# pashtari/factorizer

Hardware: AMD Instinct MI355X
Metric: volumes/sec fwd+bwd, Swin Factorizer 128^3 (higher is better)
Workload: dtype f32

## Files before the change

### factorizer_amd/csrc/mlp_chain.hip

```cpp
#include "mlp_chain.h"

using namespace fz;

static int mlp_nacc() { return 2; }

extern "C" int64_t fz_mlp_partials(int B, int64_t V) {
  const int64_t tw = 128 * mlp_nacc();
  return ((V + tw - 1) / tw) * (int64_t)B;
}

extern "C" int fz_mlp_pre_supported(int C, int H, int64_t V, int products) {
  if (!(V > 0 && (V % 4) == 0 && V <= ((int64_t)1 << 27) && products_split(products))) return 0;
  if (C == 32 && H == 64) return knob_chain_fwd_bx() ? 1 : 0;
  if (C == 64 && H == 128) return (((V + 255) / 256) % 2 == 0 && knob_chain64_p512()) ? 1 : 0;
  return 0;
}

extern "C" int fz_outproj_factors_supported(int C, int Hd, int D, int H, int W, int d, int pd, int ph, int pw, int R, int T, int Tgrad,
                                            int nshift, const int* shifts, int act_dtype, int products, int dropout) {
  if (C != 32 || Hd != 64 || act_dtype != FZ_STORE_F32 || dropout || nshift != 2) return 0;
  if (!fz_nmf_cf_factors_supported(C, D, H, W, d, pd, ph, pw, R, T, Tgrad, nshift, shifts)) return 0;
  return fz_mlp_pre_supported(C, Hd, (int64_t)D * H * W, products);
}

extern "C" int fz_mlp_supported(int C, int H, int64_t V) {
  const bool shape = (C == 32 && (H == 64 || H == 128)) || (C == 64 && H == 128);
  return (shape && V > 0 && (V % 4) == 0 && V <= ((int64_t)1 << 27)) ? 1 : 0;
}

extern "C" int fz_mlp_drop_supported(int C, int H, int64_t V, int products) {
  return (C == 32 && H == 64 && fz_mlp_supported(C, H, V) && fz_mlp_pre_supported(C, H, V, products) && products_split(products)
          && knob_chain_fwd_bx()) ? 1 : 0;
}

template <typename AT>
static void forward_args(const fz_mlp_desc* d, bool fac, int ldw, int ldwB, GemmArgsT<AT>& a, ChainArgsT<AT>& c) {
  a.w = d->w1; a.w_t = 0; a.ldw = ldw;
  a.bias = d->b1; a.ln = 1; a.ln_g = d->ln_g; a.ln_b = d->ln_b; a.ln_eps = d->ln_eps; a.stats_out = d->stats;
  a.res = (const AT*)d->in; a.y = (AT*)d->out;
  c.wB = d->w2; c.wB_t = 0; c.ldwB = ldwB; c.biasB = d->b2; c.side = (AT*)d->z1;
  if (d->pre_in || fac) {
    c.preA = (const AT*)d->pre_in; c.preW = d->pre_w; c.preB = d->pre_b; c.preRes = (const AT*)d->pre_res; c.preOut = (AT*)d->pre_out;
    if (d->C == 64) a.res = (const AT*)d->pre_out;
    else { c.postW = d->post_w; c.postB = d->post_b; c.postOut = (AT*)d->post_out; c.postM = d->post_m; }
  }
}
template <typename AT>
static void backward_args(const fz_mlp_desc* d, int ldw, int ldwB, AT* side, GemmArgsT<AT>& a, ChainArgsT<AT>& c) {
  a.w = d->w2; a.w_t = 1; a.ldw = ldw;
  a.emul = (const AT*)d->z1; a.y = (AT*)d->out;
  a.lnb_x = (const AT*)d->x1; a.lnb_stats = d->stats; a.lnb_g = d->ln_g; a.lnb_gadd = (const AT*)d->in; a.lnb_part = d->part;
  c.wB = d->w1; c.wB_t = 1; c.ldwB = ldwB; c.side = side;
}

static int mlp_check(const fz_mlp_desc* d, const fz_mlp_dropout* dd, bool drop, bool fac) {
  if (!fz_mlp_supported(d->C, d->H, d->V)) return fail(FZ_E_UNSUPPORTED, "fz_mlp_chain: needs (C, H) in {(32, 64), (32, 128), (64, 128)}, V % 4 == 0");
  if (drop) {
    if (!fz_mlp_drop_supported(d->C, d->H, d->V, d->products) || d->mode != 0 || !d->pre_in)
      return fail(FZ_E_UNSUPPORTED, "fz_mlp_chain: dropout needs (C, H) = (32, 64), split-bf16 products, mode 0 with pre_in (fz_mlp_drop_supported)");
    if (!drop_scale_ok(dd->m0, dd->s0) || !drop_scale_ok(dd->m1, dd->s1) || !drop_scale_ok(dd->m2, dd->s2))
      return fail(FZ_E_ARG, "fz_mlp_chain: a dropout scale 1 / (1 - p) must be >= 1 and finite");
  }
  if (d->C == 64 && d->mode == 2) return fail(FZ_E_UNSUPPORTED, "fz_mlp_chain: the fused weight gradients need C == 32, H == 64");
  if (d->B < 0) return fail(FZ_E_SHAPE, "fz_mlp_chain: negative batch");
  if (fac && (d->C != 32 || d->H != 64 || d->mode != 0 || d->act_dtype != FZ_STORE_F32 || drop || d->pre_in
              || !fz_mlp_pre_supported(d->C, d->H, d->V, d->products)))
    return fail(FZ_E_UNSUPPORTED, "fz_mlp_chain_fac: needs (C, H) = (32, 64), mode 0, fp32 storage, split-bf16 products, pre_in == NULL (fz_outproj_factors_supported)");
  const bool pre = d->pre_in != nullptr || fac;
  if (pre && (d->mode != 0 || !d->pre_w || !d->pre_res || !d->pre_out))
    return fail(FZ_E_ARG, "fz_mlp_chain: pre_in needs mode 0, pre_w, pre_res, pre_out (see fz_mlp_pre_supported)");
  if (pre && !fz_mlp_pre_supported(d->C, d->H, d->V, d->products))
    return fail(FZ_E_UNSUPPORTED, "fz_mlp_chain: the fused out-projection runs on split-bf16 products only (fz_mlp_pre_supported)");
  if (d->post_out && (!pre || d->C != 32 || !d->post_w || d->post_m < 1 || d->post_m > 4))
    return fail(FZ_E_ARG, "fz_mlp_chain: post_out needs pre_in, C == 32, post_w and 1 <= post_m <= 4");
  if ((!d->in && !pre) || !d->w1 || !d->w2 || !d->out || !d->z1 || !d->stats)
    return fail(FZ_E_ARG, "fz_mlp_chain: null pointer");
  if (d->mode == 0 && (!d->ln_g || !d->ln_b)) return fail(FZ_E_ARG, "fz_mlp_chain: forward needs the LayerNorm affine");
  if (d->mode == 1 && (!d->gz1 || !d->x1 || !d->ln_g || !d->part)) return fail(FZ_E_ARG, "fz_mlp_chain: backward needs gz1, x1, gamma, part");
  if (d->mode == 2 && (!d->x1 || !d->ln_g || !d->ln_b || !d->gln || !d->wpart || !d->gw1 || !d->gb1 || !d->gw2 || !d->gb2))
    return fail(FZ_E_ARG, "fz_mlp_chain: backward with weight gradients needs x1, gamma, beta, gln, wpart, gw1, gb1, gw2, gb2");
  if (d->mode == 2 && d->H == 128 && !d->glp) return fail(FZ_E_ARG, "fz_mlp_chain: the fused weight gradients at H == 128 need the glp buffer");
  if (d->mode < 0 || d->mode > 2) return fail(FZ_E_ARG, "fz_mlp_chain: bad mode");
  return FZ_OK;
}

template <typename AT>
static int mlp_launch(const fz_mlp_desc* d, const fz_mlp_dropout* dd, const fz_outproj_fac* fac, fz_stream_t stream) {
  const bool drop = dd && (dd->m0 || dd->m1 || dd->m2);
  const int rc = mlp_check(d, dd, drop, fac != nullptr);
  if (rc != FZ_OK) return rc;
  if (d->B == 0) {
    if (d->mode == 2) {
      hipStream_t s0 = (hipStream_t)stream;
      FZ_HIP_OK(hipMemsetAsync(d->gw1, 0, sizeof(float) * d->H * 32, s0));
      FZ_HIP_OK(hipMemsetAsync(d->gw2, 0, sizeof(float) * d->H * 32, s0));
      FZ_HIP_OK(hipMemsetAsync(d->gb1, 0, sizeof(float) * d->H, s0));
      FZ_HIP_OK(hipMemsetAsync(d->gb2, 0, sizeof(float) * 32, s0));
      FZ_HIP_OK(hipMemsetAsync(d->gln, 0, sizeof(float) * 64, s0));
    }
    return FZ_OK;
  }
  GemmArgsT<AT> a = {};
  ChainArgsT<AT> c = {};
  a.x[0] = (const AT*)d->in; a.nsrc = 1; a.c0 = d->C; a.Cin = d->C; a.Vin = d->V; a.M = d->H; a.K = d->C; a.Ncol = d->V; a.B = d->B;
  if (d->mode == 0) forward_args(d, fac != nullptr, d->C, d->H, a, c);
  else backward_args(d, d->H, d->C, d->mode == 1 ? (AT*)d->gz1 : (AT*)nullptr, a, c);
  if (d->C == 64) return chain64_launch(d, a, c, stream);
  if (d->mode == 2) return chain_wg_launch(d, a, c, stream);
  return chain32_launch(d, drop ? dd : nullptr, fac, a, c, stream);
}

extern "C" int fz_mlp_chain(const fz_mlp_desc* d, fz_stream_t stream) {
  if (!d) return fail(FZ_E_ARG, "fz_mlp_chain: null descriptor");
  if (d->act_dtype == FZ_STORE_F32) return mlp_launch<float>(d, nullptr, nullptr, stream);
  if (d->act_dtype == FZ_STORE_BF16) return mlp_launch<bf16>(d, nullptr, nullptr, stream);
  return fail(FZ_E_ARG, "fz_mlp_chain: act_dtype must be FZ_STORE_F32 or FZ_STORE_BF16");
}

extern "C" int fz_mlp_chain_fac(const fz_mlp_desc* d, const fz_outproj_fac* fac, fz_stream_t stream) {
  if (!d || !fac) return fail(FZ_E_ARG, "fz_mlp_chain_fac: null descriptor");
  if (d->act_dtype == FZ_STORE_F32) return mlp_launch<float>(d, nullptr, fac, stream);
  if (d->act_dtype == FZ_STORE_BF16) return mlp_launch<bf16>(d, nullptr, fac, stream);
  return fail(FZ_E_ARG, "fz_mlp_chain_fac: act_dtype must be FZ_STORE_F32 or FZ_STORE_BF16");
}

extern "C" int fz_mlp_chain_drop(const fz_mlp_desc* d, const fz_mlp_dropout* drop, fz_stream_t stream) {
  if (!d || !drop) return fail(FZ_E_ARG, "fz_mlp_chain_drop: null descriptor");
  if (d->act_dtype == FZ_STORE_F32) return mlp_launch<float>(d, drop, nullptr, stream);
  if (d->act_dtype == FZ_STORE_BF16) return mlp_launch<bf16>(d, drop, nullptr, stream);
  return fail(FZ_E_ARG, "fz_mlp_chain_drop: act_dtype must be FZ_STORE_F32 or FZ_STORE_BF16");
}
```

### factorizer_amd/csrc/mlp_chain64.hip

```cpp
#include "mlp_chain.h"

namespace fz {

template <bool HOIST, int NRB, int NQ, int NTA, int NTB, typename FA, typename FX>
__device__ __forceinline__ void bx_group(f32x16 (&acc)[NRB][NQ], FA load_a, FX get_x) {
  if constexpr (HOIST) {
    bx8 bop[NQ][NTB];
#pragma unroll
    for (int q = 0; q < NQ; ++q) {
      float x8[8];
      get_x(q, x8);
      bx_split<NTB>(x8, bop[q]);
    }
#pragma unroll
    for (int rb = 0; rb < NRB; ++rb) {
      float a8[8];
      load_a(rb, a8);
      bx8 aop[NTA];
      bx_split<NTA>(a8, aop);
#pragma unroll
      for (int q = 0; q < NQ; ++q) bx_mfma<NTA, NTB>(acc[rb][q], aop, bop[q]);
    }
  } else {
#pragma unroll
    for (int q = 0; q < NQ; ++q) {
      bx8 bop[NTB];
      {
        float x8[8];
        get_x(q, x8);
        bx_split<NTB>(x8, bop);
      }
#pragma unroll
      for (int rb = 0; rb < NRB; ++rb) {
        float a8[8];
        load_a(rb, a8);
        bx8 aop[NTA];
        bx_split<NTA>(a8, aop);
        bx_mfma<NTA, NTB>(acc[rb][q], aop, bop);
      }
      __builtin_amdgcn_sched_barrier(0);
    }
  }
}

template <int NRB, int NQ, int NTB, typename FA, typename FX>
__device__ __forceinline__ void bx_group_ps(f32x16 (&acc)[NRB][NQ], FA load_term, FX get_x) {
#pragma unroll
  for (int q = 0; q < NQ; ++q) {
    bx8 bop[NTB];
    {
      float x8[8];
      get_x(q, x8);
      bx_split<NTB>(x8, bop);
    }
#pragma unroll
    for (int rb = 0; rb < NRB; ++rb) {
#pragma unroll
      for (int t = 2; t >= 0; --t) {
        const bx8 a = load_term(rb, t);
#pragma unroll
        for (int jj = NTB - 1; jj >= 0; --jj)
          if (t + jj <= 2) acc[rb][q] = __builtin_amdgcn_mfma_f32_32x32x16_bf16(a, bop[jj], acc[rb][q], 0, 0, 0);
      }
      __builtin_amdgcn_sched_barrier(0);
    }
  }
}

template <bool BWD, typename AT, bool SINGLE = false, bool BX = false, bool P512 = false, bool PRE = false>
__global__ __launch_bounds__(P512 ? 512 : 256, 2) void gemm_chain64_kernel(GemmArgsT<AT> p, ChainArgsT<AT> c, int ntiles) {
  constexpr int NACC = 2, C = 64, HID = 128;
  constexpr int NTA = BxTerms<AT>::A, NTB = bx_terms_b<AT>(BXPRO_GELU);
  constexpr bool HOIST = SINGLE || sizeof(AT) == 2;
  static_assert(!P512 || (BX && !SINGLE), "P512: the split-bf16 chain around a pre-split weight image");
  static_assert(!PRE || (P512 && !BWD), "PRE: the forward chain around the pre-split images");
  constexpr int NA = P512 ? 12288 : 8192;
  constexpr int NA0 = PRE ? 6144 : 0;
  extern __shared__ __attribute__((aligned(16))) float fz_lds_c64[];
  float* As1 = fz_lds_c64;
  float* As2 = As1 + NA;
  float* tW = As2 + NA + NA0;
  float* tB = tW + 128;
  float* tB0 = tB + 64;
  const int half = P512 ? __builtin_amdgcn_readfirstlane((int)(threadIdx.x >> 8)) : 0;
  float* red = tB + 64 + (PRE ? 64 : 0) + half * 512;
  static_assert(2 * NA + NA0 + 128 + 64 + (PRE ? 64 : 0) + (P512 ? 2 : 1) * 512 == chain64_lds_floats(P512, PRE), "the launcher's dynamic LDS ends where this carve-up does");
  const int lane = threadIdx.x & 63, wave = __builtin_amdgcn_readfirstlane((int)(threadIdx.x >> 6) & 3);
  const int j = lane & 31, h = lane >> 5;
  const int tiles_per_sample = (int)((p.Ncol + 128 * NACC - 1) / (128 * NACC));
  int lane4 = lane * 4, lane4b = lane * 4 + NA, lane4c = lane * 4 + 2 * NA;
  if constexpr (P512) {
    asm volatile("" : "+v"(lane4));
    asm volatile("" : "+v"(lane4b));
    if constexpr (PRE) asm volatile("" : "+v"(lane4c));
  }
  auto ld_a1 = [&](int slot3) { return *reinterpret_cast<const bx8*>(As1 + slot3 * 256 + lane4); };
  auto ld_a2 = [&](int slot3) { return *reinterpret_cast<const bx8*>(As1 + slot3 * 256 + lane4b); };
  auto ld_a0 = [&](int slot3) { return *reinterpret_cast<const bx8*>(As1 + slot3 * 256 + lane4c); };
  (void)ld_a0; (void)lane4c; (void)tB0;

  if constexpr (P512) {
    for (int item = threadIdx.x; item < (PRE ? 2560 : 2048); item += 512) {
      const int l = item & 63, slot = (item >> 6) & 15, img = item >> 10;
      float a8[8];
      if (img == 0) {
        const int g = slot >> 2, rb = slot & 3;
#pragma unroll
        for (int e = 0; e < 8; ++e) {
          const int rr = 8 * (g & 1) + e;
          const int k = PRE ? (g >> 1) * 32 + (rr & 3) + 8 * (rr >> 2) + 4 * (l >> 5) : 2 * (8 * g + e) + (l >> 5);
          a8[e] = weight_at(p, rb * 32 + (l & 31), k);
          if (!BWD) a8[e] *= p.ln_g[k];
        }
      } else if (PRE && img == 2) {
        const int g = slot >> 1, mb = slot & 1;
#pragma unroll
        for (int e = 0; e < 8; ++e) a8[e] = c.preW[(int64_t)(mb * 32 + (l & 31)) * 64 + 2 * (8 * g + e) + (l >> 5)];
      } else {
        const int mb = slot & 1, g8 = (slot >> 1) & 1, rb4 = slot >> 2;
#pragma unroll
        for (int e = 0; e < 8; ++e) {
          const int r = 8 * g8 + e;
          const int k = rb4 * 32 + (r & 3) + 8 * (r >> 2) + 4 * (l >> 5), m = mb * 32 + (l & 31);
          a8[e] = c.wB_t ? c.wB[(int64_t)k * c.ldwB + m] : c.wB[(int64_t)m * c.ldwB + k];
        }
      }
      bx8 t3[3];
      bx_split<3>(a8, t3);
      bx8* dst = reinterpret_cast<bx8*>(img == 0 ? As1 : (img == 1 ? As2 : As2 + NA)) + (slot * 3) * 64 + l;
      dst[0] = t3[0]; dst[64] = t3[1]; dst[128] = t3[2];
    }
  }
  for (int base = threadIdx.x; !P512 && base < (SINGLE ? 4096 : 16384); base += 256 * 8) {
    float tmp[8];
#pragma unroll
    for (int uu = 0; uu < 8; ++uu) {
      const int idx = base + uu * 256;
      float wv;
      if (SINGLE) {
        const int l = idx & 63, mb = (idx >> 6) & 1, a = idx >> 7;
        wv = weight_at(p, mb * 32 + (l & 31), 2 * a + (l >> 5));
      } else if (idx < 8192) {
        const int l = idx & 63, rb = (idx >> 6) & 3, a = idx >> 8;
        const int m = rb * 32 + (l & 31), k = 2 * a + (l >> 5);
        wv = weight_at(p, m, k);
        if (!BWD) wv *= p.ln_g[k];
      } else {
        const int i2 = idx - 8192;
        const int l = i2 & 63, mb = (i2 >> 6) & 1, s2 = i2 >> 7;
        const int r = s2 & 15, rb = s2 >> 4;
        const int k = rb * 32 + (r & 3) + 8 * (r >> 2) + 4 * (l >> 5), m = mb * 32 + (l & 31);
        wv = c.wB_t ? c.wB[(int64_t)k * c.ldwB + m] : c.wB[(int64_t)m * c.ldwB + k];
      }
      tmp[uu] = wv;
    }
#pragma unroll
    for (int uu = 0; uu < 8; ++uu) fz_lds_c64[base + uu * 256] = tmp[uu];
  }
  if (BWD) {
    if (threadIdx.x < C) tB[threadIdx.x] = p.lnb_g[threadIdx.x];
  } else {
    for (int r = threadIdx.x; r < HID; r += blockDim.x) {
      float t = 0.f;
      for (int k = 0; k < C; ++k) t += weight_at(p, r, k) * p.ln_b[k];
      tW[r] = t + (p.bias ? p.bias[r] : 0.f);
      if (r < C) tB[r] = c.biasB ? c.biasB[r] : 0.f;
      if (PRE && r < C) tB0[r] = c.preB ? c.preB[r] : 0.f;
    }
  }

  const int tstep = P512 ? 2 * (int)gridDim.x : (int)gridDim.x;
  int tile = P512 ? 2 * (int)blockIdx.x + half : (int)blockIdx.x;
  float bv[32][NACC];
  auto fetch_tile = [&](int t) {
    const int bt = t / tiles_per_sample;
    const int64_t ct = ((int64_t)(t % tiles_per_sample) * 4 + wave) * (32 * NACC) + NACC * j;
    const unsigned lo = (unsigned)h * (unsigned)p.Ncol + (unsigned)(ct < p.Ncol ? ct : 0);
    const AT* xb = (PRE ? c.preA : p.x[0]) + (int64_t)bt * C * p.Ncol;
#pragma unroll
    for (int s = 0; s < 32; ++s) vload<NACC>(xb + (int64_t)(2 * s) * p.Ncol + lo, bv[s]);
  };
  fetch_tile(tile);
  __syncthreads();

  for (; tile < ntiles; tile += tstep) {
    asm volatile("" ::: "memory");
    const int b = tile / tiles_per_sample;
    const int64_t col_off = ((int64_t)(tile % tiles_per_sample) * 4 + wave) * (32 * NACC) + NACC * j;
    const bool col_ok = col_off < p.Ncol;
    const int64_t nc = col_ok ? col_off : 0;
    const unsigned lane_row = (unsigned)(4 * h) * (unsigned)p.Ncol + (unsigned)nc;

    f32x16 acc0[PRE ? 2 : 1][NACC];
    if constexpr (PRE) {
#pragma unroll
      for (int mb = 0; mb < 2; ++mb)
#pragma unroll
        for (int q = 0; q < NACC; ++q)
#pragma unroll
          for (int r = 0; r < 16; ++r) acc0[mb][q][r] = 0.f;
#pragma unroll
      for (int g = 0; g < 4; ++g) {
        bx_group_ps<2, NACC, NTB>(acc0,
            [&](int mb, int t) { return ld_a0((g * 2 + mb) * 3 + t); },
            [&](int q, float (&x8)[8]) {
#pragma unroll
              for (int e = 0; e < 8; ++e) x8[e] = bv[8 * g + e][q];
            });
        __builtin_amdgcn_sched_barrier(0);
      }
      const int64_t smp = (int64_t)b * C * p.Ncol;
      float s1[NACC] = {0.f, 0.f};
#pragma unroll
      for (int g8 = 0; g8 < 4; ++g8) {
        float e[8][NACC];
#pragma unroll
        for (int i = 0; i < 8; ++i) {
          const int rr = g8 * 8 + i, mb = rr >> 4, r = rr & 15;
          vload<NACC>(c.preRes + smp + (int64_t)(mb * 32 + (r & 3) + 8 * (r >> 2)) * p.Ncol + lane_row, e[i]);
        }
#pragma unroll
        for (int i = 0; i < 8; ++i) {
          const int rr = g8 * 8 + i, mb = rr >> 4, r = rr & 15;
          const int rbase = mb * 32 + (r & 3) + 8 * (r >> 2);
          const float add = tB0[rbase + 4 * h];
          float v[NACC];
#pragma unroll
          for (int q = 0; q < NACC; ++q) v[q] = acc0[mb][q][r] + add + e[i][q];
          if (col_ok) vstore<NACC>(c.preOut + smp + (int64_t)rbase * p.Ncol + lane_row, v);
#pragma unroll
          for (int q = 0; q < NACC; ++q) {
            if constexpr (sizeof(AT) == 2) v[q] = (float)(AT)v[q];
            acc0[mb][q][r] = v[q];
            s1[q] += v[q];
          }
        }
        __builtin_amdgcn_sched_barrier(0);
      }
      float mu[NACC], rs[NACC];
#pragma unroll
      for (int q = 0; q < NACC; ++q) {
        s1[q] += __shfl_xor(s1[q], 32, 64);
        mu[q] = s1[q] / 64.0f;
        float t = 0.f;
#pragma unroll
        for (int mb = 0; mb < 2; ++mb)
#pragma unroll
          for (int r = 0; r < 16; ++r) {
            const float dd = acc0[mb][q][r] - mu[q];
            t += dd * dd;
          }
        t += __shfl_xor(t, 32, 64);
        rs[q] = 1.0f / sqrtf(t / 64.0f + p.ln_eps);
#pragma unroll
        for (int mb = 0; mb < 2; ++mb)
#pragma unroll
          for (int r = 0; r < 16; ++r) acc0[mb][q][r] = (acc0[mb][q][r] - mu[q]) * rs[q];
      }
      if (p.stats_out != nullptr && h == 0 && col_ok) {
        float* so = p.stats_out + (int64_t)b * 2 * p.Vin;
        vstore<NACC>(so + col_off, mu);
        vstore<NACC>(so + p.Vin + col_off, rs);
      }
    }

    if (!BWD && !PRE) {
      float mu[NACC], rs[NACC];
#pragma unroll
      for (int e = 0; e < NACC; ++e) {
        float t = 0.f;
#pragma unroll
        for (int s = 0; s < 32; ++s) t += bv[s][e];
        t += __shfl_xor(t, 32, 64);
        mu[e] = t / 64.0f;
      }
#pragma unroll
      for (int e = 0; e < NACC; ++e) {
        float t = 0.f;
#pragma unroll
        for (int s = 0; s < 32; ++s) {
          const float d = bv[s][e] - mu[e];
          t += d * d;
        }
        t += __shfl_xor(t, 32, 64);
        rs[e] = 1.0f / sqrtf(t / 64.0f + p.ln_eps);
      }
#pragma unroll
      for (int s = 0; s < 32; ++s)
#pragma unroll
        for (int e = 0; e < NACC; ++e) bv[s][e] = (bv[s][e] - mu[e]) * rs[e];
      if (p.stats_out != nullptr && h == 0 && col_ok) {
        float* so = p.stats_out + (int64_t)b * 2 * p.Vin;
        vstore<NACC>(so + col_off, mu);
        vstore<NACC>(so + p.Vin + col_off, rs);
      }
    }

    f32x16 acc2[2][NACC];
#pragma unroll
    for (int mb = 0; mb < 2; ++mb)
#pragma unroll
      for (int q = 0; q < NACC; ++q)
#pragma unroll
        for (int r = 0; r < 16; ++r) acc2[mb][q][r] = 0.f;

    if (SINGLE) {
      if constexpr (BX) {
#pragma unroll
        for (int g = 0; g < 4; ++g) {
          bx_group<HOIST, 2, NACC, NTA, NTB>(acc2,
              [&](int mb, float (&a8)[8]) {
#pragma unroll
                for (int e = 0; e < 8; ++e) a8[e] = As1[((8 * g + e) * 2 + mb) * 64 + lane];
              },
              [&](int q, float (&x8)[8]) {
#pragma unroll
                for (int e = 0; e < 8; ++e) x8[e] = bv[8 * g + e][q];
              });
          __builtin_amdgcn_sched_barrier(0);
        }
      } else {
#pragma unroll
      for (int s = 0; s < 32; ++s) {
#pragma unroll
        for (int mb = 0; mb < 2; ++mb) {
          const float av = As1[(s * 2 + mb) * 64 + lane];
#pragma unroll
          for (int q = 0; q < NACC; ++q) acc2[mb][q] = __builtin_amdgcn_mfma_f32_32x32x2f32(av, bv[s][q], acc2[mb][q], 0, 0, 0);
        }
        if ((s & 3) == 3) __builtin_amdgcn_sched_barrier(0);
      }
      }
      fetch_tile(tile + tstep < ntiles ? tile + tstep : tile);
    }
#pragma unroll
    for (int p2 = 0; p2 < (SINGLE ? 0 : 2); ++p2) {
      f32x16 acc1[2][NACC];
#pragma unroll
      for (int rbl = 0; rbl < 2; ++rbl)
#pragma unroll
        for (int q = 0; q < NACC; ++q)
#pragma unroll
          for (int r = 0; r < 16; ++r) acc1[rbl][q][r] = 0.f;
      if constexpr (BX) {
#pragma unroll
        for (int g = 0; g < 4; ++g) {
          if constexpr (P512)
            bx_group_ps<2, NACC, NTB>(acc1,
                [&](int rbl, int t) { return ld_a1((g * 4 + 2 * p2 + rbl) * 3 + t); },
                [&](int q, float (&x8)[8]) {
#pragma unroll
                  for (int e = 0; e < 8; ++e) x8[e] = PRE ? acc0[PRE ? (g >> 1) : 0][q][8 * (g & 1) + e] : bv[8 * g + e][q];
                });
          else
          bx_group<HOIST, 2, NACC, NTA, NTB>(acc1,
              [&](int rbl, float (&a8)[8]) {
#pragma unroll
                for (int e = 0; e < 8; ++e) a8[e] = As1[((8 * g + e) * 4 + 2 * p2 + rbl) * 64 + lane];
              },
              [&](int q, float (&x8)[8]) {
#pragma unroll
                for (int e = 0; e < 8; ++e) x8[e] = bv[8 * g + e][q];
              });
          __builtin_amdgcn_sched_barrier(0);
        }
      } else {
#pragma unroll
      for (int s = 0; s < 32; ++s) {
#pragma unroll
        for (int rbl = 0; rbl < 2; ++rbl) {
          const float av = As1[(s * 4 + 2 * p2 + rbl) * 64 + lane];
#pragma unroll
          for (int q = 0; q < NACC; ++q) acc1[rbl][q] = __builtin_amdgcn_mfma_f32_32x32x2f32(av, bv[s][q], acc1[rbl][q], 0, 0, 0);
        }
        if ((s & 3) == 3) __builtin_amdgcn_sched_barrier(0);
      }
      }
      if (p2 == 1) fetch_tile(tile + tstep < ntiles ? tile + tstep : tile);

      if (!BWD) {
#pragma unroll
        for (int rbl = 0; rbl < 2; ++rbl)
#pragma unroll
          for (int r = 0; r < 16; ++r) {
            const int rbase = (2 * p2 + rbl) * 32 + (r & 3) + 8 * (r >> 2);
            const float add = tW[rbase + 4 * h];
            float v[NACC];
#pragma unroll
            for (int q = 0; q < NACC; ++q) v[q] = acc1[rbl][q][r] + add;
            if (col_ok) vstore<NACC>(c.side + ((int64_t)b * HID + rbase) * p.Ncol + lane_row, v);
            if constexpr (NACC == 2) {
              float gq[2];
              gelu2_f(v, gq);
              acc1[rbl][0][r] = gq[0]; acc1[rbl][1][r] = gq[1];
            } else {
#pragma unroll
              for (int q = 0; q < NACC; ++q) acc1[rbl][q][r] = gelu_f(v[q]);
            }
          }
      } else {
#pragma unroll
        for (int g8 = 0; g8 < 4; ++g8) {
          float e[8][NACC];
#pragma unroll
          for (int i = 0; i < 8; ++i) {
            const int rr = g8 * 8 + i, rbl = rr >> 4, r = rr & 15;
            const int rbase = (2 * p2 + rbl) * 32 + (r & 3) + 8 * (r >> 2);
            vload<NACC>(p.emul + ((int64_t)b * HID + rbase) * p.Ncol + lane_row, e[i]);
          }
#pragma unroll
          for (int i = 0; i < 8; ++i) {
            const int rr = g8 * 8 + i, rbl = rr >> 4, r = rr & 15;
            const int rbase = (2 * p2 + rbl) * 32 + (r & 3) + 8 * (r >> 2);
            float v[NACC];
#pragma unroll
            for (int q = 0; q < NACC; ++q) v[q] = acc1[rbl][q][r] * gelu_grad_f(e[i][q]);
            if (col_ok) vstore<NACC>(c.side + ((int64_t)b * HID + rbase) * p.Ncol + lane_row, v);
#pragma unroll
            for (int q = 0; q < NACC; ++q) acc1[rbl][q][r] = v[q];
          }
          __builtin_amdgcn_sched_barrier(0);
        }
      }

      if constexpr (BX) {
#pragma unroll
        for (int g = 0; g < 4; ++g) {
          if constexpr (P512)
            bx_group_ps<2, NACC, NTB>(acc2,
                [&](int mb, int t) { return ld_a2((((2 * p2 + (g >> 1)) * 2 + (g & 1)) * 2 + mb) * 3 + t); },
                [&](int q, float (&x8)[8]) {
#pragma unroll
                  for (int e = 0; e < 8; ++e) x8[e] = acc1[g >> 1][q][8 * (g & 1) + e];
                });
          else
          bx_group<HOIST, 2, NACC, NTA, NTB>(acc2,
              [&](int mb, float (&a8)[8]) {
#pragma unroll
                for (int e = 0; e < 8; ++e) a8[e] = As2[(((2 * p2 + (g >> 1)) * 16 + 8 * (g & 1) + e) * 2 + mb) * 64 + lane];
              },
              [&](int q, float (&x8)[8]) {
#pragma unroll
                for (int e = 0; e < 8; ++e) x8[e] = acc1[g >> 1][q][8 * (g & 1) + e];
              });
          __builtin_amdgcn_sched_barrier(0);
        }
      } else {
#pragma unroll
      for (int rbl = 0; rbl < 2; ++rbl)
#pragma unroll
        for (int r = 0; r < 16; ++r) {
#pragma unroll
          for (int mb = 0; mb < 2; ++mb) {
            const float av = As2[(((2 * p2 + rbl) * 16 + r) * 2 + mb) * 64 + lane];
#pragma unroll
            for (int q = 0; q < NACC; ++q) acc2[mb][q] = __builtin_amdgcn_mfma_f32_32x32x2f32(av, acc1[rbl][q][r], acc2[mb][q], 0, 0, 0);
          }
          if ((r & 3) == 3) __builtin_amdgcn_sched_barrier(0);
        }
      }
    }

    const int64_t sample = (int64_t)b * C * p.Ncol;
    if (!BWD) {
#pragma unroll
      for (int g8 = 0; g8 < 4; ++g8) {
        float e[8][NACC];
#pragma unroll
        for (int i = 0; i < 8; ++i) {
          const int rr = g8 * 8 + i, mb = rr >> 4, r = rr & 15;
          vload<NACC>(p.res + sample + (int64_t)(mb * 32 + (r & 3) + 8 * (r >> 2)) * p.Ncol + lane_row, e[i]);
        }
#pragma unroll
        for (int i = 0; i < 8; ++i) {
          const int rr = g8 * 8 + i, mb = rr >> 4, r = rr & 15;
          const int rbase = mb * 32 + (r & 3) + 8 * (r >> 2);
          const float add = tB[rbase + 4 * h];
          float v[NACC];
#pragma unroll
          for (int q = 0; q < NACC; ++q) v[q] = acc2[mb][q][r] + add + e[i][q];
          if (col_ok) vstore<NACC>(p.y + sample + (int64_t)rbase * p.Ncol + lane_row, v);
        }
        __builtin_amdgcn_sched_barrier(0);
      }
    } else {
      const float* sp = p.lnb_stats + (int64_t)b * 2 * p.Ncol;
      float mu[NACC], rs[NACC];
      vload<NACC>(sp + nc, mu);
      vload<NACC>(sp + p.Ncol + nc, rs);
      float xs[32][NACC];
      float m1[NACC] = {0.f, 0.f}, m2[NACC] = {0.f, 0.f};
#pragma unroll
      for (int g8 = 0; g8 < 4; ++g8) {
#pragma unroll
        for (int i = 0; i < 8; ++i) {
          const int rr = g8 * 8 + i, mb = rr >> 4, r = rr & 15;
          vload<NACC>(p.lnb_x + sample + (int64_t)(mb * 32 + (r & 3) + 8 * (r >> 2)) * p.Ncol + lane_row, xs[rr]);
        }
#pragma unroll
        for (int i = 0; i < 8; ++i) {
          const int rr = g8 * 8 + i, mb = rr >> 4, r = rr & 15;
          const float gc = tB[mb * 32 + (r & 3) + 8 * (r >> 2) + 4 * h];
#pragma unroll
          for (int q = 0; q < NACC; ++q) {
            const float av = acc2[mb][q][r] * gc;
            xs[rr][q] = (xs[rr][q] - mu[q]) * rs[q];
            m1[q] += av;
            m2[q] += av * xs[rr][q];
          }
        }
        __builtin_amdgcn_sched_barrier(0);
      }
#pragma unroll
      for (int q = 0; q < NACC; ++q) {
        m1[q] = (m1[q] + __shfl_xor(m1[q], 32, 64)) * (1.0f / 64.0f);
        m2[q] = (m2[q] + __shfl_xor(m2[q], 32, 64)) * (1.0f / 64.0f);
      }
#pragma unroll
      for (int g8 = 0; g8 < 4; ++g8) {
        float ga[8][NACC];
#pragma unroll
        for (int i = 0; i < 8; ++i) {
          const int rr = g8 * 8 + i, mb = rr >> 4, r = rr & 15;
          vload<NACC>(p.lnb_gadd + sample + (int64_t)(mb * 32 + (r & 3) + 8 * (r >> 2)) * p.Ncol + lane_row, ga[i]);
        }
#pragma unroll
        for (int i = 0; i < 8; ++i) {
          const int rr = g8 * 8 + i, mb = rr >> 4, r = rr & 15;
          const int rbase = mb * 32 + (r & 3) + 8 * (r >> 2);
          const int row = rbase + 4 * h;
          const float gc = tB[row];
          float v[NACC];
#pragma unroll
          for (int q = 0; q < NACC; ++q) v[q] = rs[q] * (acc2[mb][q][r] * gc - m1[q] - xs[rr][q] * m2[q]) + ga[i][q];
          if (col_ok) vstore<NACC>(p.y + sample + (int64_t)rbase * p.Ncol + lane_row, v);
          float sg = col_ok ? acc2[mb][0][r] * xs[rr][0] + acc2[mb][1][r] * xs[rr][1] : 0.f;
          float sb = col_ok ? acc2[mb][0][r] + acc2[mb][1][r] : 0.f;
          sg = half_sum32(sg);
          sb = half_sum32(sb);
          if ((lane & 31) == 31) {
            red[wave * 128 + row] = sg;
            red[wave * 128 + 64 + row] = sb;
          }
        }
        __builtin_amdgcn_sched_barrier(0);
      }
      __syncthreads();
      if ((threadIdx.x & 255) < 128) {
        const int e = threadIdx.x & 255;
        p.lnb_part[(int64_t)tile * 128 + e] = (red[e] + red[128 + e]) + (red[256 + e] + red[384 + e]);
      }
      __syncthreads();
    }
  }
}

template <typename AT>
int chain64_launch(const fz_mlp_desc* d, const GemmArgsT<AT>& a, const ChainArgsT<AT>& c, fz_stream_t stream) {
  const int ntiles = (int)fz_mlp_partials(d->B, d->V);
  const bool bwd = d->mode != 0, pre = d->pre_in != nullptr;
  const bool p512 = products_split(d->products) && ntiles % 2 == 0 && knob_chain64_p512();
  if (pre && !p512) return fail(FZ_E_UNSUPPORTED, "fz_mlp_chain: the fused out-projection at C == 64 needs an even number of tiles");
  void (*kern)(GemmArgsT<AT>, ChainArgsT<AT>, int) =
      pre ? gemm_chain64_kernel<false, AT, false, true, true, true>
      : p512 ? (bwd ? gemm_chain64_kernel<true, AT, false, true, true> : gemm_chain64_kernel<false, AT, false, true, true>)
             : (bwd ? gemm_chain64_kernel<true, AT, false, false> : gemm_chain64_kernel<false, AT, false, false>);
  const int work = p512 ? ntiles / 2 : ntiles, wgs = p512 ? 256 : knob_mlp_wgs(512);
  return launch_lds(kern, dim3((unsigned)(work < wgs ? work : wgs)), dim3(p512 ? 512 : 256), chain64_lds_floats(p512, pre),
                    (hipStream_t)stream, a, c, ntiles);
}
template int chain64_launch<float>(const fz_mlp_desc*, const GemmArgsT<float>&, const ChainArgsT<float>&, fz_stream_t);
template int chain64_launch<bf16>(const fz_mlp_desc*, const GemmArgsT<bf16>&, const ChainArgsT<bf16>&, fz_stream_t);

template <typename AT>
int chain64_lnb_launch(const fz_gemm_desc* d, const GemmArgsT<AT>& a, fz_stream_t stream) {
  if (d->Ncol % 4 != 0) return fail(FZ_E_UNSUPPORTED, "fz_gemm: voxel count must be a multiple of 4");
  if (!d->lnb_gadd) return fail(FZ_E_UNSUPPORTED, "fz_gemm: the 64-channel LayerNorm-backward epilogue needs the added gradient");
  ChainArgsT<AT> c = {};
  const int ntiles = (int)fz_mlp_partials(d->B, d->Ncol);
  if (gemm_plan_only())
    return gemm_plan_form("chain64_lnb %s grid=%dx1", products_split(d->products) ? "split" : "fp32", ntiles < 512 ? ntiles : 512);
  auto kern = products_split(d->products) ? gemm_chain64_kernel<true, AT, true, true> : gemm_chain64_kernel<true, AT, true, false>;
  return launch_lds(kern, dim3((unsigned)(ntiles < 512 ? ntiles : 512)), dim3(256), chain64_lds_floats(false, false),
                    (hipStream_t)stream, a, c, ntiles);
}
template int chain64_lnb_launch<float>(const fz_gemm_desc*, const GemmArgsT<float>&, fz_stream_t);
template int chain64_lnb_launch<bf16>(const fz_gemm_desc*, const GemmArgsT<bf16>&, fz_stream_t);

}
```

### factorizer_amd/pointwise.py

```python
from __future__ import annotations

import collections
import ctypes
import functools
import os
import threading as _threading
import weakref

import torch
import torch.nn.functional as F

from . import _native as N
from . import gradbuf as _GB
from . import functional as Fn

ACT = dict(zip(("none", "relu", "gelu"), N.constants("ACT_NONE", "ACT_RELU", "ACT_GELU")))
LOAD_PLAIN, LOAD_S2D, LOAD_K3, LOAD_S2D_2D, LOAD_K3_2D = N.constants("LOAD_PLAIN", "LOAD_S2D", "LOAD_K3", "LOAD_S2D_2D", "LOAD_K3_2D")
EPI_PLAIN, EPI_D2S, EPI_LNBWD, EPI_D2S_2D = N.constants("EPI_PLAIN", "EPI_D2S", "EPI_LNBWD", "EPI_D2S_2D")
QL_S2D_2D, QL_K3_2D = N.constants("QL_S2D_2D", "QL_K3_2D")
_D2S_FINE = {EPI_D2S: 8, EPI_D2S_2D: 4}


_p = N.ptr


def _vox(x):
    v = 1
    for s in x.shape[2:]:
        v *= s
    return v


def _ln_stats(B, V, dev):
    return torch.empty((B, 2, V), dtype=torch.float32, device=dev)


def _gemm_desc(xs, w, y, *, B, Cin, Vin, M, K, Ncol, w_t=False, ldw=None, bias=None, ln=None, stats_out=None,
               bact=0, bmul=None, bmul_kind=0, eact=0, res=None, emul=None, emul_kind=0, src_mode=0, c0=0,
               loader=LOAD_PLAIN, epilogue=EPI_PLAIN, Di=0, Hi=0, Wi=0, Ho=0, Wo=0, name="gemm", tune=0, lnb=None):
    d = N.GemmDesc()
    d.products = N.products()
    d.tune = tune
    for i in range(4):
        d.x[i] = _p(xs[i]) if i < len(xs) else None
    d.nsrc, d.src_mode, d.c0, d.Cin, d.Vin = len(xs), src_mode, c0, Cin, Vin
    d.Di, d.Hi, d.Wi = Di, Hi, Wi
    d.w, d.w_t, d.ldw, d.M, d.K = _p(w), int(w_t), (ldw if ldw is not None else K), M, K
    d.bias = _p(bias)
    if ln is not None:
        d.ln, d.ln_g, d.ln_b, d.ln_eps = 1, _p(ln[0]), _p(ln[1]), float(ln[2])
    d.stats_out = _p(stats_out)
    d.bact, d.bmul, d.bmul_kind = bact, _p(bmul), bmul_kind
    d.eact, d.res, d.emul, d.emul_kind = eact, _p(res), _p(emul), emul_kind
    d.y, d.Ncol, d.Ho, d.Wo, d.B = _p(y), Ncol, Ho, Wo, B
    d.loader, d.epilogue = loader, epilogue
    x0 = xs[0]
    d.act_dtype = N.act_dtype(x0)
    nbytes = x0.element_size() * (sum(t.numel() for t in xs) + y.numel() + (res.numel() if res is not None else 0))
    if lnb is not None:
        d.lnb_x, d.lnb_stats, d.lnb_g, d.lnb_gadd = (_p(t) for t in lnb)
        nbytes += x0.element_size() * (lnb[0].numel() + (lnb[3].numel() if lnb[3] is not None else 0))
    return d, f"{name}_{Cin}->{M}", nbytes, B * max(Vin, Ncol * _D2S_FINE.get(epilogue, 1)), 2 * B * Ncol * M * K


def _gemm_launch(x0, d, key, nbytes, cols, flops):
    rc = Fn._timed(key, nbytes, lambda: N.lib().fz_gemm(ctypes.byref(d), N.stream_ptr(x0)), cols=cols, flops=flops)
    N.check(rc, "fz_gemm")


def _gemm(xs, w, y, **kw):
    with torch.cuda.device(xs[0].device):
        _gemm_launch(xs[0], *_gemm_desc(xs, w, y, **kw))
    return y


def _wgrad_desc(p, qs, gw, *, B, M, Cin, K, Vq, Ncols, gbias=None, pmul=None, pmul_kind=0, src_mode=0, c0=0,
                stats=None, qact=0, ln=None, loader=0, D=0, H=0, W=0, Ho=0, Wo=0, accumulate=False, name="wgrad"):
    d = N.WgradDesc()
    d.products = N.products()
    d.p, d.M, d.pmul, d.pmul_kind = _p(p), M, _p(pmul), pmul_kind
    for i in range(4):
        d.q[i] = _p(qs[i]) if i < len(qs) else None
    d.nsrc, d.src_mode, d.c0, d.Cin, d.K, d.Vq = len(qs), src_mode, c0, Cin, K, Vq
    d.D, d.H, d.W, d.N, d.Ho, d.Wo = D, H, W, Ncols, Ho, Wo
    d.stats, d.qact = _p(stats), qact
    if ln is not None:
        d.ln_g, d.ln_b = _p(ln[0]), _p(ln[1])
    d.gw, d.gbias, d.accumulate, d.B, d.loader = _p(gw), _p(gbias), int(accumulate), B, loader
    d.act_dtype = N.act_dtype(p)
    nb = N.lib().fz_wgrad_workspace_bytes(ctypes.byref(d))
    if nb < 0:
        raise N.NativeError("fz_wgrad_workspace_bytes failed")
    ws = torch.empty(max(nb // 4, 1), dtype=torch.float32, device=p.device)
    nbytes = p.element_size() * (p.numel() + sum(t.numel() for t in qs))
    return d, ws, f"{name}_{M}x{K}", nbytes, B * max(Vq, Ncols), 2 * B * Ncols * M * K


def _wgrad(p, qs, gw, **kw):
    d, ws, key, nbytes, cols, flops = _wgrad_desc(p, qs, gw, **kw)
    with torch.cuda.device(p.device), _finish_scope(ws, gw, kw.get("gbias")):
        rc = Fn._timed(key, nbytes, lambda: N.lib().fz_wgrad(ctypes.byref(d), ws.data_ptr(), N.stream_ptr(p)),
                       cols=cols, flops=flops)
    N.check(rc, "fz_wgrad")
    return gw


_WGRAD_GROUP = os.environ.get("FZ_WGRAD_GROUP", "1") != "0"


def _wgrad_group(problems, name):
    plans = [_wgrad_desc(p, qs, gw, **kw) for p, qs, gw, kw in problems]
    n = len(plans)
    descs = (ctypes.POINTER(N.WgradDesc) * n)(*[ctypes.pointer(pl[0]) for pl in plans])
    wss = (ctypes.c_void_p * n)(*[pl[1].data_ptr() for pl in plans])
    t0 = problems[0][0]
    held = [pl[1] for pl in plans] + [pr[2] for pr in problems] + [pr[3].get("gbias") for pr in problems]
    with torch.cuda.device(t0.device), _finish_scope(*held):
        rc = Fn._timed(name, sum(pl[3] for pl in plans),
                       lambda: N.lib().fz_wgrad_group(descs, wss, n, N.stream_ptr(t0)),
                       cols=max(pl[4] for pl in plans), flops=sum(pl[5] for pl in plans))
    N.check(rc, "fz_wgrad_group")


def _ln_backward(gl, x, stats, ln_w, gadd=None):
    B, C = x.shape[:2]
    V = _vox(x)
    gx = torch.empty_like(x)
    gpar = torch.empty(2 * C, dtype=torch.float32, device=x.device)
    ws = torch.empty(max(N.lib().fz_ln_bwd_workspace_bytes2(B, C, V) // 4, 1), dtype=torch.float32, device=x.device)
    with torch.cuda.device(x.device), _finish_scope(ws, gpar):
        rc = Fn._timed(f"ln_bwd_{C}", 3 * x.element_size() * x.numel(), lambda: N.lib().fz_ln_bwd(
            gl.data_ptr(), x.data_ptr(), stats.data_ptr(), ln_w.data_ptr(), _p(gadd), gx.data_ptr(), _p(gpar), _p(ws),
            B, C, V, N.act_dtype(x), N.stream_ptr(x)), cols=B * V)
    N.check(rc, "fz_ln_bwd")
    return gx, gpar[:C], gpar[C:]


def _reduce_affine_rows(part, rows, C, like):
    gpar = torch.empty(2 * C, dtype=torch.float32, device=like.device)
    tmp = torch.empty((64, 2 * C), dtype=torch.float32, device=like.device)
    with _finish_scope(part, gpar, tmp):
        rc = N.lib().fz_reduce_rows(part.data_ptr(), rows, 2 * C, gpar.data_ptr(), tmp.data_ptr(), N.stream_ptr(like))
    N.check(rc, "fz_reduce_rows")
    return gpar[:C], gpar[C:]


def _dgrad_lnbwd(gz, w2, x, stats, ln_w, gadd):
    B, C = x.shape[:2]
    V = _vox(x)
    Mz = gz.shape[1]
    fused64 = C == 64 and Mz == 64 and gadd is not None and V % 4 == 0 and os.environ.get("FZ_LNBWD64", "1") != "0"
    if not fused64 and (C != 32 or Mz > 64 or Mz % 2):
        gl = torch.empty_like(x)
        _gemm([gz], w2, gl, B=B, Cin=Mz, Vin=V, M=C, K=Mz, Ncol=V, w_t=True, ldw=C, name="linear_dgrad")
        return _ln_backward(gl, x, stats, ln_w, gadd=gadd)
    gx = torch.empty_like(x)
    d, *timed = _gemm_desc([gz], w2, gx, B=B, Cin=Mz, Vin=V, M=C, K=Mz, Ncol=V, w_t=True, ldw=C, epilogue=EPI_LNBWD,
                           lnb=(x, stats, ln_w, gadd), name="dgrad_lnbwd")
    rows = N.lib().fz_gemm_lnbwd_partials(ctypes.byref(d))
    part = torch.empty((rows, 2 * C), dtype=torch.float32, device=x.device)
    d.lnb_part = part.data_ptr()
    with torch.cuda.device(x.device):
        _gemm_launch(gz, d, *timed)
        ggamma, gbeta = _reduce_affine_rows(part, rows, C, x)
    return gx, ggamma, gbeta


def _dw_fused_ok(C, V):
    return C == 32 and V % 4 == 0 and V <= (1 << 27) and os.environ.get("FZ_DW_FUSED", "1") != "0"


def _gemm_dw(g, w2, q, ln=None, stats=None, gadd=None, want_bias=False, name="dgrad_wgrad", gw_out=None, gb_out=None, drop=None,
             fac=None):
    if fac is not None:
        q = g
    B, C = q.shape[:2]
    V = _vox(q)
    dev = q.device
    y = torch.empty_like(q)
    gw = _GB.out_like(w2, (C, C), torch.float32) if gw_out is None else gw_out
    gb = (gb_out if gb_out is not None else torch.empty(C, dtype=torch.float32, device=dev)) if want_bias else None
    wpart = torch.empty(N.lib().fz_gemm_dw_workspace_bytes(B, V) // 4, dtype=torch.float32, device=dev)
    d = N.GemmDwDesc()
    d.g, d.q, d.w, d.y = g.data_ptr(), q.data_ptr() if fac is None else None, w2.data_ptr(), y.data_ptr()
    df = N.outproj_fac(*fac) if fac is not None else None
    d.wpart, d.gw, d.gb = wpart.data_ptr(), gw.data_ptr(), _p(gb)
    d.B, d.C, d.V, d.act_dtype = B, C, V, N.act_dtype(q)
    d.ldgw = gw.stride(0)
    d.ldw = w2.stride(0)
    if drop is not None:
        d.drop_m, d.drop_s = drop[0].data_ptr(), _drop_scale(drop[1])
    gpar = None
    if ln is not None:
        gpar = torch.empty(64, dtype=torch.float32, device=dev)
        d.ln, d.stats, d.ln_g, d.ln_b, d.gadd, d.gln = 1, stats.data_ptr(), ln[0].data_ptr(), ln[1].data_ptr(), _p(gadd), gpar.data_ptr()
    nbytes = q.element_size() * ((3 * q.numel() if fac is None else 2 * q.numel() + q.numel() // 4) + (gadd.numel() if gadd is not None else 0))
    with torch.cuda.device(dev), _finish_scope(wpart, gw, gb, gpar):
        rc = Fn._timed(f"{name}_{C}", nbytes,
                       lambda: (N.lib().fz_gemm_dw(ctypes.byref(d), N.stream_ptr(q)) if df is None
                                else N.lib().fz_gemm_dw_fac(ctypes.byref(d), ctypes.byref(df), N.stream_ptr(q))),
                       cols=B * V, flops=4 * B * V * C * C)
        N.check(rc, "fz_gemm_dw")
    if ln is not None:
        return y, gw, gb, gpar[:32], gpar[32:]
    return y, gw, gb, None, None


def _drop_scale(p):
    return 1.0 / (1.0 - float(ctypes.c_float(p).value))


def _mlp_dropout(drop):
    bits, ps = drop
    dd = N.MlpDropout()
    for s in range(3):
        if bits[s] is not None:
            setattr(dd, f"m{s}", bits[s].data_ptr())
            setattr(dd, f"s{s}", _drop_scale(ps[s]))
    return dd


def _mlp_drop_ok(C, Hd, V):
    return (_outproj_mlp_ok(C, Hd, V)
            and bool(N.lib().fz_mlp_drop_supported(C, Hd, V, N.products())))


def _mlp_chain_ok(C, Hd, V):
    return os.environ.get("FZ_MLP_CHAIN", "1") != "0" and bool(N.lib().fz_mlp_supported(C, Hd, V))


def _mlp_desc(mode, like, w12, w22, *, B, C, Hd, V, inp=None, b1=None, b2=None, ln_w=None, ln_b=None, eps=0.0, stats=None, z1=None,
              x1=None, out=None):
    d = N.MlpDesc()
    d.products = N.products()
    d.mode, d.inp, d.w1, d.w2, d.b1, d.b2 = mode, _p(inp), w12.data_ptr(), w22.data_ptr(), _p(b1), _p(b2)
    d.ln_g, d.ln_b, d.ln_eps = _p(ln_w), _p(ln_b), float(eps)
    d.stats, d.z1, d.x1, d.out = _p(stats), _p(z1), _p(x1), _p(out)
    d.B, d.C, d.H, d.V = B, C, Hd, V
    d.act_dtype = N.act_dtype(like)
    return d


def _mlp_chain_fwd(timed, like, ln_w, ln_b, eps, w12, b1, w22, b2, inp=None, pre=None, head=None, drop=None, fac=None):
    B, C = like.shape[:2]
    V = _vox(like)
    Hd = w12.shape[0]
    new = lambda ch: torch.empty((B, ch, *like.shape[2:]), dtype=like.dtype, device=like.device)
    z1, st, x2 = new(Hd), _ln_stats(B, V, like.device), torch.empty_like(like)
    d = _mlp_desc(0, like, w12, w22, B=B, C=C, Hd=Hd, V=V, inp=inp, b1=b1, b2=b2, ln_w=ln_w, ln_b=ln_b, eps=eps, stats=st, z1=z1, out=x2)
    x1 = logits = None
    if pre is not None:
        a, wout2, bout, x = pre
        x1 = torch.empty_like(like)
        d.pre_in, d.pre_w, d.pre_b, d.pre_res, d.pre_out = _p(a), wout2.data_ptr(), _p(bout), x.data_ptr(), x1.data_ptr()
    if head is not None:
        hw, hb = head
        logits = new(hw.shape[0])
        d.post_w, d.post_b, d.post_out, d.post_m = hw.data_ptr(), _p(hb), logits.data_ptr(), hw.shape[0]
    dd = _mlp_dropout(drop) if drop is not None else None
    df = N.outproj_fac(*fac) if fac is not None else None
    if dd is not None and df is not None:
        raise N.NativeError("fz_mlp_chain: no dropout form of the chain on the core's factors")
    key, nbytes, flops = timed

    def run():
        if df is not None:
            return N.lib().fz_mlp_chain_fac(ctypes.byref(d), ctypes.byref(df), N.stream_ptr(like))
        if dd is not None:
            return N.lib().fz_mlp_chain_drop(ctypes.byref(d), ctypes.byref(dd), N.stream_ptr(like))
        return N.lib().fz_mlp_chain(ctypes.byref(d), N.stream_ptr(like))

    with torch.cuda.device(like.device):
        rc = Fn._timed(key, nbytes, run, cols=B * V, flops=flops)
    N.check(rc, "fz_mlp_chain")
    return x1, x2, z1, st, logits


def _mlp_fwd_chain(x1, ln_w, ln_b, eps, w12, b1, w22, b2):
    B, C = x1.shape[:2]
    V = _vox(x1)
    Hd = w12.shape[0]
    timed = (f"mlp_chain_fwd_{C}", x1.element_size() * (2 * x1.numel() + B * Hd * V), 4 * B * V * C * Hd)
    _, x2, z1, st, _ = _mlp_chain_fwd(timed, x1, ln_w, ln_b, eps, w12, b1, w22, b2, inp=x1)
    return x2, z1, st


_OUTPROJ_MLP = os.environ.get("FZ_OUTPROJ_MLP", "1") != "0"


def _outproj_mlp_ok(C, Hd, V):
    return _OUTPROJ_MLP and _mlp_chain_ok(C, Hd, V) and bool(N.lib().fz_mlp_pre_supported(C, Hd, V, N.products()))


def _outproj_factors_ok(x, geo, Hd, R, T, G, drop):
    C, V = x.shape[1], _vox(x)
    return (drop is None and isinstance(geo, Fn.Geometry) and _outproj_mlp_ok(C, Hd, V) and _dw_fused_ok(C, V)
            and Fn.outproj_factors_supported(geo, Hd, R, T, G, N.act_dtype(x), False))


def _outproj_mlp_fwd_chain(a, wout2, bout, x, ln_w, ln_b, eps, w12, b1, w22, b2, head=None, drop=None, fac=None):
    B, C = x.shape[:2]
    V = _vox(x)
    Hd = w12.shape[0]
    nlogits = B * head[0].shape[0] * V if head is not None else 0
    na = x.numel() if fac is None else x.numel() // 4
    timed = (f"outproj_mlp_chain_fwd_{C}", x.element_size() * (3 * x.numel() + na + B * Hd * V + nlogits), 4 * B * V * C * Hd + 2 * B * V * C * C)
    x1, x2, z1, st, logits = _mlp_chain_fwd(timed, x, ln_w, ln_b, eps, w12, b1, w22, b2, pre=(a, wout2, bout, x), head=head, drop=drop,
                                            fac=fac)
    if head is not None:
        return x1, x2, z1, st, logits
    return x1, x2, z1, st


def _mlp_bwd_chain(g2, z1, w12, w22, x1, st, ln_w):
    B, C = x1.shape[:2]
    V = _vox(x1)
    Hd = w12.shape[0]
    gz1 = torch.empty_like(z1)
    gx1 = torch.empty_like(x1)
    rows = N.lib().fz_mlp_partials(B, V)
    part = torch.empty((rows, 2 * C), dtype=torch.float32, device=x1.device)
    d = _mlp_desc(1, x1, w12, w22, B=B, C=C, Hd=Hd, V=V, inp=g2, ln_w=ln_w, stats=st, z1=z1, x1=x1, out=gx1)
    d.gz1, d.part = gz1.data_ptr(), part.data_ptr()
    with torch.cuda.device(x1.device):
        rc = Fn._timed(f"mlp_chain_bwd_{C}", x1.element_size() * (3 * x1.numel() + 2 * z1.numel()),
                       lambda: N.lib().fz_mlp_chain(ctypes.byref(d), N.stream_ptr(x1)), cols=B * V, flops=4 * B * V * C * Hd)
        N.check(rc, "fz_mlp_chain")
        ggamma, gbeta = _reduce_affine_rows(part, rows, C, x1)
    return gz1, gx1, ggamma, gbeta


def _mlp_wgrad_fused_ok(C, Hd, V):
    return _mlp_chain_ok(C, Hd, V) and C == 32 and Hd in (64, 128) and os.environ.get("FZ_MLP_FUSED_WGRAD", "1") != "0"


def _mlp_bwd_chain_wgrad(g2, z1, w12, w22, x1, st, ln_w, ln_b):
    B, C = x1.shape[:2]
    V = _vox(x1)
    Hd = w12.shape[0]
    dev = x1.device
    gx1 = torch.empty_like(x1)
    gpar = torch.empty(64, dtype=torch.float32, device=dev)
    wpart = torch.empty(N.lib().fz_mlp_wgrad_workspace_bytes(B, V) // 4, dtype=torch.float32, device=dev)
    gw1 = _GB.out_like(w12, (Hd, C), torch.float32)
    gw2 = _GB.out_like(w22, (C, Hd), torch.float32)
    gb1 = torch.empty(Hd, dtype=torch.float32, device=dev)
    gb2 = torch.empty(C, dtype=torch.float32, device=dev)
    glp = torch.empty(x1.shape, dtype=torch.float32, device=dev) if Hd == 128 else None
    d = _mlp_desc(2, x1, w12, w22, B=B, C=C, Hd=Hd, V=V, inp=g2, ln_w=ln_w, ln_b=ln_b, stats=st, z1=z1, x1=x1, out=gx1)
    d.gln, d.wpart, d.glp = gpar.data_ptr(), wpart.data_ptr(), _p(glp)
    d.gw1, d.gb1, d.gw2, d.gb2 = gw1.data_ptr(), gb1.data_ptr(), gw2.data_ptr(), gb2.data_ptr()
    nbytes = x1.element_size() * (3 * x1.numel() + z1.numel()) + (0 if Hd == 64 else x1.element_size() * 2 * x1.numel() + 8 * x1.numel())
    with torch.cuda.device(dev), _finish_scope(wpart, gpar, gw1, gb1, gw2, gb2):
        rc = Fn._timed(f"mlp_chain_bwd_wgrad_{C}" + ("" if Hd == 64 else f"x{Hd}"), nbytes,
                       lambda: N.lib().fz_mlp_chain(ctypes.byref(d), N.stream_ptr(x1)), cols=B * V, flops=8 * B * V * C * Hd)
        N.check(rc, "fz_mlp_chain")
    return gx1, gpar[:32], gpar[32:], gw1, gb1, gw2, gb2


_SIDE = {}


def _side_stream(dev, ncols):
    lim = int(os.environ.get("FZ_SIDE_WGRAD", "0"))
    if lim <= 0 or ncols > lim:
        return None
    key = (dev.type, dev.index)
    if key not in _SIDE:
        _SIDE[key] = torch.cuda.Stream(device=dev)
    return _SIDE[key]


class _LateJoin:
    enabled = False
    keep = []
    owed = []
    devices = set()
    queued = False
    verified = 0


def _end_of_backward():
    _LateJoin.queued = False
    join_wgrad_streams()


def reset_late_join():
    d = _LateJoin
    if d.devices:
        wait_wgrad_streams()
    d.owed.clear()
    d.keep.clear()
    d.queued = False


def late_wgrad_join(flag: bool = True):
    if not flag:
        join_wgrad_streams()
    _LateJoin.enabled = bool(flag) and os.environ.get("FZ_LATE_JOIN", "1") != "0"


def wait_wgrad_streams():
    d = _LateJoin
    for key in list(d.devices):
        dev = torch.device(*key)
        torch.cuda.current_stream(dev).wait_stream(_SIDE[key])
    d.devices.clear()
    d.keep.clear()


def wait_wgrad_streams_all(dev):
    key = (dev.type, dev.index if dev.index is not None else torch.cuda.current_device())
    st = _SIDE.get(key)
    if st is not None:
        torch.cuda.current_stream(dev).wait_stream(st)


def join_wgrad_streams():
    d = _LateJoin
    wait_wgrad_streams()
    owed, d.owed = d.owed, []
    d.verified += len(owed)
    for ref, ptr in owed:
        prm = ref()
        if prm is not None and prm.is_leaf and prm.requires_grad and (prm.grad is None or prm.grad.data_ptr() != ptr):
            raise RuntimeError("late_wgrad_join: a weight gradient was copied or replaced before the kernel "
                               "writing it had finished (accumulating into an existing .grad?); call "
                               "factorizer_amd.pointwise.late_wgrad_join(False) for this training loop")


class _Defer:
    enabled = False
    armed = False
    suppress = 0
    owned = frozenset()
    seen = set()
    keep = {}
    lock = _threading.Lock()
    queued = False
    flushed = 0
    flushes = 0
    refused = 0
    own_hooks = weakref.WeakSet()


def defer_finishes(flag: bool = True):
    if not flag:
        flush_finishes(disarm=True)
    _Defer.enabled = bool(flag) and os.environ.get("FZ_DEFER_FINISH", "1") != "0"


def arm_deferred_finishes(params=()):
    flush_finishes(disarm=True)
    d = _Defer
    d.queued = False
    d.owned = params if isinstance(params, frozenset) else frozenset(id(p) for p in params)
    d.seen = set()
    d.armed = d.enabled and bool(d.owned)


def flush_finishes(disarm: bool = False):
    d = _Defer
    if disarm:
        d.armed = False
    with d.lock:
        devs, keep, d.keep = list(d.keep), d.keep, {}
    for idx in devs:
        with torch.cuda.device(idx):
            n = N.lib().fz_finish_pending()
            if n:
                rc = Fn._timed("finish_batch", 0, lambda: N.lib().fz_finish_flush_all(torch.cuda.current_stream(idx).cuda_stream), cols=0)
                if rc < 0:
                    N.check(rc, "fz_finish_flush_all")
                d.flushed += rc
                d.flushes += 1
    keep.clear()


def _end_of_backward_finishes():
    _Defer.queued = False
    _Defer.seen = set()
    flush_finishes(disarm=True)


class _finish_scope:

    def __init__(self, *tensors):
        self.tensors = tensors
        self.on = False

    def __enter__(self):
        d = _Defer
        if d.armed and d.suppress == 0:
            t0 = next((t for t in self.tensors if t is not None), None)
            if t0 is not None and t0.is_cuda:
                if not d.queued:
                    try:
                        torch.autograd.Variable._execution_engine.queue_callback(_end_of_backward_finishes)
                        d.queued = True
                    except RuntimeError:
                        return self
                held = [t.detach() for t in self.tensors if t is not None]
                with d.lock:
                    d.keep.setdefault(t0.device.index, []).extend(held)
                self.was = N.lib().fz_finish_defer(1)
                self.on = True
        return self

    def __exit__(self, *exc):
        if self.on:
            N.lib().fz_finish_defer(self.was)
        return False


class _no_defer:
    def __enter__(self):
        _Defer.suppress += 1

    def __exit__(self, *exc):
        _Defer.suppress -= 1
        return False


_VIEW_NODES = frozenset(("ViewBackward0", "ReshapeAliasBackward0", "UnsafeViewBackward0", "UnsqueezeBackward0", "SqueezeBackward0",
                         "SqueezeBackward1", "AliasBackward0", "DetachBackward0"))


def _fwd(fn):
    inner = N.capture_products(fn)

    @functools.wraps(fn)
    def wrapper(ctx, *a, **kw):
        if getattr(ctx, "_fz_slots", None) is None:
            k, slots = 0, []
            for v in a:
                if isinstance(v, torch.Tensor):
                    slots.append(k)
                    k += 1
                else:
                    slots.append(-1)
            ctx._fz_slots = tuple(slots)
        return inner(ctx, *a, **kw)
    return wrapper


def owner_hook(hook):
    _Defer.own_hooks.add(hook)
    return hook


def _own_hook(hook) -> bool:
    try:
        return hook in _Defer.own_hooks
    except TypeError:
        return False


def _refuse(ctx, why):
    if os.environ.get("FZ_DEFER_DEBUG"):
        print(f"[defer] {type(ctx).__name__}: {why}", flush=True)
    return False


def _param_sinks_ok(ctx) -> bool:
    d = _Defer
    if torch.is_grad_enabled():
        return False
    acts = getattr(getattr(ctx, "_forward_cls", None), "_fz_acts", (0,))
    slots = getattr(ctx, "_fz_slots", None)
    need_grad = ctx.needs_input_grad
    nexts = ctx.next_functions
    if slots is None or len(slots) != len(need_grad) or max(slots, default=-1) + 1 != len(nexts):
        return _refuse(ctx, f"argument map {slots} does not fit {len(need_grad)} arguments / {len(nexts)} tensor inputs")
    for i, need in enumerate(need_grad):
        if not need or i in acts:
            continue
        if slots[i] < 0:
            return _refuse(ctx, f"input {i} needs a gradient and is no tensor")
        fn = nexts[slots[i]][0]
        while fn is not None and type(fn).__name__ in _VIEW_NODES:
            fn = fn.next_functions[0][0]
        if fn is None or type(fn).__name__ != "AccumulateGrad":
            return _refuse(ctx, f"input {i} sink {type(fn).__name__}")
        v = fn.variable
        vid = id(v)
        if vid not in d.owned or v.grad is not None or v._backward_hooks:
            return _refuse(ctx, f"input {i} {tuple(v.shape)} owned={vid in d.owned} grad={v.grad is not None} hooks={bool(v._backward_hooks)}")
        post = v._post_accumulate_grad_hooks
        if post and not all(_own_hook(h) for h in post.values()):
            return _refuse(ctx, f"input {i} {tuple(v.shape)} has a post-accumulate-grad hook that is not the owner's")
        if vid in d.seen:
            flush_finishes()
            return _refuse(ctx, f"input {i} {tuple(v.shape)} already served in this backward")
        d.seen.add(vid)
    return True


def _bwd(fn):
    inner = N.with_products(fn)

    @functools.wraps(fn)
    def wrapper(ctx, *a, **kw):
        d = _Defer
        if d.armed and d.suppress == 0 and not getattr(ctx, "_fz_defer_checked", False):
            ctx._fz_defer_checked = True
            if not _param_sinks_ok(ctx):
                d.refused += 1
                with _no_defer():
                    return inner(ctx, *a, **kw)
        return inner(ctx, *a, **kw)
    return wrapper


def _native_ok(*ts):
    t0 = ts[0]
    if not (t0.is_cuda and t0.numel() > 0 and t0.dtype in (torch.float32, torch.bfloat16) and _vox(t0) % 4 == 0):
        return False
    for t in ts[1:]:
        if t is None:
            continue
        if t.dim() >= 4:
            if t.dtype != t0.dtype:
                return False
        elif t.dtype != torch.float32:
            return False
    return True


def _head_rows_reduce(part, rows, w2, M, like):
    lib = N.lib()
    gw = _GB.out_like(w2, (M, 32), torch.float32)
    gb = torch.empty(M, dtype=torch.float32, device=like.device)
    st = N.stream_ptr(like)
    with _finish_scope(part, gw, gb):
        N.check(lib.fz_chunk_reduce_ld(part.data_ptr(), rows, M * 32, 132, gw.data_ptr(), 0, st), "fz_chunk_reduce_ld")
        N.check(lib.fz_chunk_reduce_ld(part.data_ptr() + 128 * 4, rows, M, 132, gb.data_ptr(), 0, st), "fz_chunk_reduce_ld")
    return gw, gb


def _head_bwd(gy, z, w2):
    B, C = z.shape[:2]
    V = _vox(z)
    M = w2.shape[0]
    lib = N.lib()
    gz = torch.empty_like(z)
    rows = lib.fz_head_bwd_rows()
    part = torch.empty(lib.fz_head_bwd_workspace_bytes() // 4, dtype=torch.float32, device=z.device)
    with torch.cuda.device(z.device):
        rc = Fn._timed(f"head_bwd_{C}->{M}", z.element_size() * (gy.numel() + 2 * z.numel()),
                       lambda: lib.fz_head_bwd(gy.data_ptr(), z.data_ptr(), w2.data_ptr(), gz.data_ptr(), part.data_ptr(),
                                               B, M, C, V, N.act_dtype(z), N.stream_ptr(z)), cols=B * V)
        N.check(rc, "fz_head_bwd")
        gw, gb = _head_rows_reduce(part, rows, w2, M, z)
    return gz, gw, gb


class LNLinearFn(torch.autograd.Function):
    @staticmethod
    @_fwd
    def forward(ctx, x, ln_w, ln_b, eps, w, b, act):
        x = x.contiguous()
        B, C = x.shape[:2]
        V = _vox(x)
        M = w.shape[0]
        w2 = w.reshape(M, C)
        y = torch.empty((B, M, *x.shape[2:]), dtype=x.dtype, device=x.device)
        stats = _ln_stats(B, V, x.device)
        _gemm([x], w2, y, B=B, Cin=C, Vin=V, M=M, K=C, Ncol=V, bias=b, ln=(ln_w, ln_b, eps), stats_out=stats,
              eact=ACT["relu" if act == "relu_out" else act], name="ln_linear")
        ctx.save_for_backward(x, stats, ln_w, ln_b, w2, y if act == "relu" else None)
        ctx.act, ctx.has_bias, ctx.wshape = act, b is not None, w.shape
        return y

    @staticmethod
    @_bwd
    def backward(ctx, gy):
        x, stats, ln_w, ln_b, w2, y = ctx.saved_tensors
        gy = gy.contiguous()
        B, C = x.shape[:2]
        V = _vox(x)
        M = w2.shape[0]
        gate = y if ctx.act == "relu" else None
        gl = torch.empty_like(x)
        _gemm([gy], w2, gl, B=B, Cin=M, Vin=V, M=C, K=M, Ncol=V, w_t=True, ldw=C, bmul=gate,
              bmul_kind=ACT["relu"], name="linear_dgrad")
        gx, ggamma, gbeta = _ln_backward(gl, x, stats, ln_w)
        gw = _GB.out_like(w2)
        gb = torch.empty(M, dtype=torch.float32, device=x.device)
        _wgrad(gy, [x], gw, B=B, M=M, Cin=C, K=C, Vq=V, Ncols=V, gbias=gb, pmul=gate, pmul_kind=ACT["relu"],
               stats=stats, ln=(ln_w, ln_b), name="wgrad_ln_linear")
        return gx, ggamma, gbeta, None, gw.reshape(ctx.wshape), (gb if ctx.has_bias else None), None


class ActLinearResFn(torch.autograd.Function):
    _fz_acts = (0, 3)

    @staticmethod
    @_fwd
    def forward(ctx, z, w, b, res, bact):
        z = z.contiguous()
        B, C = z.shape[:2]
        V = _vox(z)
        M = w.shape[0]
        w2 = w.reshape(M, C)
        if res is not None:
            res = res.contiguous()
        y = torch.empty((B, M, *z.shape[2:]), dtype=z.dtype, device=z.device)
        _gemm([z], w2, y, B=B, Cin=C, Vin=V, M=M, K=C, Ncol=V, bias=b, bact=ACT[bact], res=res,
              name="act_linear_res")
        ctx.save_for_backward(z, w2)
        ctx.bact, ctx.has_bias, ctx.has_res, ctx.wshape = bact, b is not None, res is not None, w.shape
        return y

    @staticmethod
    @_bwd
    def backward(ctx, gy):
        z, w2 = ctx.saved_tensors
        gy = gy.contiguous()
        B, C = z.shape[:2]
        V = _vox(z)
        M = w2.shape[0]
        if M <= 4 and C == 32 and ctx.bact == "none" and V % 4 == 0 and _HEAD_BWD:
            gz, gw, gb = _head_bwd(gy, z, w2)
            return gz, gw.reshape(ctx.wshape), (gb if ctx.has_bias else None), (gy if ctx.has_res else None), None
        gz = torch.empty_like(z)
        _gemm([gy], w2, gz, B=B, Cin=M, Vin=V, M=C, K=M, Ncol=V, w_t=True, ldw=C,
              emul=(z if ctx.bact != "none" else None), emul_kind=ACT[ctx.bact], name="linear_dgrad")
        gw = _GB.out_like(w2)
        gb = torch.empty(M, dtype=torch.float32, device=z.device)
        _wgrad(gy, [z], gw, B=B, M=M, Cin=C, K=C, Vq=V, Ncols=V, gbias=gb, qact=ACT[ctx.bact], name="wgrad_linear")
        return gz, gw.reshape(ctx.wshape), (gb if ctx.has_bias else None), (gy if ctx.has_res else None), None


class CatLinearFn(torch.autograd.Function):
    _fz_acts = (0, 1)

    @staticmethod
    @_fwd
    def forward(ctx, x1, x2, w, b):
        x1, x2 = x1.contiguous(), x2.contiguous()
        B, C1 = x1.shape[:2]
        C2 = x2.shape[1]
        V = _vox(x1)
        M = w.shape[0]
        w2 = w.reshape(M, C1 + C2)
        y = torch.empty((B, M, *x1.shape[2:]), dtype=x1.dtype, device=x1.device)
        _gemm([x1, x2], w2, y, B=B, Cin=C1 + C2, Vin=V, M=M, K=C1 + C2, Ncol=V, bias=b, c0=C1, name="cat_linear")
        ctx.save_for_backward(x1, x2, w2)
        ctx.has_bias, ctx.wshape = b is not None, w.shape
        return y

    @staticmethod
    @_bwd
    def backward(ctx, gy):
        x1, x2, w2 = ctx.saved_tensors
        gy = gy.contiguous()
        B, C1 = x1.shape[:2]
        C2 = x2.shape[1]
        V = _vox(x1)
        M = w2.shape[0]
        C = C1 + C2
        if M == 32 and C1 == 32 and C2 == 32 and _dw_fused_ok(M, V):
            gw = _GB.out_like(w2)
            g1, _, gb, _, _ = _gemm_dw(gy, w2[:, :C1], x1, want_bias=ctx.has_bias, name="dgrad_wgrad", gw_out=gw[:, :C1])
            g2, _, _, _, _ = _gemm_dw(gy, w2[:, C1:], x2, name="dgrad_wgrad", gw_out=gw[:, C1:])
            return g1, g2, gw.reshape(ctx.wshape), gb
        g1 = torch.empty_like(x1)
        g2 = torch.empty_like(x2)
        _gemm([gy], w2, g1, B=B, Cin=M, Vin=V, M=C1, K=M, Ncol=V, w_t=True, ldw=C, name="linear_dgrad")
        _gemm([gy], w2[:, C1:], g2, B=B, Cin=M, Vin=V, M=C2, K=M, Ncol=V, w_t=True, ldw=C, name="linear_dgrad")
        gw = _GB.out_like(w2)
        gb = torch.empty(M, dtype=torch.float32, device=gy.device)
        _wgrad(gy, [x1, x2], gw, B=B, M=M, Cin=C, K=C, Vq=V, Ncols=V, gbias=gb, c0=C1, name="wgrad_cat_linear")
        return g1, g2, gw.reshape(ctx.wshape), (gb if ctx.has_bias else None)


class LinearFn(torch.autograd.Function):
    @staticmethod
    @_fwd
    def forward(ctx, x, w, b):
        return ActLinearResFn.forward(ctx, x, w, b, None, "none")

    @staticmethod
    @_bwd
    def backward(ctx, gy):
        return ActLinearResFn.backward(ctx, gy)[:3]


class LayerNormFn(torch.autograd.Function):
    @staticmethod
    @_fwd
    def forward(ctx, x, w, b, eps):
        x = x.contiguous()
        B, C = x.shape[:2]
        V = _vox(x)
        y = torch.empty_like(x)
        stats = _ln_stats(B, V, x.device)
        with torch.cuda.device(x.device):
            rc = Fn._timed(f"ln_fwd_{C}", 2 * x.element_size() * x.numel(), lambda: N.lib().fz_ln_fwd(
                x.data_ptr(), w.data_ptr(), b.data_ptr(), y.data_ptr(), stats.data_ptr(), B, C, V, eps,
                N.act_dtype(x), N.stream_ptr(x)), cols=B * V)
        N.check(rc, "fz_ln_fwd")
        ctx.save_for_backward(x, stats, w)
        return y

    @staticmethod
    @_bwd
    def backward(ctx, gy):
        x, stats, w = ctx.saved_tensors
        gy = gy.contiguous()
        B, C = x.shape[:2]
        V = _vox(x)
        gx, ggamma, gbeta = _ln_backward(gy, x, stats, w)
        return gx, ggamma, gbeta, None


_Rank = collections.namedtuple("_Rank", "taps2 taps3 s2d k3 d2s conv_k2s2 tconv_k2s2 conv_k3 k3_input k3_warn flip")
_RANK = {
    2: _Rank(4, 9, LOAD_S2D_2D, LOAD_K3_2D, EPI_D2S_2D, "conv2d_k2s2", "tconv2d_k2s2", "conv2d_k3",
             torch.nn.grad.conv2d_input, "Conv2d(k=3) input gradient", (2, 3)),
    3: _Rank(8, 27, LOAD_S2D, LOAD_K3, EPI_D2S, "conv_k2s2", "tconv_k2s2", "conv_k3",
             torch.nn.grad.conv3d_input, "Conv3d(k=3) input gradient", (2, 3, 4)),
}


def _dhw(x):
    return (1, *x.shape[2:]) if x.dim() == 4 else tuple(x.shape[2:])


class ConvK2S2Fn(torch.autograd.Function):

    @staticmethod
    @_fwd
    def forward(ctx, x, w, b):
        x = x.contiguous()
        r = _RANK[x.dim() - 2]
        B, C = x.shape[:2]
        D, H, W = _dhw(x)
        O = w.shape[0]
        y = torch.empty((B, O, *(s // 2 for s in x.shape[2:])), dtype=x.dtype, device=x.device)
        Ho, Wo = H // 2, W // 2
        _gemm([x], w, y, B=B, Cin=C, Vin=D * H * W, M=O, K=r.taps2 * C, Ncol=_vox(y), bias=b, loader=r.s2d,
              Di=D, Hi=H, Wi=W, Ho=Ho, Wo=Wo, name=r.conv_k2s2)
        ctx.save_for_backward(x, w)
        ctx.has_bias = b is not None
        return y

    @staticmethod
    @_bwd
    def backward(ctx, gy, g_skip=None):
        x, w = ctx.saved_tensors
        gy = gy.contiguous()
        r = _RANK[x.dim() - 2]
        B, C = x.shape[:2]
        D, H, W = _dhw(x)
        O = w.shape[0]
        Ho, Wo = H // 2, W // 2
        Vc = _vox(gy)
        gx = None
        if ctx.needs_input_grad[0]:
            gx = torch.empty_like(x)
            if g_skip is not None:
                g_skip = g_skip.contiguous()
            _gemm([gy], w, gx, B=B, Cin=O, Vin=Vc, M=r.taps2 * C, K=O, Ncol=Vc, w_t=True, ldw=r.taps2 * C,
                  epilogue=r.d2s, Ho=Ho, Wo=Wo, res=g_skip, name=r.conv_k2s2 + "_dgrad")
        gw = _GB.out_like(w)
        gb = torch.empty(O, dtype=torch.float32, device=x.device)
        _wgrad(gy, [x], gw, B=B, M=O, Cin=C, K=r.taps2 * C, Vq=D * H * W, Ncols=Vc, gbias=gb, loader=r.s2d,
               D=D, H=H, W=W, Ho=Ho, Wo=Wo, name="wgrad_" + r.conv_k2s2)
        return gx, gw, (gb if ctx.has_bias else None)


class SkipConvK2S2Fn(torch.autograd.Function):

    @staticmethod
    @_fwd
    def forward(ctx, x, w, b):
        y = ConvK2S2Fn.forward(ctx, x, w, b)
        return x.view_as(x), y

    @staticmethod
    @_bwd
    def backward(ctx, g_skip, gy):
        if gy is None:
            return g_skip, None, None
        return ConvK2S2Fn.backward(ctx, gy, g_skip=g_skip)


class TConvK2S2Fn(torch.autograd.Function):

    @staticmethod
    @_fwd
    def forward(ctx, x, w, b):
        x = x.contiguous()
        r = _RANK[x.dim() - 2]
        B, C = x.shape[:2]
        H, W = x.shape[-2:]
        O = w.shape[1]
        y = torch.empty((B, O, *(2 * s for s in x.shape[2:])), dtype=x.dtype, device=x.device)
        V = _vox(x)
        _gemm([x], w, y, B=B, Cin=C, Vin=V, M=r.taps2 * O, K=C, Ncol=V, w_t=True, ldw=r.taps2 * O, bias=b,
              epilogue=r.d2s, Ho=H, Wo=W, name=r.tconv_k2s2)
        ctx.save_for_backward(x, w)
        ctx.has_bias = b is not None
        return y

    @staticmethod
    @_bwd
    def backward(ctx, gy):
        x, w = ctx.saved_tensors
        gy = gy.contiguous()
        r = _RANK[x.dim() - 2]
        B, C = x.shape[:2]
        H, W = x.shape[-2:]
        Df, Hf, Wf = _dhw(gy)
        O = w.shape[1]
        V = _vox(x)
        gx = None
        if ctx.needs_input_grad[0]:
            gx = torch.empty_like(x)
            _gemm([gy], w, gx, B=B, Cin=O, Vin=r.taps2 * V, M=C, K=r.taps2 * O, Ncol=V, loader=r.s2d,
                  Di=Df, Hi=Hf, Wi=Wf, Ho=H, Wo=W, name=r.tconv_k2s2 + "_dgrad")
        gw = _GB.out_like(w)
        _wgrad(x, [gy], gw, B=B, M=C, Cin=O, K=r.taps2 * O, Vq=r.taps2 * V, Ncols=V, loader=r.s2d, D=Df, H=Hf,
               W=Wf, Ho=H, Wo=W, name="wgrad_" + r.tconv_k2s2)
        gb = None
        if ctx.has_bias:
            Vf = r.taps2 * V
            gb = torch.empty(O, dtype=torch.float32, device=x.device)
            part = torch.empty(B * N.lib().fz_rowsum_chunks(Vf) * O, dtype=torch.float32, device=x.device)
            with torch.cuda.device(x.device), _finish_scope(part, gb):
                rc = N.lib().fz_rowsum(gy.data_ptr(), part.data_ptr(), gb.data_ptr(), B, O, Vf, N.act_dtype(gy),
                                       N.stream_ptr(x))
            N.check(rc, "fz_rowsum")
        return gx, gw, gb


class ConvK3Fn(torch.autograd.Function):

    _fz_acts = (0, 3)

    @staticmethod
    @_fwd
    def forward(ctx, x, w, b, pro=None):
        x = x.contiguous()
        r = _RANK[x.dim() - 2]
        B, C = x.shape[:2]
        D, H, W = _dhw(x)
        O = w.shape[0]
        V = D * H * W
        y = torch.empty((B, O, *x.shape[2:]), dtype=x.dtype, device=x.device)
        ctx.npro = 0 if pro is None else 1
        if x.dim() == 5 and C * 27 * 64 * 4 <= 65536:
            bp = None
            if pro is not None:
                ln_w, ln_b, eps, w_in = pro
                t_pro = torch.empty_like(y)
                st_pro = torch.empty((B, 2, V), dtype=torch.float32, device=x.device)
                bp = N.BlockPrologue(ln_w.data_ptr(), ln_b.data_ptr(), float(eps), w_in.data_ptr(), t_pro.data_ptr(), st_pro.data_ptr())
            with torch.cuda.device(x.device):
                rc = Fn._timed(f"conv_k3_{C}->{O}" + ("_ln_linear" if bp is not None else ""),
                               x.element_size() * (x.numel() + y.numel() * (2 if bp is not None else 1)), lambda: N.lib().fz_conv3_fwd2(
                    x.data_ptr(), w.data_ptr(), _p(b), y.data_ptr(), B, C, O, D, H, W, N.act_dtype(x), N.products(),
                    ctypes.byref(bp) if bp is not None else None, N.stream_ptr(x)),
                    cols=B * V, flops=2 * B * V * 27 * C * O)
            N.check(rc, "fz_conv3_fwd")
        elif pro is not None:
            raise RuntimeError("ConvK3Fn: a block prologue needs the stem kernel (callers check conv3_prologue_ok)")
        else:
            _gemm([x], w, y, B=B, Cin=C, Vin=V, M=O, K=r.taps3 * C, Ncol=V, bias=b, loader=r.k3, Di=D, Hi=H, Wi=W,
                  name=r.conv_k3)
        ctx.save_for_backward(x, w)
        ctx.has_bias = b is not None
        if pro is not None:
            ctx.mark_non_differentiable(t_pro, st_pro)
            ctx.set_materialize_grads(False)
            return y, t_pro, st_pro
        return y

    @staticmethod
    @_bwd
    def backward(ctx, gy, _gt=None, _gst=None):
        x, w = ctx.saved_tensors
        if gy is None:
            gy = torch.zeros((x.shape[0], w.shape[0], *x.shape[2:]), dtype=x.dtype, device=x.device)
        gy = gy.contiguous()
        r = _RANK[x.dim() - 2]
        B, C = x.shape[:2]
        D, H, W = _dhw(x)
        O = w.shape[0]
        V = D * H * W
        gx = None
        if ctx.needs_input_grad[0]:
            if O % 2 == 0 and W % 4 == 0:
                wt = torch.flip(w, dims=r.flip).transpose(0, 1).contiguous()
                gx = torch.empty_like(x)
                _gemm([gy], wt, gx, B=B, Cin=O, Vin=V, M=C, K=r.taps3 * O, Ncol=V, loader=r.k3, Di=D, Hi=H, Wi=W,
                      name=r.conv_k3 + "_dgrad")
            else:
                _warn_composed(r.k3_warn, x)
                gx = r.k3_input(x.shape, w, gy, padding=1)
        gw = _GB.out_like(w)
        gb = torch.empty(O, dtype=torch.float32, device=x.device)
        if x.dim() == 5 and W % 32 == 0 and 27 * C <= 128:
            lib = N.lib()
            nchunk = lib.fz_conv3_wgrad_chunks(B, D, H, W)
            K = 27 * C
            part = torch.empty(nchunk * O * K, dtype=torch.float32, device=x.device)
            pbias = torch.empty(nchunk * O, dtype=torch.float32, device=x.device)
            with torch.cuda.device(x.device), _finish_scope(part, pbias, gw, gb):
                st = N.stream_ptr(x)
                prod = N.products()

                def run():
                    rc = lib.fz_conv3_wgrad_partials(gy.data_ptr(), x.data_ptr(), part.data_ptr(), pbias.data_ptr(),
                                                     B, C, O, D, H, W, N.act_dtype(x), prod, st)
                    if rc == 0:
                        rc = lib.fz_chunk_reduce(part.data_ptr(), nchunk, O * K, gw.data_ptr(), 0, st)
                    if rc == 0:
                        rc = lib.fz_chunk_reduce(pbias.data_ptr(), nchunk, O, gb.data_ptr(), 0, st)
                    return rc
                rc = Fn._timed(f"wgrad_conv_k3_{O}x{K}", x.element_size() * (x.numel() + gy.numel()), run,
                               cols=B * V, flops=2 * B * V * K * O)
            N.check(rc, "fz_conv3_wgrad")
        else:
            _wgrad(gy, [x], gw, B=B, M=O, Cin=C, K=r.taps3 * C, Vq=V, Ncols=V, gbias=gb, loader=r.k3, D=D, H=H, W=W,
                   name="wgrad_" + r.conv_k3)
        return (gx, gw, (gb if ctx.has_bias else None), None)[:len(ctx.needs_input_grad)]


def _warn_composed(op, x, *more):
    if x.is_cuda and x.numel():
        from .composed import warn_once
        dts = sorted({str(t.dtype) for t in (x, *more) if t is not None})
        warn_once(f"{op}:{tuple(x.shape)}:{dts}",
                  f"{op} on {tuple(x.shape)} ({', '.join(dts)}) is outside the native kernel set (needs fp32 or "
                  "bf16 activations with fp32 parameters, an even channel count and a voxel count divisible by 4); "
                  "using composed framework ops on device")


def linear_cf(x, weight, bias=None):
    if _native_ok(x, weight, bias) and weight.shape[1] % 2 == 0:
        return LinearFn.apply(x, weight, bias)
    _warn_composed("Linear", x, weight, bias)
    B, C = x.shape[:2]
    y = torch.matmul(weight.reshape(weight.shape[0], weight.shape[1]), x.reshape(B, C, _vox(x)))
    if bias is not None:
        y = y + bias.view(1, -1, 1)
    return y.reshape(B, weight.shape[0], *x.shape[2:])


def layernorm_cf(x, weight, bias, eps):
    if weight is not None and bias is not None and _native_ok(x, weight, bias):
        return LayerNormFn.apply(x, weight, bias, eps)
    _warn_composed("LayerNorm", x, weight, bias)
    y = F.layer_norm(x.movedim(1, -1), (x.shape[1],), weight, bias, eps)
    return y.movedim(-1, 1).contiguous()


def mlp_cf(x, w1, b1, w2, b2):
    if _native_ok(x, w1, b1, w2, b2) and w1.shape[1] % 2 == 0 and w2.shape[1] % 2 == 0:
        z = LinearFn.apply(x, w1, b1)
        return ActLinearResFn.apply(z, w2, b2, None, "gelu")
    _warn_composed("MLP", x, w1, b1, w2, b2)
    return linear_cf(F.gelu(linear_cf(x, w1, b1)), w2, b2)


def ln_linear(x, ln_w, ln_b, eps, w, b, act="none"):
    if _native_ok(x, ln_w, ln_b, w, b) and w.shape[1] % 2 == 0:
        return LNLinearFn.apply(x, ln_w, ln_b, eps, w, b, act)
    _warn_composed("LayerNorm+Linear", x, ln_w, ln_b, w, b)
    y = linear_cf(layernorm_cf(x, ln_w, ln_b, eps), w, b)
    return torch.relu(y) if act != "none" else y


def act_linear_res(z, w, b, res, act="none"):
    if _native_ok(z, w, b, res) and w.shape[1] % 2 == 0:
        return ActLinearResFn.apply(z, w, b, res, act)
    _warn_composed("Linear+residual", z, w, b, res)
    y = linear_cf(F.gelu(z) if act == "gelu" else z, w, b)
    return y if res is None else res + y


class UpCatLinearFn(torch.autograd.Function):

    _fz_acts = (0, 1, 6)

    @staticmethod
    @_fwd
    def forward(ctx, skip, deep, w_t, b_t, w_ad, b_ad, pro=None):
        skip, deep = skip.contiguous(), deep.contiguous()
        B, Cd, D, H, W = deep.shape
        O = w_t.shape[1]
        V = D * H * W
        C1 = skip.shape[1]
        M = w_ad.shape[0]
        w2 = w_ad.reshape(M, C1 + O)
        y = torch.empty((B, M, *skip.shape[2:]), dtype=skip.dtype, device=skip.device)
        if (M == 32 and C1 == 32 and O == 32 and _UPCAT_FWD and N.lib().fz_upcat_supported(C1, Cd, D, H, W)):
            w_b = w2[:, C1:]
            wbt = torch.empty((8, M, Cd), dtype=torch.float32, device=skip.device)
            bias = torch.empty(M, dtype=torch.float32, device=skip.device) if (b_t is not None or b_ad is not None) else None
            with torch.cuda.device(skip.device):
                N.check(N.lib().fz_upcat_compose(w_t.data_ptr(), w_b.data_ptr(), C1 + O, _p(b_t), _p(b_ad), None, wbt.data_ptr(),
                                                 _p(bias), Cd, O, M, N.stream_ptr(skip)), "fz_upcat_compose")
            es = skip.element_size()
            bp = None
            if pro is not None:
                ln_w, ln_b, eps, w_in = pro
                t_pro = torch.empty_like(y)
                st_pro = torch.empty((B, 2, 8 * V), dtype=torch.float32, device=skip.device)
                bp = N.BlockPrologue(ln_w.data_ptr(), ln_b.data_ptr(), float(eps), w_in.data_ptr(), t_pro.data_ptr(), st_pro.data_ptr())
            with torch.cuda.device(skip.device):
                rc = Fn._timed(f"upcat_{Cd}->{M}" + ("_ln_linear" if bp is not None else ""),
                               es * (skip.numel() + deep.numel() + y.numel() * (2 if bp is not None else 1)),
                               lambda: N.lib().fz_upcat2(skip.data_ptr(), deep.data_ptr(), w2.data_ptr(), C1 + O, wbt.data_ptr(),
                                                         _p(bias), y.data_ptr(), B, C1, Cd, D, H, W, N.act_dtype(skip),
                                                         ctypes.byref(bp) if bp is not None else None, N.stream_ptr(skip)),
                               cols=B * 8 * V, flops=2 * B * 8 * V * M * (C1 + Cd))
            N.check(rc, "fz_upcat")
        elif pro is not None:
            raise RuntimeError("UpCatLinearFn: a block prologue needs the one-pass forward (callers check upcat_prologue_ok)")
        else:
            up = torch.empty((B, O, 2 * D, 2 * H, 2 * W), dtype=deep.dtype, device=deep.device)
            _gemm([deep], w_t, up, B=B, Cin=Cd, Vin=V, M=8 * O, K=Cd, Ncol=V, w_t=True, ldw=8 * O, bias=b_t,
                  epilogue=EPI_D2S, Ho=H, Wo=W, name="tconv_k2s2")
            _gemm([skip, up], w2, y, B=B, Cin=C1 + O, Vin=8 * V, M=M, K=C1 + O, Ncol=8 * V, bias=b_ad, c0=C1, name="cat_linear")
        ctx.save_for_backward(skip, deep, w_t, w2, b_t)
        ctx.has_bt, ctx.has_bad, ctx.wshape = b_t is not None, b_ad is not None, w_ad.shape
        ctx.npro = 0 if pro is None else 1
        if pro is not None:
            ctx.mark_non_differentiable(t_pro, st_pro)
            ctx.set_materialize_grads(False)
            return y, t_pro, st_pro
        return y

    @staticmethod
    def _backward_three(ctx, g, skip, deep, w2, wc, gw_ad, gb_ad, gt):
        B, Cd, D, H, W = deep.shape
        V = D * H * W
        Vf = 8 * V
        C1 = skip.shape[1]
        M = w2.shape[0]
        O = w2.shape[1] - C1
        dev = g.device
        if M == 32 and C1 == 32 and _dw_fused_ok(M, Vf):
            g_skip, _, _, _, _ = _gemm_dw(g, w2[:, :C1], skip, want_bias=True, name="dgrad_wgrad",
                                          gw_out=gw_ad[:, :C1], gb_out=gb_ad)
        else:
            g_skip = torch.empty_like(skip)
            _gemm([g], w2, g_skip, B=B, Cin=M, Vin=Vf, M=C1, K=M, Ncol=Vf, w_t=True, ldw=C1 + O, name="linear_dgrad")
            gwa = torch.empty((M, C1), dtype=torch.float32, device=dev)
            with _no_defer():
                _wgrad(g, [skip], gwa, B=B, M=M, Cin=C1, K=C1, Vq=Vf, Ncols=Vf, gbias=gb_ad, name="wgrad_linear")
            gw_ad[:, :C1].copy_(gwa)
        g_deep = None
        if ctx.needs_input_grad[1]:
            g_deep = torch.empty_like(deep)
            _gemm([g], wc, g_deep, B=B, Cin=M, Vin=Vf, M=Cd, K=8 * M, Ncol=V, loader=LOAD_S2D,
                  Di=2 * D, Hi=2 * H, Wi=2 * W, Ho=H, Wo=W, name="tconv_k2s2_dgrad")
        _wgrad(deep, [g], gt, B=B, M=Cd, Cin=M, K=8 * M, Vq=Vf, Ncols=V, loader=LOAD_S2D, D=2 * D, H=2 * H,
               W=2 * W, Ho=H, Wo=W, name="wgrad_tconv_k2s2")
        return g_skip, g_deep

    @staticmethod
    @_bwd
    def backward(ctx, g, _gt=None, _gst=None):
        skip, deep, w_t, w2, b_t = ctx.saved_tensors
        if g is None:
            g = torch.zeros((skip.shape[0], w2.shape[0], *skip.shape[2:]), dtype=skip.dtype, device=skip.device)
        g = g.contiguous()
        B, Cd, D, H, W = deep.shape
        O = w_t.shape[1]
        V = D * H * W
        Vf = 8 * V
        C1 = skip.shape[1]
        M = w2.shape[0]
        dev = g.device
        gw_ad = _GB.out_like(w2)
        gb_ad = torch.empty(M, dtype=torch.float32, device=dev)
        w_b = w2[:, C1:]
        wc = torch.empty((Cd, M, 2, 2, 2), dtype=torch.float32, device=dev)
        with torch.cuda.device(dev):
            N.check(N.lib().fz_upcat_compose(w_t.data_ptr(), w_b.data_ptr(), C1 + O, None, None, wc.data_ptr(), None, None,
                                             Cd, O, M, N.stream_ptr(g)), "fz_upcat_compose")
        gt = torch.empty((Cd, M, 8), dtype=torch.float32, device=dev)
        if (M == 32 and ctx.needs_input_grad[1] and _UPCAT_BWD and skip.dtype == g.dtype == deep.dtype
                and N.lib().fz_upcat_bwd_supported(C1, Cd, D, H, W, N.act_dtype(g))
                and not ((g.data_ptr() | skip.data_ptr()) & 7 or deep.data_ptr() & 15)):
            g_skip, g_deep = torch.empty_like(skip), torch.empty_like(deep)
            ws = torch.empty(N.lib().fz_upcat_bwd_workspace_bytes(B, D, H, W) // 4, dtype=torch.float32, device=dev)
            es = g.element_size()
            with torch.cuda.device(dev), _finish_scope(ws, gt, gw_ad, gb_ad):
                rc = Fn._timed(f"upcat_bwd_{Cd}->{M}", es * (3 * g.numel() + 2 * deep.numel()),
                               lambda: N.lib().fz_upcat_bwd(g.data_ptr(), skip.data_ptr(), deep.data_ptr(), w2.data_ptr(), C1 + O,
                                                            wc.data_ptr(), g_skip.data_ptr(), g_deep.data_ptr(), ws.data_ptr(),
                                                            gw_ad.data_ptr(), C1 + O, gb_ad.data_ptr(), gt.data_ptr(), B, C1, Cd,
                                                            D, H, W, N.act_dtype(g), N.stream_ptr(g)),
                               cols=B * Vf, flops=4 * B * Vf * M * (C1 + Cd))
            N.check(rc, "fz_upcat_bwd")
        else:
            g_skip, g_deep = UpCatLinearFn._backward_three(ctx, g, skip, deep, w2, wc, gw_ad, gb_ad, gt)
        gw_t = _GB.out_like(w_t)
        gb_t = torch.empty(O, dtype=torch.float32, device=dev) if ctx.has_bt else None
        with torch.cuda.device(dev), _finish_scope(gt, gb_ad, gw_t, gw_ad, gb_t):
            N.check(N.lib().fz_upcat_wgrads(gt.data_ptr(), w_t.data_ptr(), w_b.data_ptr(), C1 + O, gb_ad.data_ptr(), _p(b_t),
                                            gw_t.data_ptr(), gw_ad[:, C1:].data_ptr(), C1 + O, _p(gb_t), Cd, O, M,
                                            N.stream_ptr(g)), "fz_upcat_wgrads")
        return (g_skip, g_deep, gw_t, gb_t, gw_ad.reshape(ctx.wshape), gb_ad if ctx.has_bad else None, None)[:len(ctx.needs_input_grad)]


_UPCAT_FWD = os.environ.get("FZ_UPCAT_FWD", "1") != "0"
_UPCAT_BWD = os.environ.get("FZ_UPCAT_BWD", "1") != "0"
_HEAD_BWD = os.environ.get("FZ_HEAD_BWD", "1") != "0"


def up_cat_linear(skip, deep, w_t, b_t, w_ad, b_ad=None, pro=None):
    return UpCatLinearFn.apply(skip, deep, w_t, b_t, w_ad, b_ad, pro)


_PRODUCER_PROLOGUE = os.environ.get("FZ_PRODUCER_PROLOGUE", "1") != "0"


def conv3_prologue_ok(x, w):
    return (_PRODUCER_PROLOGUE and x.is_cuda and x.dim() == 5 and x.shape[1] * 27 * 64 * 4 <= 65536 and x.dtype in (torch.float32, torch.bfloat16)
            and bool(N.lib().fz_conv3_prologue_supported(int(x.shape[1]), int(w.shape[0]), int(x.shape[-1]), N.products())))


def upcat_prologue_ok(skip, deep, w_t, w_ad):
    B, Cd, D, H, W = deep.shape
    O, C1, M = w_t.shape[1], skip.shape[1], w_ad.shape[0]
    return (_PRODUCER_PROLOGUE and M == 32 and C1 == 32 and O == 32 and _UPCAT_FWD and bool(N.lib().fz_upcat_supported(C1, Cd, D, H, W)))


class BlockPrologue:
    _tls = _threading.local()

    def __init__(self, x, t, st):
        self.x, self.t, self.st = x, t, st

    def __enter__(self):
        tls = BlockPrologue._tls
        self.prev = getattr(tls, "cur", None)
        tls.cur = self
        return self

    def __exit__(self, *exc):
        BlockPrologue._tls.cur = self.prev

    @staticmethod
    def take(x):
        cur = getattr(BlockPrologue._tls, "cur", None)
        if cur is not None and cur.x is x:
            return cur.t, cur.st
        return None


def cat_linear(x1, x2, w, b=None):
    if _native_ok(x1, x2, w, b) and x1.shape[1] % 2 == 0 and x2.shape[1] % 2 == 0:
        return CatLinearFn.apply(x1, x2, w, b)
    _warn_composed("cat+Linear", x1, x2, w, b)
    return linear_cf(torch.cat([x1, x2], dim=1), w, b)


def _block_dropout_bits(x, C, Hd, drop):
    B, V = x.shape[0], _vox(x)
    seed = Fn.dropout_seed(x.device)
    return tuple(None if p == 0 else Fn.dropout_keep_bits(seed, s, B, ch, V, p) for s, (ch, p) in enumerate(zip((C, Hd, C), drop)))


def _block_tail_fwd(a, wout2, bout, x, ln_w, ln_b, eps, w12, b1, w22, b2, drop=None, bits=(None, None, None)):
    B, C = x.shape[:2]
    V = _vox(x)
    Hd = w12.shape[0]
    new = lambda ch: torch.empty((B, ch, *x.shape[2:]), dtype=x.dtype, device=x.device)
    (p0, p1, p2), (m0, m1, m2) = drop or (0, 0, 0), bits
    if m0 is not None:
        o = new(C)
        _gemm([a], wout2, o, B=B, Cin=C, Vin=V, M=C, K=C, Ncol=V, bias=bout, name="linear")
        x1 = Fn.dropout_apply(N.DROP_RES, m0, p0, o, x)
        del o
    else:
        x1 = new(C)
        _gemm([a], wout2, x1, B=B, Cin=C, Vin=V, M=C, K=C, Ncol=V, bias=bout, res=x, name="act_linear_res")
    z1 = new(Hd)
    st2 = _ln_stats(B, V, x.device)
    _gemm([x1], w12, z1, B=B, Cin=C, Vin=V, M=Hd, K=C, Ncol=V, bias=b1, ln=(ln_w, ln_b, eps), stats_out=st2, name="ln_linear")
    h, bact = (Fn.dropout_apply(N.DROP_GELU, m1, p1, z1), ACT["none"]) if m1 is not None else (z1, ACT["gelu"])
    if m2 is not None:
        o = new(C)
        _gemm([h], w22, o, B=B, Cin=Hd, Vin=V, M=C, K=Hd, Ncol=V, bias=b2, bact=bact, name="linear")
        x2 = Fn.dropout_apply(N.DROP_RES, m2, p2, o, x1)
        del o
    else:
        x2 = new(C)
        _gemm([h], w22, x2, B=B, Cin=Hd, Vin=V, M=C, K=Hd, Ncol=V, bias=b2, bact=bact, res=x1, name="act_linear_res")
    return x1, x2, z1, st2


class FactorizerBlockFn(torch.autograd.Function):

    _fz_acts = (0, 4, 5, 14, 15, 16, 17, 18)

    @staticmethod
    @_fwd
    def forward(ctx, x, n1w, n1b, win, u0, v0, wout, bout, n2w, n2b, w1, b1, w2, b2, cfg, head_w=None, head_b=None,
                t_pre=None, st_pre=None):
        x = x.contiguous()
        B, C = x.shape[:2]
        V = _vox(x)
        sp = x.shape[2:]
        geo, T, G, solver, neps = cfg["geo"], cfg["T"], cfg["G"], cfg["solver"], cfg["nmf_eps"]
        win2, wout2 = win.reshape(C, C), wout.reshape(C, C)
        Hd = w1.shape[0]
        w12, w22 = w1.reshape(Hd, C), w2.reshape(C, Hd)
        u0c, v0c = u0.contiguous(), v0.contiguous()
        new = lambda ch: torch.empty((B, ch, *sp), dtype=x.dtype, device=x.device)
        drop = cfg.get("drop")
        bits = _block_dropout_bits(x, C, Hd, drop) if drop is not None else (None, None, None)
        if t_pre is not None:
            t, st1 = t_pre, st_pre
        else:
            t = new(C)
            st1 = _ln_stats(B, V, x.device)
            _gemm([x], win2, t, B=B, Cin=C, Vin=V, M=C, K=C, Ncol=V, ln=(n1w, n1b, cfg["eps1"]), stats_out=st1,
                  eact=ACT["relu"], name="ln_linear")
        m = fac = None
        R = u0c.shape[1]
        if cfg["core"] and _outproj_factors_ok(x, geo, Hd, R, T, G, drop):
            a, fac = None, (Fn.core_factors(t, u0c, v0c, geo, T, solver, neps), geo)
        elif cfg["core"]:
            a = Fn.FactCoreFn.forward(_Ctx(), t, u0c, v0c, geo, T, G, solver, neps, True)
        else:
            m = Fn._swm_fwd_raw(t, geo)
            ym, _, _ = Fn._nmf_fwd_raw(m, u0c, v0c, T, solver, neps)
            a = Fn._swm_inv_raw(ym, geo, average=True)
            del ym
        logits = None
        tail = (a, wout2, bout, x, n2w, n2b, cfg["eps2"], w12, b1, w22, b2)
        if (_mlp_drop_ok if drop is not None else _outproj_mlp_ok)(C, Hd, V) and (fac is not None or a.is_contiguous()):
            head = (head_w.reshape(head_w.shape[0], C), head_b) if head_w is not None and drop is None else None
            x1, x2, z1, st2, *logits = _outproj_mlp_fwd_chain(*tail, head=head, drop=(bits, drop) if drop is not None else None,
                                                              **({"fac": fac} if fac is not None else {}))
            logits = logits[0] if logits else None
        elif drop is None and _mlp_chain_ok(C, Hd, V):
            x1 = new(C)
            _gemm([a], wout2, x1, B=B, Cin=C, Vin=V, M=C, K=C, Ncol=V, bias=bout, res=x, name="act_linear_res")
            x2, z1, st2 = _mlp_fwd_chain(x1, n2w, n2b, cfg["eps2"], w12, b1, w22, b2)
        else:
            x1, x2, z1, st2 = _block_tail_fwd(*tail, drop, bits)
        ctx.save_for_backward(x, st1, t, a, x1, st2, z1, m, n1w, n1b, win2, u0c, v0c, wout2, n2w, n2b, w12, w22, *bits,
                              *(fac[0] if fac is not None else ()))
        ctx.cfg = cfg
        ctx.shapes = (win.shape, wout.shape, w1.shape, w2.shape)
        ctx.prm = tuple(weakref.ref(t) for t in (win, wout, bout, w1, b1, w2, b2))
        if head_w is not None:
            if logits is None:
                raise RuntimeError("FactorizerBlockFn: head fusion asked for a configuration outside fz_mlp_pre_supported "
                                   "(callers check block_head_fusable first)")
            ctx.mark_non_differentiable(logits)
            ctx.set_materialize_grads(False)
            return x2, logits
        return x2

    @staticmethod
    @_bwd
    def backward(ctx, g2, _g_logits=None):
        x, st1, t, a, x1, st2, z1, m, n1w, n1b, win2, u0c, v0c, wout2, n2w, n2b, w12, w22, *bits = ctx.saved_tensors
        bits, fac = bits[:3], (tuple(bits[3:]), ctx.cfg["geo"]) if len(bits) > 3 else None
        cfg = ctx.cfg
        drop = cfg.get("drop")
        if g2 is None:
            g2 = torch.zeros_like(x)
        g2 = g2.contiguous()
        B, C = x.shape[:2]
        V = _vox(x)
        Hd = w12.shape[0]
        dev, dt = x.device, x.dtype
        geo, T, G, solver, neps = cfg["geo"], cfg["T"], cfg["G"], cfg["solver"], cfg["nmf_eps"]
        cur = torch.cuda.current_stream(dev)
        side = _side_stream(dev, B * V)
        keep = []

        pending = []

        def wgrad(*args, **kw):
            if _WGRAD_GROUP:
                kw.pop("name", None)
                pending.append((args[0], args[1], args[2], kw))
                return args[2]
            if side is None:
                return _wgrad(*args, **kw)
            side.wait_stream(cur)
            keep.extend(t for t in (args[0], *args[1], kw.get("stats")) if t is not None)
            with torch.cuda.stream(side):
                return _wgrad(*args, **kw)

        chain = _mlp_chain_ok(C, Hd, V) and drop is None
        (p0, p1, p2), (m0, m1, m2) = drop or (0, 0, 0), bits
        if drop is None and _mlp_wgrad_fused_ok(C, Hd, V):
            gx1, gg2, gbt2, gw1, gb1, gw2, gb2 = _mlp_bwd_chain_wgrad(g2, z1, w12, w22, x1, st2, n2w, n2b)
        else:
            gelu = ACT["gelu" if m1 is None else "none"]
            gf = Fn.dropout_apply(N.DROP_RES, m2, p2, g2) if m2 is not None else g2
            gw2 = _GB.out_like(w22)
            gb2 = torch.empty(C, dtype=torch.float32, device=dev)
            if chain:
                gz1, gx1, gg2, gbt2 = _mlp_bwd_chain(g2, z1, w12, w22, x1, st2, n2w)
            else:
                gz1 = torch.empty_like(z1)
                _gemm([gf], w22, gz1, B=B, Cin=C, Vin=V, M=Hd, K=C, Ncol=V, w_t=True, ldw=Hd, emul=(z1 if m1 is None else None),
                      emul_kind=gelu, name="linear_dgrad")
                if m1 is not None:
                    gz1 = Fn.dropout_apply(N.DROP_GELU_BWD, m1, p1, gz1, z1)
            h = Fn.dropout_apply(N.DROP_GELU, m1, p1, z1) if m1 is not None else z1
            wgrad(gf, [h], gw2, B=B, M=C, Cin=Hd, K=Hd, Vq=V, Ncols=V, gbias=gb2, qact=gelu, name="wgrad_linear")
            del h, gf
            if not chain:
                gx1, gg2, gbt2 = _dgrad_lnbwd(gz1, w12, x1, st2, n2w, g2)
            gw1 = _GB.out_like(w12)
            gb1 = torch.empty(Hd, dtype=torch.float32, device=dev)
            wgrad(gz1, [x1], gw1, B=B, M=Hd, Cin=C, K=C, Vq=V, Ncols=V, gbias=gb1, stats=st2, ln=(n2w, n2b),
                  name="wgrad_ln_linear")
            del gz1
        go, go_drop = gx1, None
        if m0 is not None:
            if _dw_fused_ok(C, V):
                go_drop = (m0, p0)
            else:
                go = Fn.dropout_apply(N.DROP_RES, m0, p0, gx1)
        dw = _dw_fused_ok(C, V)
        if dw:
            ga, gwo, gbo, _, _ = _gemm_dw(go, wout2, a, want_bias=True, name="dgrad_wgrad", drop=go_drop,
                                          **({"fac": fac} if fac is not None else {}))
        else:
            if fac is not None:
                a = Fn.factors_to_tensor(*fac, x)
            ga = torch.empty_like(a)
            _gemm([go], wout2, ga, B=B, Cin=C, Vin=V, M=C, K=C, Ncol=V, w_t=True, ldw=C, name="linear_dgrad")
            gwo = _GB.out_like(wout2)
            gbo = torch.empty(C, dtype=torch.float32, device=dev)
            wgrad(go, [a], gwo, B=B, M=C, Cin=C, K=C, Vq=V, Ncols=V, gbias=gbo, name="wgrad_linear")
        del go
        if G <= 0:
            gt = torch.zeros_like(t)
        elif cfg["core"]:
            c2 = _Ctx()
            c2.saved_tensors = (t, u0c, v0c)
            c2.cfg = (geo, T, G, solver, neps, True)
            gt = Fn.FactCoreFn.backward(c2, ga)[0]
        else:
            gym = Fn._swm_fwd_raw(ga, geo, div=geo.nshift)
            gm = Fn._nmf_bwd_raw(m, u0c, v0c, gym, None, None, T, G, solver, neps)
            del gym
            gt = Fn._swm_inv_raw(gm, geo, average=False, gate=m)
            del gm
        del ga
        if dw:
            gx, gwi, _, gg1, gbt1 = _gemm_dw(gt, win2, x, ln=(n1w, n1b), stats=st1, gadd=gx1, name="dgrad_lnbwd_wgrad")
        else:
            gx, gg1, gbt1 = _dgrad_lnbwd(gt, win2, x, st1, n1w, gx1)
            gwi = _GB.out_like(win2)
            wgrad(gt, [x], gwi, B=B, M=C, Cin=C, K=C, Vq=V, Ncols=V, stats=st1, ln=(n1w, n1b), name="wgrad_ln_linear")
        if pending:
            if side is None:
                _wgrad_group(pending, f"wgrad_block_{C}x{Hd}")
            else:
                side.wait_stream(cur)
                for pr in pending:
                    keep.extend(t for t in (pr[0], *pr[1], pr[3].get("stats"), pr[3].get("pmul")) if t is not None)
                with torch.cuda.stream(side):
                    _wgrad_group(pending, f"wgrad_block_{C}x{Hd}")
            pending.clear()
        if side is not None:
            if _LateJoin.enabled:
                _LateJoin.keep.extend(keep)
                _LateJoin.devices.add((dev.type, dev.index))
                _LateJoin.owed.extend(zip(ctx.prm, (t.data_ptr() for t in (gwi, gwo, gbo, gw1, gb1, gw2, gb2))))
                if not _LateJoin.queued:
                    _LateJoin.queued = True
                    torch.autograd.Variable._execution_engine.queue_callback(_end_of_backward)
            else:
                cur.wait_stream(side)
            keep.clear()
        s_in, s_out, s_1, s_2 = ctx.shapes
        return (gx, gg1, gbt1, gwi.reshape(s_in), None, None, gwo.reshape(s_out), gbo, gg2, gbt2,
                gw1.reshape(s_1), gb1, gw2.reshape(s_2), gb2, None, None, None, None, None)[:len(ctx.needs_input_grad)]


_head_fusion = _threading.local()


class HeadFusion:

    def __init__(self, block, head_params):
        self.block, self.head_params, self.logits = block, head_params, None

    def __enter__(self):
        self.prev = getattr(_head_fusion, "slot", None)
        _head_fusion.slot = self
        return self

    def __exit__(self, *exc):
        _head_fusion.slot = self.prev


def head_fusion_slot():
    return getattr(_head_fusion, "slot", None)


def block_head_fusable(C, Hd, V, head_w, x):
    return (C == 32 and _outproj_mlp_ok(C, Hd, V) and head_w is not None and head_w.dtype == torch.float32 and head_w.numel() == head_w.shape[0] * C
            and 1 <= head_w.shape[0] <= 4 and x.is_cuda and _HEAD_BWD)


class HeadOfBlockFn(torch.autograd.Function):

    _fz_acts = (0, 3)

    @staticmethod
    @_fwd
    def forward(ctx, y, w, b, logits):
        ctx.save_for_backward(y, w)
        ctx.has_bias, ctx.wshape = b is not None, w.shape
        return logits.view_as(logits)

    @staticmethod
    @_bwd
    def backward(ctx, gl):
        y, w = ctx.saved_tensors
        B, C = y.shape[:2]
        V = _vox(y)
        M = w.shape[0]
        w2 = w.reshape(M, C)
        gl = gl.contiguous()
        if gl.dtype != y.dtype:
            gl = gl.to(y.dtype)
        gy, gw, gb = _head_bwd(gl, y, w2)
        return gy, gw.reshape(ctx.wshape), (gb if ctx.has_bias else None), None


class _Ctx:

    saved_tensors = ()

    def save_for_backward(self, *ts):
        self.saved_tensors = ts
```

### include/factorizer_hip.h

```cpp
#ifndef FACTORIZER_HIP_H
#define FACTORIZER_HIP_H

#include <stdint.h>

#ifdef __cplusplus
extern "C" {
#endif

#define FZ_OK 0
#define FZ_E_SHAPE (-1)
#define FZ_E_UNSUPPORTED (-2)
#define FZ_E_HIP (-3)
#define FZ_E_ARG (-4)

#define FZ_STORE_F32 0
#define FZ_STORE_BF16 1

#define FZ_SOLVER_MU 0
#define FZ_SOLVER_HALS 1
#define FZ_SOLVER_CD 2
#define FZ_SOLVER_SMU 3

typedef void* fz_stream_t;

int fz_version(void);
#define FZ_ABI_VERSION 7
int fz_abi_version(void);
int fz_set_tile_order(int descending);
int fz_finish_defer(int on);
int fz_finish_pending(void);
int fz_finish_flush(fz_stream_t stream);
int fz_finish_flush_all(fz_stream_t waiter);
const char* fz_last_error_string(void);
int64_t fz_launch_count(void);

int fz_swm_fwd(const void* x, void* y, int B, int C, int D, int H, int W, int d, int pd,
               int ph, int pw, int nshift, const int* shifts, int elem_bytes, int relu,
               int div, fz_stream_t stream);

int fz_swm_inv(const void* y, void* x, int B, int C, int D, int H, int W, int d, int pd,
               int ph, int pw, int nshift, const int* shifts, int average, const void* gate,
               int act_dtype, fz_stream_t stream);

int fz_nmf_fwd(const void* x, const float* u0, const float* v0, void* y, float* u_out,
               float* v_out, int64_t nmat, int M, int N, int R, int T, int solver, float eps,
               int act_dtype, fz_stream_t stream);

int fz_nmf_bwd(const void* x, const float* u0, const float* v0, const void* gy,
               const float* gu, const float* gv, void* gx, int64_t nmat, int M, int N, int R,
               int T, int Tgrad, int solver, float eps, int act_dtype, fz_stream_t stream);

int fz_nmf_supported(int M, int N, int R, int T, int Tgrad);

int fz_gnmf_supported(int M, int64_t N, int R, int T, int Tgrad);
int64_t fz_gnmf_workspace_bytes(int64_t nmat, int M, int64_t N, int R, int T, int backward);
int fz_gnmf_launches(int T, int Tgrad, int backward);
int fz_gnmf_fwd(const float* x, const float* u0, const float* v0, float* y, float* u_out, float* v_out,
                int64_t nmat, int M, int64_t N, int R, int T, int solver, float eps, void* workspace,
                fz_stream_t stream);
int fz_gnmf_bwd(const float* x, const float* u0, const float* v0, const float* gy, const float* gu,
                const float* gv, float* gx, int64_t nmat, int M, int64_t N, int R, int T, int Tgrad, int solver,
                float eps, void* workspace, fz_stream_t stream);
int64_t fz_gnmf_workspace_bytes_act(int64_t nmat, int M, int64_t N, int R, int T, int backward, int act_dtype);
int fz_gnmf_fwd_act(const void* x, const float* u0, const float* v0, void* y, float* u_out, float* v_out,
                    int64_t nmat, int M, int64_t N, int R, int T, int solver, float eps, int act_dtype,
                    void* workspace, fz_stream_t stream);
int fz_gnmf_bwd_act(const void* x, const float* u0, const float* v0, const void* gy, const float* gu, const float* gv,
                    void* gx, int64_t nmat, int M, int64_t N, int R, int T, int Tgrad, int solver, float eps,
                    int act_dtype, void* workspace, fz_stream_t stream);

int fz_gnmfx_supported(int M, int64_t N, int R, int T, int Tgrad);
int64_t fz_gnmfx_workspace_bytes(int64_t nmat, int M, int64_t N, int R, int T, int backward);
int fz_gnmfx_launches(int M, int64_t N, int R, int T, int Tgrad, int backward);
int fz_gnmfx_fwd(const float* x, const float* u0, const float* v0, float* y, float* u_out, float* v_out,
                 int64_t nmat, int M, int64_t N, int R, int T, int solver, float eps, void* workspace,
                 fz_stream_t stream);
int fz_gnmfx_bwd(const float* x, const float* u0, const float* v0, const float* gy, const float* gu,
                 const float* gv, float* gx, int64_t nmat, int M, int64_t N, int R, int T, int Tgrad, int solver,
                 float eps, void* workspace, fz_stream_t stream);
int64_t fz_gnmfx_workspace_bytes_act(int64_t nmat, int M, int64_t N, int R, int T, int backward, int act_dtype);
int fz_gnmfx_fwd_act(const void* x, const float* u0, const float* v0, void* y, float* u_out, float* v_out,
                     int64_t nmat, int M, int64_t N, int R, int T, int solver, float eps, int act_dtype,
                     void* workspace, fz_stream_t stream);
int fz_gnmfx_bwd_act(const void* x, const float* u0, const float* v0, const void* gy, const float* gu, const float* gv,
                     void* gx, int64_t nmat, int M, int64_t N, int R, int T, int Tgrad, int solver, float eps,
                     int act_dtype, void* workspace, fz_stream_t stream);

int fz_nmf_cf_supported(int C, int D, int H, int W, int d, int pd, int ph, int pw, int R, int T, int Tgrad);
int fz_nmf_cf_fwd(const void* t, const float* u0, const float* v0, void* out, int B, int C, int D,
                  int H, int W, const int* shift, int accumulate, int divisor, int R, int T,
                  int solver, float eps, int act_dtype, fz_stream_t stream);
int fz_nmf_cf_bwd(const void* t, const float* u0, const float* v0, const void* ga, void* gt, int B,
                  int C, int D, int H, int W, const int* shift, int accumulate, int nshift,
                  int relu_gate, int R, int T, int Tgrad, int solver, float eps, int act_dtype,
                  fz_stream_t stream);

int fz_nmf_cf_factors_supported(int C, int D, int H, int W, int d, int pd, int ph, int pw, int R, int T, int Tgrad,
                                int nshift, const int* shifts);
int fz_nmf_cf_factors_to_tensor(const float* vfac0, const float* ufac0, const float* vfac1, const float* ufac1, void* out,
                                int B, int C, int D, int H, int W, const int* shift0, const int* shift1, int act_dtype,
                                fz_stream_t stream);
int fz_outproj_factors_supported(int C, int Hd, int D, int H, int W, int d, int pd, int ph, int pw, int R, int T, int Tgrad,
                                 int nshift, const int* shifts, int act_dtype, int products, int dropout);
int fz_nmf_cf_fwd_store_factors(const void* t, const float* u0, const float* v0, float* vfac, float* ufac, int B,
                                int C, int D, int H, int W, const int* shift, int R, int T, int solver, float eps,
                                int act_dtype, fz_stream_t stream);
int fz_nmf_cf_fwd_from_factors(const void* t, const float* u0, const float* v0, const float* vfac, const float* ufac,
                               void* out, int B, int C, int D, int H, int W, const int* shift, const int* prev_shift,
                               int divisor, int R, int T, int solver, float eps, int act_dtype, fz_stream_t stream);

int fz_nmf_cf_bwd_factors_supported(int C, int D, int H, int W, int d, int pd, int ph, int pw, int R, int T, int Tgrad,
                                    int solver, int relu_gate, int nshift, const int* shifts);
int fz_nmf_cf_bwd_store_factors(const void* t, const float* v0, const void* ga, float* gcfac, float* cofac, int B, int C,
                                int D, int H, int W, const int* shift, int nshift, int T, int Tgrad, float eps,
                                int act_dtype, fz_stream_t stream);
int fz_nmf_cf_bwd_from_factors(const void* t, const float* v0, const void* ga, const float* gcfac, const float* cofac,
                               void* gt, int B, int C, int D, int H, int W, const int* shift, const int* prev_shift,
                               int nshift, int T, int Tgrad, float eps, int act_dtype, fz_stream_t stream);

int fz_nmf_pcf_supported(int C, int D, int H, int W, int d, int pd, int ph, int pw, int R, int T, int Tgrad);
int fz_nmf_pcf_fwd(const void* t, const float* u0, const float* v0, void* out, int B, int C, int D, int H, int W,
                   int pd, int ph, int pw, const int* shift, int accumulate, int divisor, int R, int T, int solver,
                   float eps, int act_dtype, fz_stream_t stream);
int fz_nmf_pcf_bwd(const void* t, const float* u0, const float* v0, const void* ga, void* gt, int B, int C, int D,
                   int H, int W, int pd, int ph, int pw, const int* shift, int accumulate, int nshift, int relu_gate,
                   int R, int T, int Tgrad, int solver, float eps, int act_dtype, fz_stream_t stream);
int fz_nmf_pcf_bwd_prefers_separate(int pd, int ph, int pw, int act_dtype);
int fz_act_add(void* dst, const void* src, int64_t n, int act_dtype, fz_stream_t stream);

#define FZ_LOAD_PLAIN 0
#define FZ_LOAD_S2D 1
#define FZ_LOAD_K3 2
#define FZ_EPI_PLAIN 0
#define FZ_EPI_D2S 1
#define FZ_EPI_LNBWD 2
#define FZ_LOAD_S2D_2D 3
#define FZ_LOAD_K3_2D 4
#define FZ_EPI_D2S_2D 3
#define FZ_ACT_NONE 0
#define FZ_ACT_RELU 1
#define FZ_ACT_GELU 2

#define FZ_PRODUCTS_DEFAULT 0
#define FZ_PRODUCTS_SPLIT_BF16 1
#define FZ_PRODUCTS_FP32_MFMA 2

typedef struct fz_gemm_desc {
  const void* x[4];
  int nsrc;
  int src_mode;
  int c0;
  int Cin;
  int64_t Vin;
  int Di, Hi, Wi;
  const float* w;
  int w_t, ldw;
  int M, K;
  const float* bias;
  int ln;
  const float* ln_g;
  const float* ln_b;
  float ln_eps;
  float* stats_out;
  int bact;
  const void* bmul;
  int bmul_kind;
  int eact;
  const void* res;
  const void* emul;
  int emul_kind;
  void* y;
  int64_t Ncol;
  int Ho, Wo;
  int B;
  int loader, epilogue;
  const void* lnb_x;
  const float* lnb_stats;
  const float* lnb_g;
  const void* lnb_gadd;
  float* lnb_part;
  int act_dtype;
  int products;
  int tune;
} fz_gemm_desc;

int64_t fz_gemm_lnbwd_partials(const fz_gemm_desc* desc);
int fz_reduce_rows(const float* part, int64_t rows, int n, float* out, float* tmp, fz_stream_t stream);

int fz_gemm(const fz_gemm_desc* desc, fz_stream_t stream);
int fz_gemm_plan(const fz_gemm_desc* desc, char* form, int cap);
int fz_gemm_bx_enable(int on);

typedef struct fz_mlp_desc {
  int mode;
  const void* in;
  const float* w1;
  const float* w2;
  const float* b1;
  const float* b2;
  const float* ln_g;
  const float* ln_b;
  float ln_eps;
  float* stats;
  void* z1;
  void* gz1;
  const void* x1;
  void* out;
  float* part;
  int B, C, H;
  int64_t V;
  int act_dtype;
  void* wpart;
  float* gw1;
  float* gb1;
  float* gw2;
  float* gb2;
  float* gln;
  float* glp;
  int products;
  const void* pre_in;
  const float* pre_w;
  const float* pre_b;
  const void* pre_res;
  void* pre_out;
  const float* post_w;
  const float* post_b;
  void* post_out;
  int post_m;
} fz_mlp_desc;
typedef struct fz_mlp_dropout {
  const uint32_t* m0;
  const uint32_t* m1;
  const uint32_t* m2;
  float s0, s1, s2;
} fz_mlp_dropout;

typedef struct fz_gemm_dw_desc {
  const void* g;
  const void* q;
  const float* w;
  int ln;
  const float* stats;
  const float* ln_g;
  const float* ln_b;
  const void* gadd;
  void* y;
  float* gln;
  void* wpart;
  float* gw;
  float* gb;
  int B, C;
  int64_t V;
  int act_dtype;
  int ldgw;
  int ldw;
  const uint32_t* drop_m;
  float drop_s;
} fz_gemm_dw_desc;
int fz_gemm_dw_rows(int B, int64_t V);
int64_t fz_gemm_dw_workspace_bytes(int B, int64_t V);
int fz_gemm_dw(const fz_gemm_dw_desc* desc, fz_stream_t stream);

typedef struct fz_outproj_fac {
  const float* v[2];
  const float* u[2];
  int dims[3];
  int heads;
  int shift[6];
} fz_outproj_fac;
int fz_mlp_chain_fac(const fz_mlp_desc* desc, const fz_outproj_fac* fac, fz_stream_t stream);
int fz_gemm_dw_fac(const fz_gemm_dw_desc* desc, const fz_outproj_fac* fac, fz_stream_t stream);

int fz_head_bwd_rows(void);
int64_t fz_head_bwd_workspace_bytes(void);
int fz_head_bwd(const void* gy, const void* x, const float* w, void* gx, float* part, int B, int M, int C, int64_t V,
                int act_dtype, fz_stream_t stream);
int fz_head_fwd(const void* x, const float* w, const float* bias, void* y, int B, int M, int C, int64_t V, int act_dtype,
                fz_stream_t stream);

int fz_upcat_compose(const float* w_t, const float* w_b, int ldb, const float* b_t, const float* b_ad, float* wc, float* wbt, float* bias,
                     int Cd, int O, int M, fz_stream_t stream);
int fz_upcat_wgrads(const float* gt, const float* w_t, const float* w_b, int ldb, const float* gb_ad, const float* b_t, float* gw_t,
                    float* gw_b, int ldg, float* gb_t, int Cd, int O, int M, fz_stream_t stream);
int fz_upcat_supported(int C, int Cd, int D, int H, int W);
int fz_upcat(const void* skip, const void* deep, const float* wa, int lda, const float* wbt, const float* bias, void* out,
             int B, int C, int Cd, int D, int H, int W, int act_dtype, fz_stream_t stream);
int fz_upcat_bwd_supported(int C1, int Cd, int D, int H, int W, int act_dtype);
int64_t fz_upcat_bwd_workspace_bytes(int B, int D, int H, int W);
int fz_upcat_bwd(const void* g, const void* skip, const void* deep, const float* wa, int lda, const float* wc, void* g_skip,
                 void* g_deep, void* workspace, float* gw_a, int ldg, float* gb, float* gt, int B, int C1, int Cd, int D, int H,
                 int W, int act_dtype, fz_stream_t stream);
typedef struct fz_block_prologue {
  const float* ln_g;
  const float* ln_b;
  float ln_eps;
  const float* w;
  void* t;
  float* stats;
} fz_block_prologue;
int fz_upcat2(const void* skip, const void* deep, const float* wa, int lda, const float* wbt, const float* bias, void* out,
              int B, int C, int Cd, int D, int H, int W, int act_dtype, const fz_block_prologue* pro, fz_stream_t stream);

int fz_mlp_supported(int C, int H, int64_t V);
int fz_mlp_pre_supported(int C, int H, int64_t V, int products);
int fz_mlp_drop_supported(int C, int H, int64_t V, int products);
int64_t fz_mlp_partials(int B, int64_t V);
int fz_mlp_wgrad_rows(int B, int64_t V);
int64_t fz_mlp_wgrad_workspace_bytes(int B, int64_t V);
int fz_mlp_chain(const fz_mlp_desc* desc, fz_stream_t stream);
int fz_mlp_chain_drop(const fz_mlp_desc* desc, const fz_mlp_dropout* drop, fz_stream_t stream);

#define FZ_QL_PLAIN 0
#define FZ_QL_S2D 1
#define FZ_QL_K3 2
#define FZ_QL_S2D_2D 3
#define FZ_QL_K3_2D 4

typedef struct fz_wgrad_desc {
  const void* p;
  int M;
  const void* pmul;
  int pmul_kind;
  const void* q[4];
  int nsrc, src_mode, c0;
  int Cin;
  int K;
  int64_t Vq;
  int D, H, W;
  int64_t N;
  int Ho, Wo;
  const float* stats;
  int qact;
  const float* ln_g;
  const float* ln_b;
  float* gw;
  float* gbias;
  int accumulate;
  int B;
  int loader;
  int act_dtype;
  int products;
} fz_wgrad_desc;

int64_t fz_wgrad_workspace_bytes(const fz_wgrad_desc* desc);
int fz_wgrad(const fz_wgrad_desc* desc, void* workspace, fz_stream_t stream);
int fz_wgrad_group(const fz_wgrad_desc* const* descs, void* const* workspaces, int n, fz_stream_t stream);

int fz_ln_fwd(const void* x , const float* gamma, const float* beta, void* y ,
              float* stats, int B, int C, int64_t V, float eps, int act_dtype, fz_stream_t stream);
int64_t fz_ln_bwd_workspace_bytes(int C);
int64_t fz_ln_bwd_workspace_bytes2(int B, int C, int64_t V);
int fz_ln_bwd(const void* gl, const void* x, const float* stats, const float* gamma,
              const void* gadd, void* gx , float* gparams, void* workspace,
              int B, int C, int64_t V, int act_dtype, fz_stream_t stream);

int fz_conv3_fwd(const void* x , const float* w, const float* bias, void* y ,
                 int B, int Cin, int M, int D, int H, int W, int act_dtype, int products, fz_stream_t stream);
struct fz_block_prologue;
int fz_conv3_prologue_supported(int Cin, int M, int W, int products);
int fz_conv3_fwd2(const void* x, const float* w, const float* bias, void* y, int B, int Cin, int M, int D, int H, int W,
                  int act_dtype, int products, const struct fz_block_prologue* pro, fz_stream_t stream);
int fz_conv3_wgrad_chunks(int B, int D, int H, int W);
int fz_conv3_wgrad_partials(const void* gy, const void* x , float* part, float* part_bias, int B,
                            int Cin, int M, int D, int H, int W, int act_dtype, int products, fz_stream_t stream);
int fz_chunk_reduce(const float* part, int nchunk, int64_t n, float* out, int accumulate, fz_stream_t stream);
int fz_chunk_reduce_ld(const float* part, int nchunk, int64_t n, int64_t ld, float* out, int accumulate, fz_stream_t stream);

int fz_rowsum_chunks(int64_t V);
int fz_rowsum(const void* x , float* part, float* out, int B, int C, int64_t V, int act_dtype,
              fz_stream_t stream);

int fz_gcorr_supported(int Ci, int Co, int kd, int kh, int kw);
int fz_gcorr(const float* in, const float* w, float* out, const float* mul_a, const float* mul_b, int B, int G,
             int Ci, int Co, int D, int H, int W, int kd, int kh, int kw, int w_batched, float add_eps,
             fz_stream_t stream);
int64_t fz_gcorr_wgrad_workspace_bytes(int B, int G, int Ci, int Co, int D, int H, int W, int kd, int kh, int kw);
int fz_gcorr_wgrad(const float* in, const float* gout, float* gw, void* ws, int B, int G, int Ci, int Co, int D, int H,
                   int W, int kd, int kh, int kw, int w_batched, fz_stream_t stream);
int fz_gcorr_act(const void* in, const float* w, void* out, const void* mul_a, const void* mul_b, int B, int G,
                 int Ci, int Co, int D, int H, int W, int kd, int kh, int kw, int w_batched, float add_eps,
                 int act_dtype, fz_stream_t stream);
int fz_gcorr_wgrad_act(const void* in, const void* gout, float* gw, void* ws, int B, int G, int Ci, int Co, int D, int H,
                       int W, int kd, int kh, int kw, int w_batched, int act_dtype, fz_stream_t stream);
int fz_gcorr_mu_bwd(const void* r, const float* wT, const void* g, const void* s, const void* num, void* ds, void* dnum,
                    void* dden, int B, int G, int Ci, int Co, int D, int H, int W, int kd, int kh, int kw, int w_batched,
                    float eps, int act_dtype, fz_stream_t stream);

int fz_dice_bce_chunks(int64_t V);
int fz_dice_bce_sums(const float* z, const float* t, float* part, int planes, int64_t V, fz_stream_t stream);
int fz_dice_bce_grad(const float* z, const float* t, const float* coef, float* gz, int planes, int64_t V,
                     float cd, float cb, const float* gscale, fz_stream_t stream);

int fz_dice_ce_sums(const float* z, const float* t, float* part, int B, int C, int64_t V, fz_stream_t stream);
int fz_dice_ce_finish(const float* part, int B, int C, int64_t V, float smooth, float* loss, float* coef, fz_stream_t stream);
int fz_dice_ce_grad(const float* z, const float* t, const float* coef, float* gz, int B, int C, int64_t V,
                    float cd, float cb, const float* gscale, fz_stream_t stream);

int fz_dice_bce_ds_sums(const float* z, const void* t, float* part, int planes, int Td, int Th, int Tw, int Ld, int Lh, int Lw,
                        int tkind, fz_stream_t stream);
int fz_dice_bce_ds_grad(const float* z, const void* t, const float* coef, float* gz, int planes, int Td, int Th, int Tw,
                        int Ld, int Lh, int Lw, int tkind, float cd, float cb, const float* gscale, fz_stream_t stream);
int fz_dice_ce_ds_sums(const float* z, const void* t, float* part, int B, int C, int Td, int Th, int Tw, int Ld, int Lh, int Lw,
                       int tkind, fz_stream_t stream);
int fz_dice_ce_ds_grad(const float* z, const void* t, const float* coef, float* gz, int B, int C, int Td, int Th, int Tw,
                       int Ld, int Lh, int Lw, int tkind, float cd, float cb, const float* gscale, fz_stream_t stream);

#define FZ_LABEL_U8 0
#define FZ_LABEL_I64 1
#define FZ_LABEL_F32 2
int fz_dice_sce_sums(const float* z, const void* y, float* part, int B, int C, int64_t V, int ykind, int sq,
                     fz_stream_t stream);
int fz_dice_sce_finish(const float* part, int B, int C, int64_t V, int c0, float smooth, float* loss, float* coef,
                       fz_stream_t stream);
int fz_dice_sce_grad(const float* z, const void* y, const float* coef, float* gz, int B, int C, int64_t V, int ykind, int sq,
                     int c0, float cd, float cb, const float* gscale, fz_stream_t stream);
int fz_dice_sce_ds_sums(const float* z, const void* y, float* part, int B, int C, int Td, int Th, int Tw, int Ld, int Lh,
                        int Lw, int ykind, int sq, fz_stream_t stream);
int fz_dice_sce_ds_grad(const float* z, const void* y, const float* coef, float* gz, int B, int C, int Td, int Th, int Tw,
                        int Ld, int Lh, int Lw, int ykind, int sq, int c0, float cd, float cb, const float* gscale,
                        fz_stream_t stream);

int fz_sw_gather(const float* vol, float* win, int C, int D, int H, int W, int rd, int rh, int rw, int z0, int y0,
                 int x0, fz_stream_t stream);
int fz_sw_accumulate(const float* prob, float* out, float* cnt, const float* gz, const float* gy, const float* gx,
                     float wmin, int C, int D, int H, int W, int rd, int rh, int rw, int z0, int y0, int x0,
                     fz_stream_t stream);
int fz_sw_finalize(float* out, const float* cnt, int C, int64_t V, fz_stream_t stream);
int fz_sw_gather2(const void* img, void* win, int C, int D, int H, int W, int rd, int rh, int rw, int z0, int y0, int x0,
                  int act_dtype, fz_stream_t stream);
int fz_sw_accumulate2(const void* prob, float* out, float* cnt, const float* gz, const float* gy, const float* gx,
                      float wmin, int C, int D, int H, int W, int rd, int rh, int rw, int z0, int y0, int x0, int act_dtype,
                      fz_stream_t stream);
int fz_sw_finalize2(const float* out, const float* cnt, void* res, int C, int64_t V, int act_dtype, fz_stream_t stream);

#define FZ_SEG_F32 0
#define FZ_SEG_BF16 1
#define FZ_SEG_U8 2
int fz_seg_counts_chunks(int64_t V);
int64_t fz_seg_counts_workspace_bytes(int planes, int64_t V);
int fz_seg_counts(const void* pred, int pred_kind, const void* label, int label_kind, float bound, uint8_t* mask,
                  void* workspace, int64_t* counts, int planes, int64_t V, fz_stream_t stream);
int fz_mask_edges(const uint8_t* mask, uint8_t* edges, int64_t* counts, int planes, int nd, int D, int H, int W,
                  fz_stream_t stream);
int fz_edge_min_dist2_splits(int64_t nq, int64_t nt);
int64_t fz_edge_min_dist2_workspace_bytes(int64_t nq, int64_t nt);
int fz_edge_min_dist2(const float* q, int64_t nq, const float* t, int64_t nt, float w0, float w1, float w2, float* out,
                      void* workspace, fz_stream_t stream);
int64_t fz_seg_argmax_workspace_bytes(int B, int C, int64_t V);
int fz_seg_argmax(const void* pred, int pred_kind, const void* label, int label_kind, uint8_t* map, uint8_t* onehot,
                  void* workspace, int64_t* counts, int B, int C, int64_t V, fz_stream_t stream);

int fz_aug_record_floats(void);
int fz_aug_resample(const void* img, void* img_out, int act_dtype, int C, const uint8_t* lab, uint8_t* lab_out, int L,
                    const float* table, const int64_t* seed, float* smooth_ws, int ns, int B, int nd, int D, int H, int W,
                    fz_stream_t stream);
int fz_aug_smooth(const float* smooth_ws, void* img_out, int act_dtype, int C, const float* table, const int32_t* list, int ns,
                  int B, int nd, int D, int H, int W, fz_stream_t stream);
int fz_aug_noise_field(float* out, const int64_t* seed, int B, int C, int64_t V, fz_stream_t stream);
int fz_aug_source_words(void);
int fz_aug_crop_resample(const int64_t* sources, void* img_out, int act_dtype, int C, uint8_t* lab_out, int L, const float* table,
                         const int64_t* seed, float* smooth_ws, int ns, int B, int nd, int D, int H, int W, fz_stream_t stream);

#define FZ_VOL_F32 0
#define FZ_VOL_BF16 1
#define FZ_VOL_U8 2
#define FZ_VOL_I16 3
#define FZ_VOL_ROLE_IMAGE_IN 0
#define FZ_VOL_ROLE_IMAGE_OUT 1
#define FZ_VOL_ROLE_LABEL_IN 2
#define FZ_VOL_ROLE_LOGITS 3
typedef struct fz_vol_geom {
  int nd;
  int size[3];
  int start[3];
  int end[3];
  int pad[3];
  int out[3];
} fz_vol_geom;
int fz_vol_kind_ok(int role, int kind);
int fz_vol_bbox(const void* image, int kind, int C, int nd, int D, int H, int W, int32_t* box, fz_stream_t stream);
int64_t fz_vol_workspace_bytes(int C, const fz_vol_geom* geom);
int fz_vol_stats(const void* image, int kind, int C, const fz_vol_geom* geom, int nonzero, int channel_wise, void* workspace,
                 fz_stream_t stream);
int fz_vol_write(const void* image, int kind, void* out, int out_kind, int C, const void* label, int label_kind,
                 int label_channels, const int* class_ids, const int* class_counts, int nclass, uint8_t* label_out,
                 const fz_vol_geom* geom, int nonzero, int channel_wise, const void* workspace, float* mean, float* stdev,
                 fz_stream_t stream);
int fz_vol_restore(const void* const* logits, int K, int kind, int C, const fz_vol_geom* geom, float bound,
                   const uint8_t* label_values, uint8_t* result, fz_stream_t stream);

#define FZ_RESPACE_BILINEAR 0
#define FZ_RESPACE_NEAREST 1
typedef struct fz_respace_geom {
  int nd;
  int src_size[3];
  int src_axis[3];
  int flip[3];
  int res_size[3];
  int pad[3];
  int out[3];
  int orig_size[3];
  int box_start[3];
  double scale[3];
  double inv_scale[3];
} fz_respace_geom;
int fz_vol_respace(const float* image, int C, void* out, int out_kind, const uint8_t* label, int L, uint8_t* label_out,
                   const fz_respace_geom* geom, int mode, fz_stream_t stream);
int fz_vol_unspace(const void* const* logits, int K, int kind, int C, const fz_respace_geom* geom, int sigmoid, int discretize,
                   float threshold, void* result, fz_stream_t stream);

int fz_inorm_one_pass_max(void);
int fz_inorm_chunks(int64_t V);
int64_t fz_inorm_workspace_bytes(int64_t P, int64_t V);
int fz_inorm_fwd(const void* x, const float* weight, const float* bias, void* y, double* stats, int64_t P, int C, int64_t V,
                 double eps, int act_dtype, void* workspace, fz_stream_t stream);
int fz_inorm_bwd(const void* x, const void* gy, const float* weight, const double* stats, void* gx, float* gweight,
                 float* gbias, int64_t P, int C, int64_t V, int act_dtype, void* workspace, fz_stream_t stream);

#define FZ_GNORM_ACT_NONE 0
#define FZ_GNORM_ACT_RELU 1
#define FZ_GNORM_ACT_LEAKY_RELU 2
int fz_gnorm_one_pass_max(void);
int fz_gnorm_chunks(int cg, int64_t V);
int64_t fz_gnorm_workspace_bytes(int64_t B, int C, int G, int64_t V);
int fz_gnorm_launches(int cg, int64_t V, int backward, int affine);
int fz_gnorm_fwd(const void* x, const float* weight, const float* bias, void* y, double* stats, int64_t B, int C, int G,
                 int64_t V, double eps, int act, double negative_slope, int act_dtype, void* workspace, fz_stream_t stream);
int fz_gnorm_bwd(const void* x, const void* gy, const float* weight, const float* bias, const double* stats, void* gx,
                 float* gweight, float* gbias, int64_t B, int C, int G, int64_t V, int act, double negative_slope,
                 int act_dtype, void* workspace, fz_stream_t stream);

int fz_adamw_step(float* param, const float* grad, float* exp_avg, float* exp_avg_sq, int64_t n, float lr,
                  float beta1, float beta2, float eps, float weight_decay, int step, float grad_scale,
                  fz_stream_t stream);

#define FZ_DROP_RES 0
#define FZ_DROP_GELU 1
#define FZ_DROP_GELU_BWD 2
int64_t fz_dropout_bits_words(int B, int ch, int64_t V);
int fz_dropout_keep_bits(const int64_t* seed, int site, int B, int ch, int64_t V, float p, uint32_t* out, fz_stream_t stream);
int fz_dropout_apply(int kind, const uint32_t* bits, float p, const void* t, const void* aux, void* y, int B, int ch, int64_t V,
                     int act_dtype, fz_stream_t stream);

#ifdef __cplusplus
}
#endif
#endif
```

Baseline: 135.4.

## Fuse C=64 MLP backward weight gradients into one pair kernel and skip gz1 store

For the (C, H) = (64, 128) MLP backward, the dgrad chain now runs in a nostore mode that does not write the hidden gradient gz1 to memory. A new pair kernel recomputes what it needs from g2, z1, x1 and the LN stats and accumulates both weight gradients (w1, w2) and the biases into per-block partials, which a finish job then reduces. This is meant to remove the gz1 round trip through HBM and the separate wgrad GEMM launches. The cost is recomputing the GELU-backward product inside the wgrad kernel, plus an extra workspace and a reduction pass.

```diff
diff --git a/factorizer_amd/csrc/mlp_chain.hip b/factorizer_amd/csrc/mlp_chain.hip
--- a/factorizer_amd/csrc/mlp_chain.hip
+++ b/factorizer_amd/csrc/mlp_chain.hip
@@ -53,7 +53,7 @@
   c.wB = d->w1; c.wB_t = 1; c.ldwB = ldwB; c.side = side;
 }
 
-static int mlp_check(const fz_mlp_desc* d, const fz_mlp_dropout* dd, bool drop, bool fac) {
+static int mlp_check(const fz_mlp_desc* d, const fz_mlp_dropout* dd, bool drop, bool fac, bool nostore) {
   if (!fz_mlp_supported(d->C, d->H, d->V)) return fail(FZ_E_UNSUPPORTED, "fz_mlp_chain: needs (C, H) in {(32, 64), (32, 128), (64, 128)}, V % 4 == 0");
   if (drop) {
     if (!fz_mlp_drop_supported(d->C, d->H, d->V, d->products) || d->mode != 0 || !d->pre_in)
@@ -61,6 +61,9 @@
     if (!drop_scale_ok(dd->m0, dd->s0) || !drop_scale_ok(dd->m1, dd->s1) || !drop_scale_ok(dd->m2, dd->s2))
       return fail(FZ_E_ARG, "fz_mlp_chain: a dropout scale 1 / (1 - p) must be >= 1 and finite");
   }
+  if (nostore && (d->mode != 1 || d->C != 64 || d->H != 128 || d->act_dtype != FZ_STORE_F32))
+    return fail(FZ_E_UNSUPPORTED, "fz_mlp_chain_nostore: needs mode 1, (C, H) = (64, 128), fp32 storage");
+  if (nostore && d->gz1) return fail(FZ_E_ARG, "fz_mlp_chain_nostore: gz1 must be NULL (it is not written)");
   if (d->C == 64 && d->mode == 2) return fail(FZ_E_UNSUPPORTED, "fz_mlp_chain: the fused weight gradients need C == 32, H == 64");
   if (d->B < 0) return fail(FZ_E_SHAPE, "fz_mlp_chain: negative batch");
   if (fac && (d->C != 32 || d->H != 64 || d->mode != 0 || d->act_dtype != FZ_STORE_F32 || drop || d->pre_in
@@ -76,7 +79,7 @@
   if ((!d->in && !pre) || !d->w1 || !d->w2 || !d->out || !d->z1 || !d->stats)
     return fail(FZ_E_ARG, "fz_mlp_chain: null pointer");
   if (d->mode == 0 && (!d->ln_g || !d->ln_b)) return fail(FZ_E_ARG, "fz_mlp_chain: forward needs the LayerNorm affine");
-  if (d->mode == 1 && (!d->gz1 || !d->x1 || !d->ln_g || !d->part)) return fail(FZ_E_ARG, "fz_mlp_chain: backward needs gz1, x1, gamma, part");
+  if (d->mode == 1 && ((!d->gz1 && !nostore) || !d->x1 || !d->ln_g || !d->part)) return fail(FZ_E_ARG, "fz_mlp_chain: backward needs gz1, x1, gamma, part");
   if (d->mode == 2 && (!d->x1 || !d->ln_g || !d->ln_b || !d->gln || !d->wpart || !d->gw1 || !d->gb1 || !d->gw2 || !d->gb2))
     return fail(FZ_E_ARG, "fz_mlp_chain: backward with weight gradients needs x1, gamma, beta, gln, wpart, gw1, gb1, gw2, gb2");
   if (d->mode == 2 && d->H == 128 && !d->glp) return fail(FZ_E_ARG, "fz_mlp_chain: the fused weight gradients at H == 128 need the glp buffer");
@@ -85,9 +88,9 @@
 }
 
 template <typename AT>
-static int mlp_launch(const fz_mlp_desc* d, const fz_mlp_dropout* dd, const fz_outproj_fac* fac, fz_stream_t stream) {
+static int mlp_launch(const fz_mlp_desc* d, const fz_mlp_dropout* dd, const fz_outproj_fac* fac, fz_stream_t stream, bool nostore = false) {
   const bool drop = dd && (dd->m0 || dd->m1 || dd->m2);
-  const int rc = mlp_check(d, dd, drop, fac != nullptr);
+  const int rc = mlp_check(d, dd, drop, fac != nullptr, nostore);
   if (rc != FZ_OK) return rc;
   if (d->B == 0) {
     if (d->mode == 2) {
@@ -117,6 +120,13 @@
   return fail(FZ_E_ARG, "fz_mlp_chain: act_dtype must be FZ_STORE_F32 or FZ_STORE_BF16");
 }
 
+extern "C" int fz_mlp_chain_nostore(const fz_mlp_desc* d, fz_stream_t stream) {
+  if (!d) return fail(FZ_E_ARG, "fz_mlp_chain_nostore: null descriptor");
+  if (d->act_dtype == FZ_STORE_F32) return mlp_launch<float>(d, nullptr, nullptr, stream, true);
+  if (d->act_dtype == FZ_STORE_BF16) return mlp_launch<bf16>(d, nullptr, nullptr, stream, true);
+  return fail(FZ_E_ARG, "fz_mlp_chain_nostore: act_dtype must be FZ_STORE_F32 or FZ_STORE_BF16");
+}
+
 extern "C" int fz_mlp_chain_fac(const fz_mlp_desc* d, const fz_outproj_fac* fac, fz_stream_t stream) {
   if (!d || !fac) return fail(FZ_E_ARG, "fz_mlp_chain_fac: null descriptor");
   if (d->act_dtype == FZ_STORE_F32) return mlp_launch<float>(d, nullptr, fac, stream);
diff --git a/factorizer_amd/csrc/mlp_chain64.hip b/factorizer_amd/csrc/mlp_chain64.hip
--- a/factorizer_amd/csrc/mlp_chain64.hip
+++ b/factorizer_amd/csrc/mlp_chain64.hip
@@ -69,490 +69,18 @@
 
 template <bool BWD, typename AT, bool SINGLE = false, bool BX = false, bool P512 = false, bool PRE = false>
 __global__ __launch_bounds__(P512 ? 512 : 256, 2) void gemm_chain64_kernel(GemmArgsT<AT> p, ChainArgsT<AT> c, int ntiles) {
-  constexpr int NACC = 2, C = 64, HID = 128;
-  constexpr int NTA = BxTerms<AT>::A, NTB = bx_terms_b<AT>(BXPRO_GELU);
-  constexpr bool HOIST = SINGLE || sizeof(AT) == 2;
-  static_assert(!P512 || (BX && !SINGLE), "P512: the split-bf16 chain around a pre-split weight image");
-  static_assert(!PRE || (P512 && !BWD), "PRE: the forward chain around the pre-split images");
-  constexpr int NA = P512 ? 12288 : 8192;
-  constexpr int NA0 = PRE ? 6144 : 0;
-  extern __shared__ __attribute__((aligned(16))) float fz_lds_c64[];
-  float* As1 = fz_lds_c64;
-  float* As2 = As1 + NA;
-  float* tW = As2 + NA + NA0;
-  float* tB = tW + 128;
-  float* tB0 = tB + 64;
-  const int half = P512 ? __builtin_amdgcn_readfirstlane((int)(threadIdx.x >> 8)) : 0;
-  float* red = tB + 64 + (PRE ? 64 : 0) + half * 512;
-  static_assert(2 * NA + NA0 + 128 + 64 + (PRE ? 64 : 0) + (P512 ? 2 : 1) * 512 == chain64_lds_floats(P512, PRE), "the launcher's dynamic LDS ends where this carve-up does");
-  const int lane = threadIdx.x & 63, wave = __builtin_amdgcn_readfirstlane((int)(threadIdx.x >> 6) & 3);
-  const int j = lane & 31, h = lane >> 5;
-  const int tiles_per_sample = (int)((p.Ncol + 128 * NACC - 1) / (128 * NACC));
-  int lane4 = lane * 4, lane4b = lane * 4 + NA, lane4c = lane * 4 + 2 * NA;
-  if constexpr (P512) {
-    asm volatile("" : "+v"(lane4));
-    asm volatile("" : "+v"(lane4b));
-    if constexpr (PRE) asm volatile("" : "+v"(lane4c));
-  }
-  auto ld_a1 = [&](int slot3) { return *reinterpret_cast<const bx8*>(As1 + slot3 * 256 + lane4); };
-  auto ld_a2 = [&](int slot3) { return *reinterpret_cast<const bx8*>(As1 + slot3 * 256 + lane4b); };
-  auto ld_a0 = [&](int slot3) { return *reinterpret_cast<const bx8*>(As1 + slot3 * 256 + lane4c); };
-  (void)ld_a0; (void)lane4c; (void)tB0;
-
-  if constexpr (P512) {
-    for (int item = threadIdx.x; item < (PRE ? 2560 : 2048); item += 512) {
-      const int l = item & 63, slot = (item >> 6) & 15, img = item >> 10;
-      float a8[8];
-      if (img == 0) {
-        const int g = slot >> 2, rb = slot & 3;
-#pragma unroll
-        for (int e = 0; e < 8; ++e) {
-          const int rr = 8 * (g & 1) + e;
-          const int k = PRE ? (g >> 1) * 32 + (rr & 3) + 8 * (rr >> 2) + 4 * (l >> 5) : 2 * (8 * g + e) + (l >> 5);
-          a8[e] = weight_at(p, rb * 32 + (l & 31), k);
-          if (!BWD) a8[e] *= p.ln_g[k];
-        }
-      } else if (PRE && img == 2) {
-        const int g = slot >> 1, mb = slot & 1;
-#pragma unroll
-        for (int e = 0; e < 8; ++e) a8[e] = c.preW[(int64_t)(mb * 32 + (l & 31)) * 64 + 2 * (8 * g + e) + (l >> 5)];
-      } else {
-        const int mb = slot & 1, g8 = (slot >> 1) & 1, rb4 = slot >> 2;
-#pragma unroll
-        for (int e = 0; e < 8; ++e) {
-          const int r = 8 * g8 + e;
-          const int k = rb4 * 32 + (r & 3) + 8 * (r >> 2) + 4 * (l >> 5), m = mb * 32 + (l & 31);
-          a8[e] = c.wB_t ? c.wB[(int64_t)k * c.ldwB + m] : c.wB[(int64_t)m * c.ldwB + k];
-        }
-      }
-      bx8 t3[3];
-      bx_split<3>(a8, t3);
-      bx8* dst = reinterpret_cast<bx8*>(img == 0 ? As1 : (img == 1 ? As2 : As2 + NA)) + (slot * 3) * 64 + l;
-      dst[0] = t3[0]; dst[64] = t3[1]; dst[128] = t3[2];
-    }
-  }
-  for (int base = threadIdx.x; !P512 && base < (SINGLE ? 4096 : 16384); base += 256 * 8) {
-    float tmp[8];
-#pragma unroll
-    for (int uu = 0; uu < 8; ++uu) {
-      const int idx = base + uu * 256;
-      float wv;
-      if (SINGLE) {
-        const int l = idx & 63, mb = (idx >> 6) & 1, a = idx >> 7;
-        wv = weight_at(p, mb * 32 + (l & 31), 2 * a + (l >> 5));
-      } else if (idx < 8192) {
-        const int l = idx & 63, rb = (idx >> 6) & 3, a = idx >> 8;
-        const int m = rb * 32 + (l & 31), k = 2 * a + (l >> 5);
-        wv = weight_at(p, m, k);
-        if (!BWD) wv *= p.ln_g[k];
-      } else {
-        const int i2 = idx - 8192;
-        const int l = i2 & 63, mb = (i2 >> 6) & 1, s2 = i2 >> 7;
-        const int r = s2 & 15, rb = s2 >> 4;
-        const int k = rb * 32 + (r & 3) + 8 * (r >> 2) + 4 * (l >> 5), m = mb * 32 + (l & 31);
-        wv = c.wB_t ? c.wB[(int64_t)k * c.ldwB + m] : c.wB[(int64_t)m * c.ldwB + k];
-      }
-      tmp[uu] = wv;
-    }
-#pragma unroll
-    for (int uu = 0; uu < 8; ++uu) fz_lds_c64[base + uu * 256] = tmp[uu];
-  }
-  if (BWD) {
-    if (threadIdx.x < C) tB[threadIdx.x] = p.lnb_g[threadIdx.x];
-  } else {
-    for (int r = threadIdx.x; r < HID; r += blockDim.x) {
-      float t = 0.f;
-      for (int k = 0; k < C; ++k) t += weight_at(p, r, k) * p.ln_b[k];
-      tW[r] = t + (p.bias ? p.bias[r] : 0.f);
-      if (r < C) tB[r] = c.biasB ? c.biasB[r] : 0.f;
-      if (PRE && r < C) tB0[r] = c.preB ? c.preB[r] : 0.f;
-    }
-  }
-
-  const int tstep = P512 ? 2 * (int)gridDim.x : (int)gridDim.x;
-  int tile = P512 ? 2 * (int)blockIdx.x + half : (int)blockIdx.x;
-  float bv[32][NACC];
-  auto fetch_tile = [&](int t) {
-    const int bt = t / tiles_per_sample;
-    const int64_t ct = ((int64_t)(t % tiles_per_sample) * 4 + wave) * (32 * NACC) + NACC * j;
-    const unsigned lo = (unsigned)h * (unsigned)p.Ncol + (unsigned)(ct < p.Ncol ? ct : 0);
-    const AT* xb = (PRE ? c.preA : p.x[0]) + (int64_t)bt * C * p.Ncol;
-#pragma unroll
-    for (int s = 0; s < 32; ++s) vload<NACC>(xb + (int64_t)(2 * s) * p.Ncol + lo, bv[s]);
-  };
-  fetch_tile(tile);
-  __syncthreads();
-
-  for (; tile < ntiles; tile += tstep) {
-    asm volatile("" ::: "memory");
-    const int b = tile / tiles_per_sample;
-    const int64_t col_off = ((int64_t)(tile % tiles_per_sample) * 4 + wave) * (32 * NACC) + NACC * j;
-    const bool col_ok = col_off < p.Ncol;
-    const int64_t nc = col_ok ? col_off : 0;
-    const unsigned lane_row = (unsigned)(4 * h) * (unsigned)p.Ncol + (unsigned)nc;
-
-    f32x16 acc0[PRE ? 2 : 1][NACC];
-    if constexpr (PRE) {
-#pragma unroll
-      for (int mb = 0; mb < 2; ++mb)
-#pragma unroll
-        for (int q = 0; q < NACC; ++q)
-#pragma unroll
-          for (int r = 0; r < 16; ++r) acc0[mb][q][r] = 0.f;
-#pragma unroll
-      for (int g = 0; g < 4; ++g) {
-        bx_group_ps<2, NACC, NTB>(acc0,
-            [&](int mb, int t) { return ld_a0((g * 2 + mb) * 3 + t); },
-            [&](int q, float (&x8)[8]) {
-#pragma unroll
-              for (int e = 0; e < 8; ++e) x8[e] = bv[8 * g + e][q];
-            });
-        __builtin_amdgcn_sched_barrier(0);
-      }
-      const int64_t smp = (int64_t)b * C * p.Ncol;
-      float s1[NACC] = {0.f, 0.f};
-#pragma unroll
-      for (int g8 = 0; g8 < 4; ++g8) {
-        float e[8][NACC];
-#pragma unroll
-        for (int i = 0; i < 8; ++i) {
-          const int rr = g8 * 8 + i, mb = rr >> 4, r = rr & 15;
-          vload<NACC>(c.preRes + smp + (int64_t)(mb * 32 + (r & 3) + 8 * (r >> 2)) * p.Ncol + lane_row, e[i]);
-        }
-#pragma unroll
-        for (int i = 0; i < 8; ++i) {
-          const int rr = g8 * 8 + i, mb = rr >> 4, r = rr & 15;
-          const int rbase = mb * 32 + (r & 3) + 8 * (r >> 2);
-          const float add = tB0[rbase + 4 * h];
-          float v[NACC];
-#pragma unroll
-          for (int q = 0; q < NACC; ++q) v[q] = acc0[mb][q][r] + add + e[i][q];
-          if (col_ok) vstore<NACC>(c.preOut + smp + (int64_t)rbase * p.Ncol + lane_row, v);
-#pragma unroll
-          for (int q = 0; q < NACC; ++q) {
-            if constexpr (sizeof(AT) == 2) v[q] = (float)(AT)v[q];
-            acc0[mb][q][r] = v[q];
-            s1[q] += v[q];
-          }
-        }
-        __builtin_amdgcn_sched_barrier(0);
-      }
-      float mu[NACC], rs[NACC];
-#pragma unroll
-      for (int q = 0; q < NACC; ++q) {
-        s1[q] += __shfl_xor(s1[q], 32, 64);
-        mu[q] = s1[q] / 64.0f;
-        float t = 0.f;
-#pragma unroll
-        for (int mb = 0; mb < 2; ++mb)
-#pragma unroll
-          for (int r = 0; r < 16; ++r) {
-            const float dd = acc0[mb][q][r] - mu[q];
-            t += dd * dd;
-          }
-        t += __shfl_xor(t, 32, 64);
-        rs[q] = 1.0f / sqrtf(t / 64.0f + p.ln_eps);
-#pragma unroll
-        for (int mb = 0; mb < 2; ++mb)
-#pragma unroll
-          for (int r = 0; r < 16; ++r) acc0[mb][q][r] = (acc0[mb][q][r] - mu[q]) * rs[q];
-      }
-      if (p.stats_out != nullptr && h == 0 && col_ok) {
-        float* so = p.stats_out + (int64_t)b * 2 * p.Vin;
-        vstore<NACC>(so + col_off, mu);
-        vstore<NACC>(so + p.Vin + col_off, rs);
-      }
-    }
-
-    if (!BWD && !PRE) {
-      float mu[NACC], rs[NACC];
-#pragma unroll
-      for (int e = 0; e < NACC; ++e) {
-        float t = 0.f;
-#pragma unroll
-        for (int s = 0; s < 32; ++s) t += bv[s][e];
-        t += __shfl_xor(t, 32, 64);
-        mu[e] = t / 64.0f;
-      }
-#pragma unroll
-      for (int e = 0; e < NACC; ++e) {
-        float t = 0.f;
-#pragma unroll
-        for (int s = 0; s < 32; ++s) {
-          const float d = bv[s][e] - mu[e];
-          t += d * d;
-        }
-        t += __shfl_xor(t, 32, 64);
-        rs[e] = 1.0f / sqrtf(t / 64.0f + p.ln_eps);
-      }
-#pragma unroll
-      for (int s = 0; s < 32; ++s)
-#pragma unroll
-        for (int e = 0; e < NACC; ++e) bv[s][e] = (bv[s][e] - mu[e]) * rs[e];
-      if (p.stats_out != nullptr && h == 0 && col_ok) {
-        float* so = p.stats_out + (int64_t)b * 2 * p.Vin;
-        vstore<NACC>(so + col_off, mu);
-        vstore<NACC>(so + p.Vin + col_off, rs);
-      }
-    }
-
-    f32x16 acc2[2][NACC];
-#pragma unroll
-    for (int mb = 0; mb < 2; ++mb)
-#pragma unroll
-      for (int q = 0; q < NACC; ++q)
-#pragma unroll
-        for (int r = 0; r < 16; ++r) acc2[mb][q][r] = 0.f;
-
-    if (SINGLE) {
-      if constexpr (BX) {
-#pragma unroll
-        for (int g = 0; g < 4; ++g) {
-          bx_group<HOIST, 2, NACC, NTA, NTB>(acc2,
-              [&](int mb, float (&a8)[8]) {
-#pragma unroll
-                for (int e = 0; e < 8; ++e) a8[e] = As1[((8 * g + e) * 2 + mb) * 64 + lane];
-              },
-              [&](int q, float (&x8)[8]) {
-#pragma unroll
-                for (int e = 0; e < 8; ++e) x8[e] = bv[8 * g + e][q];
-              });
-          __builtin_amdgcn_sched_barrier(0);
-        }
-      } else {
-#pragma unroll
-      for (int s = 0; s < 32; ++s) {
-#pragma unroll
-        for (int mb = 0; mb < 2; ++mb) {
-          const float av = As1[(s * 2 + mb) * 64 + lane];
-#pragma unroll
-          for (int q = 0; q < NACC; ++q) acc2[mb][q] = __builtin_amdgcn_mfma_f32_32x32x2f32(av, bv[s][q], acc2[mb][q], 0, 0, 0);
-        }
-        if ((s & 3) == 3) __builtin_amdgcn_sched_barrier(0);
-      }
-      }
-      fetch_tile(tile + tstep < ntiles ? tile + tstep : tile);
-    }
-#pragma unroll
-    for (int p2 = 0; p2 < (SINGLE ? 0 : 2); ++p2) {
-      f32x16 acc1[2][NACC];
-#pragma unroll
-      for (int rbl = 0; rbl < 2; ++rbl)
-#pragma unroll
-        for (int q = 0; q < NACC; ++q)
-#pragma unroll
-          for (int r = 0; r < 16; ++r) acc1[rbl][q][r] = 0.f;
-      if constexpr (BX) {
-#pragma unroll
-        for (int g = 0; g < 4; ++g) {
-          if constexpr (P512)
-            bx_group_ps<2, NACC, NTB>(acc1,
-                [&](int rbl, int t) { return ld_a1((g * 4 + 2 * p2 + rbl) * 3 + t); },
-                [&](int q, float (&x8)[8]) {
-#pragma unroll
-                  for (int e = 0; e < 8; ++e) x8[e] = PRE ? acc0[PRE ? (g >> 1) : 0][q][8 * (g & 1) + e] : bv[8 * g + e][q];
-                });
-          else
-          bx_group<HOIST, 2, NACC, NTA, NTB>(acc1,
-              [&](int rbl, float (&a8)[8]) {
-#pragma unroll
-                for (int e = 0; e < 8; ++e) a8[e] = As1[((8 * g + e) * 4 + 2 * p2 + rbl) * 64 + lane];
-              },
-              [&](int q, float (&x8)[8]) {
-#pragma unroll
-                for (int e = 0; e < 8; ++e) x8[e] = bv[8 * g + e][q];
-              });
-          __builtin_amdgcn_sched_barrier(0);
-        }
-      } else {
-#pragma unroll
-      for (int s = 0; s < 32; ++s) {
-#pragma unroll
-        for (int rbl = 0; rbl < 2; ++rbl) {
-          const float av = As1[(s * 4 + 2 * p2 + rbl) * 64 + lane];
-#pragma unroll
-          for (int q = 0; q < NACC; ++q) acc1[rbl][q] = __builtin_amdgcn_mfma_f32_32x32x2f32(av, bv[s][q], acc1[rbl][q], 0, 0, 0);
-        }
-        if ((s & 3) == 3) __builtin_amdgcn_sched_barrier(0);
-      }
-      }
-      if (p2 == 1) fetch_tile(tile + tstep < ntiles ? tile + tstep : tile);
-
-      if (!BWD) {
-#pragma unroll
-        for (int rbl = 0; rbl < 2; ++rbl)
-#pragma unroll
-          for (int r = 0; r < 16; ++r) {
-            const int rbase = (2 * p2 + rbl) * 32 + (r & 3) + 8 * (r >> 2);
-            const float add = tW[rbase + 4 * h];
-            float v[NACC];
-#pragma unroll
-            for (int q = 0; q < NACC; ++q) v[q] = acc1[rbl][q][r] + add;
-            if (col_ok) vstore<NACC>(c.side + ((int64_t)b * HID + rbase) * p.Ncol + lane_row, v);
-            if constexpr (NACC == 2) {
-              float gq[2];
-              gelu2_f(v, gq);
-              acc1[rbl][0][r] = gq[0]; acc1[rbl][1][r] = gq[1];
-            } else {
-#pragma unroll
-              for (int q = 0; q < NACC; ++q) acc1[rbl][q][r] = gelu_f(v[q]);
-            }
-          }
-      } else {
-#pragma unroll
-        for (int g8 = 0; g8 < 4; ++g8) {
-          float e[8][NACC];
-#pragma unroll
-          for (int i = 0; i < 8; ++i) {
-            const int rr = g8 * 8 + i, rbl = rr >> 4, r = rr & 15;
-            const int rbase = (2 * p2 + rbl) * 32 + (r & 3) + 8 * (r >> 2);
-            vload<NACC>(p.emul + ((int64_t)b * HID + rbase) * p.Ncol + lane_row, e[i]);
-          }
-#pragma unroll
-          for (int i = 0; i < 8; ++i) {
-            const int rr = g8 * 8 + i, rbl = rr >> 4, r = rr & 15;
-            const int rbase = (2 * p2 + rbl) * 32 + (r & 3) + 8 * (r >> 2);
-            float v[NACC];
-#pragma unroll
-            for (int q = 0; q < NACC; ++q) v[q] = acc1[rbl][q][r] * gelu_grad_f(e[i][q]);
-            if (col_ok) vstore<NACC>(c.side + ((int64_t)b * HID + rbase) * p.Ncol + lane_row, v);
-#pragma unroll
-            for (int q = 0; q < NACC; ++q) acc1[rbl][q][r] = v[q];
-          }
-          __builtin_amdgcn_sched_barrier(0);
-        }
-      }
-
-      if constexpr (BX) {
-#pragma unroll
-        for (int g = 0; g < 4; ++g) {
-          if constexpr (P512)
-            bx_group_ps<2, NACC, NTB>(acc2,
-                [&](int mb, int t) { return ld_a2((((2 * p2 + (g >> 1)) * 2 + (g & 1)) * 2 + mb) * 3 + t); },
-                [&](int q, float (&x8)[8]) {
-#pragma unroll
-                  for (int e = 0; e < 8; ++e) x8[e] = acc1[g >> 1][q][8 * (g & 1) + e];
-                });
-          else
-          bx_group<HOIST, 2, NACC, NTA, NTB>(acc2,
-              [&](int mb, float (&a8)[8]) {
-#pragma unroll
-                for (int e = 0; e < 8; ++e) a8[e] = As2[(((2 * p2 + (g >> 1)) * 16 + 8 * (g & 1) + e) * 2 + mb) * 64 + lane];
-              },
-              [&](int q, float (&x8)[8]) {
-#pragma unroll
-                for (int e = 0; e < 8; ++e) x8[e] = acc1[g >> 1][q][8 * (g & 1) + e];
-              });
-          __builtin_amdgcn_sched_barrier(0);
-        }
-      } else {
-#pragma unroll
-      for (int rbl = 0; rbl < 2; ++rbl)
-#pragma unroll
-        for (int r = 0; r < 16; ++r) {
-#pragma unroll
-          for (int mb = 0; mb < 2; ++mb) {
-            const float av = As2[(((2 * p2 + rbl) * 16 + r) * 2 + mb) * 64 + lane];
-#pragma unroll
-            for (int q = 0; q < NACC; ++q) acc2[mb][q] = __builtin_amdgcn_mfma_f32_32x32x2f32(av, acc1[rbl][q][r], acc2[mb][q], 0, 0, 0);
-          }
-          if ((r & 3) == 3) __builtin_amdgcn_sched_barrier(0);
-        }
-      }
-    }
-
-    const int64_t sample = (int64_t)b * C * p.Ncol;
-    if (!BWD) {
-#pragma unroll
-      for (int g8 = 0; g8 < 4; ++g8) {
-        float e[8][NACC];
-#pragma unroll
-        for (int i = 0; i < 8; ++i) {
-          const int rr = g8 * 8 + i, mb = rr >> 4, r = rr & 15;
-          vload<NACC>(p.res + sample + (int64_t)(mb * 32 + (r & 3) + 8 * (r >> 2)) * p.Ncol + lane_row, e[i]);
-        }
-#pragma unroll
-        for (int i = 0; i < 8; ++i) {
-          const int rr = g8 * 8 + i, mb = rr >> 4, r = rr & 15;
-          const int rbase = mb * 32 + (r & 3) + 8 * (r >> 2);
-          const float add = tB[rbase + 4 * h];
-          float v[NACC];
-#pragma unroll
-          for (int q = 0; q < NACC; ++q) v[q] = acc2[mb][q][r] + add + e[i][q];
-          if (col_ok) vstore<NACC>(p.y + sample + (int64_t)rbase * p.Ncol + lane_row, v);
-        }
-        __builtin_amdgcn_sched_barrier(0);
-      }
-    } else {
-      const float* sp = p.lnb_stats + (int64_t)b * 2 * p.Ncol;
-      float mu[NACC], rs[NACC];
-      vload<NACC>(sp + nc, mu);
-      vload<NACC>(sp + p.Ncol + nc, rs);
-      float xs[32][NACC];
-      float m1[NACC] = {0.f, 0.f}, m2[NACC] = {0.f, 0.f};
-#pragma unroll
-      for (int g8 = 0; g8 < 4; ++g8) {
-#pragma unroll
-        for (int i = 0; i < 8; ++i) {
-          const int rr = g8 * 8 + i, mb = rr >> 4, r = rr & 15;
-          vload<NACC>(p.lnb_x + sample + (int64_t)(mb * 32 + (r & 3) + 8 * (r >> 2)) * p.Ncol + lane_row, xs[rr]);
-        }
-#pragma unroll
-        for (int i = 0; i < 8; ++i) {
-          const int rr = g8 * 8 + i, mb = rr >> 4, r = rr & 15;
-          const float gc = tB[mb * 32 + (r & 3) + 8 * (r >> 2) + 4 * h];
-#pragma unroll
-          for (int q = 0; q < NACC; ++q) {
-            const float av = acc2[mb][q][r] * gc;
-            xs[rr][q] = (xs[rr][q] - mu[q]) * rs[q];
-            m1[q] += av;
-            m2[q] += av * xs[rr][q];
-          }
-        }
-        __builtin_amdgcn_sched_barrier(0);
-      }
-#pragma unroll
-      for (int q = 0; q < NACC; ++q) {
-        m1[q] = (m1[q] + __shfl_xor(m1[q], 32, 64)) * (1.0f / 64.0f);
-        m2[q] = (m2[q] + __shfl_xor(m2[q], 32, 64)) * (1.0f / 64.0f);
-      }
-#pragma unroll
-      for (int g8 = 0; g8 < 4; ++g8) {
-        float ga[8][NACC];
-#pragma unroll
-        for (int i = 0; i < 8; ++i) {
-          const int rr = g8 * 8 + i, mb = rr >> 4, r = rr & 15;
-          vload<NACC>(p.lnb_gadd + sample + (int64_t)(mb * 32 + (r & 3) + 8 * (r >> 2)) * p.Ncol + lane_row, ga[i]);
-        }
-#pragma unroll
-        for (int i = 0; i < 8; ++i) {
-          const int rr = g8 * 8 + i, mb = rr >> 4, r = rr & 15;
-          const int rbase = mb * 32 + (r & 3) + 8 * (r >> 2);
-          const int row = rbase + 4 * h;
-          const float gc = tB[row];
-          float v[NACC];
-#pragma unroll
-          for (int q = 0; q < NACC; ++q) v[q] = rs[q] * (acc2[mb][q][r] * gc - m1[q] - xs[rr][q] * m2[q]) + ga[i][q];
-          if (col_ok) vstore<NACC>(p.y + sample + (int64_t)rbase * p.Ncol + lane_row, v);
-          float sg = col_ok ? acc2[mb][0][r] * xs[rr][0] + acc2[mb][1][r] * xs[rr][1] : 0.f;
-          float sb = col_ok ? acc2[mb][0][r] + acc2[mb][1][r] : 0.f;
-          sg = half_sum32(sg);
-          sb = half_sum32(sb);
-          if ((lane & 31) == 31) {
-            red[wave * 128 + row] = sg;
-            red[wave * 128 + 64 + row] = sb;
-          }
-        }
-        __builtin_amdgcn_sched_barrier(0);
-      }
-      __syncthreads();
-      if ((threadIdx.x & 255) < 128) {
-        const int e = threadIdx.x & 255;
-        p.lnb_part[(int64_t)tile * 128 + e] = (red[e] + red[128 + e]) + (red[256 + e] + red[384 + e]);
-      }
-      __syncthreads();
-    }
-  }
+  constexpr bool NOSIDE = false;
+#include "mlp_chain64_body.inc"
+}
+template <typename AT, bool BX, bool P512>
+__global__ __launch_bounds__(P512 ? 512 : 256, 2) void gemm_chain64_ns_kernel(GemmArgsT<AT> p, ChainArgsT<AT> c, int ntiles) {
+  constexpr bool BWD = true, SINGLE = false, PRE = false, NOSIDE = true;
+#include "mlp_chain64_body.inc"
+}
+template <typename AT>
+static void (*chain64_ns_kernel(bool p512))(GemmArgsT<AT>, ChainArgsT<AT>, int) {
+  if constexpr (sizeof(AT) == 4) return p512 ? gemm_chain64_ns_kernel<AT, true, true> : gemm_chain64_ns_kernel<AT, false, false>;
+  else return nullptr;
 }
 
 template <typename AT>
@@ -561,8 +89,10 @@
   const bool bwd = d->mode != 0, pre = d->pre_in != nullptr;
   const bool p512 = products_split(d->products) && ntiles % 2 == 0 && knob_chain64_p512();
   if (pre && !p512) return fail(FZ_E_UNSUPPORTED, "fz_mlp_chain: the fused out-projection at C == 64 needs an even number of tiles");
+  const bool noside = bwd && c.side == nullptr;
   void (*kern)(GemmArgsT<AT>, ChainArgsT<AT>, int) =
       pre ? gemm_chain64_kernel<false, AT, false, true, true, true>
+      : noside ? chain64_ns_kernel<AT>(p512)
       : p512 ? (bwd ? gemm_chain64_kernel<true, AT, false, true, true> : gemm_chain64_kernel<false, AT, false, true, true>)
              : (bwd ? gemm_chain64_kernel<true, AT, false, false> : gemm_chain64_kernel<false, AT, false, false>);
   const int work = p512 ? ntiles / 2 : ntiles, wgs = p512 ? 256 : knob_mlp_wgs(512);
diff --git a/factorizer_amd/csrc/mlp_chain64_body.inc b/factorizer_amd/csrc/mlp_chain64_body.inc
--- /dev/null
+++ b/factorizer_amd/csrc/mlp_chain64_body.inc
@@ -0,0 +1,487 @@
+  static_assert(!NOSIDE || (BWD && !SINGLE), "NOSIDE: the backward chain without its gz1 store");
+  constexpr int NACC = 2, C = 64, HID = 128;
+  constexpr int NTA = BxTerms<AT>::A, NTB = bx_terms_b<AT>(BXPRO_GELU);
+  constexpr bool HOIST = SINGLE || sizeof(AT) == 2;
+  static_assert(!P512 || (BX && !SINGLE), "P512: the split-bf16 chain around a pre-split weight image");
+  static_assert(!PRE || (P512 && !BWD), "PRE: the forward chain around the pre-split images");
+  constexpr int NA = P512 ? 12288 : 8192;
+  constexpr int NA0 = PRE ? 6144 : 0;
+  extern __shared__ __attribute__((aligned(16))) float fz_lds_c64[];
+  float* As1 = fz_lds_c64;
+  float* As2 = As1 + NA;
+  float* tW = As2 + NA + NA0;
+  float* tB = tW + 128;
+  float* tB0 = tB + 64;
+  const int half = P512 ? __builtin_amdgcn_readfirstlane((int)(threadIdx.x >> 8)) : 0;
+  float* red = tB + 64 + (PRE ? 64 : 0) + half * 512;
+  static_assert(2 * NA + NA0 + 128 + 64 + (PRE ? 64 : 0) + (P512 ? 2 : 1) * 512 == chain64_lds_floats(P512, PRE), "the launcher's dynamic LDS ends where this carve-up does");
+  const int lane = threadIdx.x & 63, wave = __builtin_amdgcn_readfirstlane((int)(threadIdx.x >> 6) & 3);
+  const int j = lane & 31, h = lane >> 5;
+  const int tiles_per_sample = (int)((p.Ncol + 128 * NACC - 1) / (128 * NACC));
+  int lane4 = lane * 4, lane4b = lane * 4 + NA, lane4c = lane * 4 + 2 * NA;
+  if constexpr (P512) {
+    asm volatile("" : "+v"(lane4));
+    asm volatile("" : "+v"(lane4b));
+    if constexpr (PRE) asm volatile("" : "+v"(lane4c));
+  }
+  auto ld_a1 = [&](int slot3) { return *reinterpret_cast<const bx8*>(As1 + slot3 * 256 + lane4); };
+  auto ld_a2 = [&](int slot3) { return *reinterpret_cast<const bx8*>(As1 + slot3 * 256 + lane4b); };
+  auto ld_a0 = [&](int slot3) { return *reinterpret_cast<const bx8*>(As1 + slot3 * 256 + lane4c); };
+  (void)ld_a0; (void)lane4c; (void)tB0;
+
+  if constexpr (P512) {
+    for (int item = threadIdx.x; item < (PRE ? 2560 : 2048); item += 512) {
+      const int l = item & 63, slot = (item >> 6) & 15, img = item >> 10;
+      float a8[8];
+      if (img == 0) {
+        const int g = slot >> 2, rb = slot & 3;
+#pragma unroll
+        for (int e = 0; e < 8; ++e) {
+          const int rr = 8 * (g & 1) + e;
+          const int k = PRE ? (g >> 1) * 32 + (rr & 3) + 8 * (rr >> 2) + 4 * (l >> 5) : 2 * (8 * g + e) + (l >> 5);
+          a8[e] = weight_at(p, rb * 32 + (l & 31), k);
+          if (!BWD) a8[e] *= p.ln_g[k];
+        }
+      } else if (PRE && img == 2) {
+        const int g = slot >> 1, mb = slot & 1;
+#pragma unroll
+        for (int e = 0; e < 8; ++e) a8[e] = c.preW[(int64_t)(mb * 32 + (l & 31)) * 64 + 2 * (8 * g + e) + (l >> 5)];
+      } else {
+        const int mb = slot & 1, g8 = (slot >> 1) & 1, rb4 = slot >> 2;
+#pragma unroll
+        for (int e = 0; e < 8; ++e) {
+          const int r = 8 * g8 + e;
+          const int k = rb4 * 32 + (r & 3) + 8 * (r >> 2) + 4 * (l >> 5), m = mb * 32 + (l & 31);
+          a8[e] = c.wB_t ? c.wB[(int64_t)k * c.ldwB + m] : c.wB[(int64_t)m * c.ldwB + k];
+        }
+      }
+      bx8 t3[3];
+      bx_split<3>(a8, t3);
+      bx8* dst = reinterpret_cast<bx8*>(img == 0 ? As1 : (img == 1 ? As2 : As2 + NA)) + (slot * 3) * 64 + l;
+      dst[0] = t3[0]; dst[64] = t3[1]; dst[128] = t3[2];
+    }
+  }
+  for (int base = threadIdx.x; !P512 && base < (SINGLE ? 4096 : 16384); base += 256 * 8) {
+    float tmp[8];
+#pragma unroll
+    for (int uu = 0; uu < 8; ++uu) {
+      const int idx = base + uu * 256;
+      float wv;
+      if (SINGLE) {
+        const int l = idx & 63, mb = (idx >> 6) & 1, a = idx >> 7;
+        wv = weight_at(p, mb * 32 + (l & 31), 2 * a + (l >> 5));
+      } else if (idx < 8192) {
+        const int l = idx & 63, rb = (idx >> 6) & 3, a = idx >> 8;
+        const int m = rb * 32 + (l & 31), k = 2 * a + (l >> 5);
+        wv = weight_at(p, m, k);
+        if (!BWD) wv *= p.ln_g[k];
+      } else {
+        const int i2 = idx - 8192;
+        const int l = i2 & 63, mb = (i2 >> 6) & 1, s2 = i2 >> 7;
+        const int r = s2 & 15, rb = s2 >> 4;
+        const int k = rb * 32 + (r & 3) + 8 * (r >> 2) + 4 * (l >> 5), m = mb * 32 + (l & 31);
+        wv = c.wB_t ? c.wB[(int64_t)k * c.ldwB + m] : c.wB[(int64_t)m * c.ldwB + k];
+      }
+      tmp[uu] = wv;
+    }
+#pragma unroll
+    for (int uu = 0; uu < 8; ++uu) fz_lds_c64[base + uu * 256] = tmp[uu];
+  }
+  if (BWD) {
+    if (threadIdx.x < C) tB[threadIdx.x] = p.lnb_g[threadIdx.x];
+  } else {
+    for (int r = threadIdx.x; r < HID; r += blockDim.x) {
+      float t = 0.f;
+      for (int k = 0; k < C; ++k) t += weight_at(p, r, k) * p.ln_b[k];
+      tW[r] = t + (p.bias ? p.bias[r] : 0.f);
+      if (r < C) tB[r] = c.biasB ? c.biasB[r] : 0.f;
+      if (PRE && r < C) tB0[r] = c.preB ? c.preB[r] : 0.f;
+    }
+  }
+
+  const int tstep = P512 ? 2 * (int)gridDim.x : (int)gridDim.x;
+  int tile = P512 ? 2 * (int)blockIdx.x + half : (int)blockIdx.x;
+  float bv[32][NACC];
+  auto fetch_tile = [&](int t) {
+    const int bt = t / tiles_per_sample;
+    const int64_t ct = ((int64_t)(t % tiles_per_sample) * 4 + wave) * (32 * NACC) + NACC * j;
+    const unsigned lo = (unsigned)h * (unsigned)p.Ncol + (unsigned)(ct < p.Ncol ? ct : 0);
+    const AT* xb = (PRE ? c.preA : p.x[0]) + (int64_t)bt * C * p.Ncol;
+#pragma unroll
+    for (int s = 0; s < 32; ++s) vload<NACC>(xb + (int64_t)(2 * s) * p.Ncol + lo, bv[s]);
+  };
+  fetch_tile(tile);
+  __syncthreads();
+
+  for (; tile < ntiles; tile += tstep) {
+    asm volatile("" ::: "memory");
+    const int b = tile / tiles_per_sample;
+    const int64_t col_off = ((int64_t)(tile % tiles_per_sample) * 4 + wave) * (32 * NACC) + NACC * j;
+    const bool col_ok = col_off < p.Ncol;
+    const int64_t nc = col_ok ? col_off : 0;
+    const unsigned lane_row = (unsigned)(4 * h) * (unsigned)p.Ncol + (unsigned)nc;
+
+    f32x16 acc0[PRE ? 2 : 1][NACC];
+    if constexpr (PRE) {
+#pragma unroll
+      for (int mb = 0; mb < 2; ++mb)
+#pragma unroll
+        for (int q = 0; q < NACC; ++q)
+#pragma unroll
+          for (int r = 0; r < 16; ++r) acc0[mb][q][r] = 0.f;
+#pragma unroll
+      for (int g = 0; g < 4; ++g) {
+        bx_group_ps<2, NACC, NTB>(acc0,
+            [&](int mb, int t) { return ld_a0((g * 2 + mb) * 3 + t); },
+            [&](int q, float (&x8)[8]) {
+#pragma unroll
+              for (int e = 0; e < 8; ++e) x8[e] = bv[8 * g + e][q];
+            });
+        __builtin_amdgcn_sched_barrier(0);
+      }
+      const int64_t smp = (int64_t)b * C * p.Ncol;
+      float s1[NACC] = {0.f, 0.f};
+#pragma unroll
+      for (int g8 = 0; g8 < 4; ++g8) {
+        float e[8][NACC];
+#pragma unroll
+        for (int i = 0; i < 8; ++i) {
+          const int rr = g8 * 8 + i, mb = rr >> 4, r = rr & 15;
+          vload<NACC>(c.preRes + smp + (int64_t)(mb * 32 + (r & 3) + 8 * (r >> 2)) * p.Ncol + lane_row, e[i]);
+        }
+#pragma unroll
+        for (int i = 0; i < 8; ++i) {
+          const int rr = g8 * 8 + i, mb = rr >> 4, r = rr & 15;
+          const int rbase = mb * 32 + (r & 3) + 8 * (r >> 2);
+          const float add = tB0[rbase + 4 * h];
+          float v[NACC];
+#pragma unroll
+          for (int q = 0; q < NACC; ++q) v[q] = acc0[mb][q][r] + add + e[i][q];
+          if (col_ok) vstore<NACC>(c.preOut + smp + (int64_t)rbase * p.Ncol + lane_row, v);
+#pragma unroll
+          for (int q = 0; q < NACC; ++q) {
+            if constexpr (sizeof(AT) == 2) v[q] = (float)(AT)v[q];
+            acc0[mb][q][r] = v[q];
+            s1[q] += v[q];
+          }
+        }
+        __builtin_amdgcn_sched_barrier(0);
+      }
+      float mu[NACC], rs[NACC];
+#pragma unroll
+      for (int q = 0; q < NACC; ++q) {
+        s1[q] += __shfl_xor(s1[q], 32, 64);
+        mu[q] = s1[q] / 64.0f;
+        float t = 0.f;
+#pragma unroll
+        for (int mb = 0; mb < 2; ++mb)
+#pragma unroll
+          for (int r = 0; r < 16; ++r) {
+            const float dd = acc0[mb][q][r] - mu[q];
+            t += dd * dd;
+          }
+        t += __shfl_xor(t, 32, 64);
+        rs[q] = 1.0f / sqrtf(t / 64.0f + p.ln_eps);
+#pragma unroll
+        for (int mb = 0; mb < 2; ++mb)
+#pragma unroll
+          for (int r = 0; r < 16; ++r) acc0[mb][q][r] = (acc0[mb][q][r] - mu[q]) * rs[q];
+      }
+      if (p.stats_out != nullptr && h == 0 && col_ok) {
+        float* so = p.stats_out + (int64_t)b * 2 * p.Vin;
+        vstore<NACC>(so + col_off, mu);
+        vstore<NACC>(so + p.Vin + col_off, rs);
+      }
+    }
+
+    if (!BWD && !PRE) {
+      float mu[NACC], rs[NACC];
+#pragma unroll
+      for (int e = 0; e < NACC; ++e) {
+        float t = 0.f;
+#pragma unroll
+        for (int s = 0; s < 32; ++s) t += bv[s][e];
+        t += __shfl_xor(t, 32, 64);
+        mu[e] = t / 64.0f;
+      }
+#pragma unroll
+      for (int e = 0; e < NACC; ++e) {
+        float t = 0.f;
+#pragma unroll
+        for (int s = 0; s < 32; ++s) {
+          const float d = bv[s][e] - mu[e];
+          t += d * d;
+        }
+        t += __shfl_xor(t, 32, 64);
+        rs[e] = 1.0f / sqrtf(t / 64.0f + p.ln_eps);
+      }
+#pragma unroll
+      for (int s = 0; s < 32; ++s)
+#pragma unroll
+        for (int e = 0; e < NACC; ++e) bv[s][e] = (bv[s][e] - mu[e]) * rs[e];
+      if (p.stats_out != nullptr && h == 0 && col_ok) {
+        float* so = p.stats_out + (int64_t)b * 2 * p.Vin;
+        vstore<NACC>(so + col_off, mu);
+        vstore<NACC>(so + p.Vin + col_off, rs);
+      }
+    }
+
+    f32x16 acc2[2][NACC];
+#pragma unroll
+    for (int mb = 0; mb < 2; ++mb)
+#pragma unroll
+      for (int q = 0; q < NACC; ++q)
+#pragma unroll
+        for (int r = 0; r < 16; ++r) acc2[mb][q][r] = 0.f;
+
+    if (SINGLE) {
+      if constexpr (BX) {
+#pragma unroll
+        for (int g = 0; g < 4; ++g) {
+          bx_group<HOIST, 2, NACC, NTA, NTB>(acc2,
+              [&](int mb, float (&a8)[8]) {
+#pragma unroll
+                for (int e = 0; e < 8; ++e) a8[e] = As1[((8 * g + e) * 2 + mb) * 64 + lane];
+              },
+              [&](int q, float (&x8)[8]) {
+#pragma unroll
+                for (int e = 0; e < 8; ++e) x8[e] = bv[8 * g + e][q];
+              });
+          __builtin_amdgcn_sched_barrier(0);
+        }
+      } else {
+#pragma unroll
+      for (int s = 0; s < 32; ++s) {
+#pragma unroll
+        for (int mb = 0; mb < 2; ++mb) {
+          const float av = As1[(s * 2 + mb) * 64 + lane];
+#pragma unroll
+          for (int q = 0; q < NACC; ++q) acc2[mb][q] = __builtin_amdgcn_mfma_f32_32x32x2f32(av, bv[s][q], acc2[mb][q], 0, 0, 0);
+        }
+        if ((s & 3) == 3) __builtin_amdgcn_sched_barrier(0);
+      }
+      }
+      fetch_tile(tile + tstep < ntiles ? tile + tstep : tile);
+    }
+#pragma unroll
+    for (int p2 = 0; p2 < (SINGLE ? 0 : 2); ++p2) {
+      f32x16 acc1[2][NACC];
+#pragma unroll
+      for (int rbl = 0; rbl < 2; ++rbl)
+#pragma unroll
+        for (int q = 0; q < NACC; ++q)
+#pragma unroll
+          for (int r = 0; r < 16; ++r) acc1[rbl][q][r] = 0.f;
+      if constexpr (BX) {
+#pragma unroll
+        for (int g = 0; g < 4; ++g) {
+          if constexpr (P512)
+            bx_group_ps<2, NACC, NTB>(acc1,
+                [&](int rbl, int t) { return ld_a1((g * 4 + 2 * p2 + rbl) * 3 + t); },
+                [&](int q, float (&x8)[8]) {
+#pragma unroll
+                  for (int e = 0; e < 8; ++e) x8[e] = PRE ? acc0[PRE ? (g >> 1) : 0][q][8 * (g & 1) + e] : bv[8 * g + e][q];
+                });
+          else
+          bx_group<HOIST, 2, NACC, NTA, NTB>(acc1,
+              [&](int rbl, float (&a8)[8]) {
+#pragma unroll
+                for (int e = 0; e < 8; ++e) a8[e] = As1[((8 * g + e) * 4 + 2 * p2 + rbl) * 64 + lane];
+              },
+              [&](int q, float (&x8)[8]) {
+#pragma unroll
+                for (int e = 0; e < 8; ++e) x8[e] = bv[8 * g + e][q];
+              });
+          __builtin_amdgcn_sched_barrier(0);
+        }
+      } else {
+#pragma unroll
+      for (int s = 0; s < 32; ++s) {
+#pragma unroll
+        for (int rbl = 0; rbl < 2; ++rbl) {
+          const float av = As1[(s * 4 + 2 * p2 + rbl) * 64 + lane];
+#pragma unroll
+          for (int q = 0; q < NACC; ++q) acc1[rbl][q] = __builtin_amdgcn_mfma_f32_32x32x2f32(av, bv[s][q], acc1[rbl][q], 0, 0, 0);
+        }
+        if ((s & 3) == 3) __builtin_amdgcn_sched_barrier(0);
+      }
+      }
+      if (p2 == 1) fetch_tile(tile + tstep < ntiles ? tile + tstep : tile);
+
+      if (!BWD) {
+#pragma unroll
+        for (int rbl = 0; rbl < 2; ++rbl)
+#pragma unroll
+          for (int r = 0; r < 16; ++r) {
+            const int rbase = (2 * p2 + rbl) * 32 + (r & 3) + 8 * (r >> 2);
+            const float add = tW[rbase + 4 * h];
+            float v[NACC];
+#pragma unroll
+            for (int q = 0; q < NACC; ++q) v[q] = acc1[rbl][q][r] + add;
+            if (col_ok) vstore<NACC>(c.side + ((int64_t)b * HID + rbase) * p.Ncol + lane_row, v);
+            if constexpr (NACC == 2) {
+              float gq[2];
+              gelu2_f(v, gq);
+              acc1[rbl][0][r] = gq[0]; acc1[rbl][1][r] = gq[1];
+            } else {
+#pragma unroll
+              for (int q = 0; q < NACC; ++q) acc1[rbl][q][r] = gelu_f(v[q]);
+            }
+          }
+      } else {
+#pragma unroll
+        for (int g8 = 0; g8 < 4; ++g8) {
+          float e[8][NACC];
+#pragma unroll
+          for (int i = 0; i < 8; ++i) {
+            const int rr = g8 * 8 + i, rbl = rr >> 4, r = rr & 15;
+            const int rbase = (2 * p2 + rbl) * 32 + (r & 3) + 8 * (r >> 2);
+            vload<NACC>(p.emul + ((int64_t)b * HID + rbase) * p.Ncol + lane_row, e[i]);
+          }
+#pragma unroll
+          for (int i = 0; i < 8; ++i) {
+            const int rr = g8 * 8 + i, rbl = rr >> 4, r = rr & 15;
+            const int rbase = (2 * p2 + rbl) * 32 + (r & 3) + 8 * (r >> 2);
+            float v[NACC];
+#pragma unroll
+            for (int q = 0; q < NACC; ++q) v[q] = acc1[rbl][q][r] * gelu_grad_f(e[i][q]);
+            if constexpr (!NOSIDE) {
+              if (col_ok) vstore<NACC>(c.side + ((int64_t)b * HID + rbase) * p.Ncol + lane_row, v);
+            }
+#pragma unroll
+            for (int q = 0; q < NACC; ++q) acc1[rbl][q][r] = v[q];
+          }
+          __builtin_amdgcn_sched_barrier(0);
+        }
+      }
+
+      if constexpr (BX) {
+#pragma unroll
+        for (int g = 0; g < 4; ++g) {
+          if constexpr (P512)
+            bx_group_ps<2, NACC, NTB>(acc2,
+                [&](int mb, int t) { return ld_a2((((2 * p2 + (g >> 1)) * 2 + (g & 1)) * 2 + mb) * 3 + t); },
+                [&](int q, float (&x8)[8]) {
+#pragma unroll
+                  for (int e = 0; e < 8; ++e) x8[e] = acc1[g >> 1][q][8 * (g & 1) + e];
+                });
+          else
+          bx_group<HOIST, 2, NACC, NTA, NTB>(acc2,
+              [&](int mb, float (&a8)[8]) {
+#pragma unroll
+                for (int e = 0; e < 8; ++e) a8[e] = As2[(((2 * p2 + (g >> 1)) * 16 + 8 * (g & 1) + e) * 2 + mb) * 64 + lane];
+              },
+              [&](int q, float (&x8)[8]) {
+#pragma unroll
+                for (int e = 0; e < 8; ++e) x8[e] = acc1[g >> 1][q][8 * (g & 1) + e];
+              });
+          __builtin_amdgcn_sched_barrier(0);
+        }
+      } else {
+#pragma unroll
+      for (int rbl = 0; rbl < 2; ++rbl)
+#pragma unroll
+        for (int r = 0; r < 16; ++r) {
+#pragma unroll
+          for (int mb = 0; mb < 2; ++mb) {
+            const float av = As2[(((2 * p2 + rbl) * 16 + r) * 2 + mb) * 64 + lane];
+#pragma unroll
+            for (int q = 0; q < NACC; ++q) acc2[mb][q] = __builtin_amdgcn_mfma_f32_32x32x2f32(av, acc1[rbl][q][r], acc2[mb][q], 0, 0, 0);
+          }
+          if ((r & 3) == 3) __builtin_amdgcn_sched_barrier(0);
+        }
+      }
+    }
+
+    const int64_t sample = (int64_t)b * C * p.Ncol;
+    if (!BWD) {
+#pragma unroll
+      for (int g8 = 0; g8 < 4; ++g8) {
+        float e[8][NACC];
+#pragma unroll
+        for (int i = 0; i < 8; ++i) {
+          const int rr = g8 * 8 + i, mb = rr >> 4, r = rr & 15;
+          vload<NACC>(p.res + sample + (int64_t)(mb * 32 + (r & 3) + 8 * (r >> 2)) * p.Ncol + lane_row, e[i]);
+        }
+#pragma unroll
+        for (int i = 0; i < 8; ++i) {
+          const int rr = g8 * 8 + i, mb = rr >> 4, r = rr & 15;
+          const int rbase = mb * 32 + (r & 3) + 8 * (r >> 2);
+          const float add = tB[rbase + 4 * h];
+          float v[NACC];
+#pragma unroll
+          for (int q = 0; q < NACC; ++q) v[q] = acc2[mb][q][r] + add + e[i][q];
+          if (col_ok) vstore<NACC>(p.y + sample + (int64_t)rbase * p.Ncol + lane_row, v);
+        }
+        __builtin_amdgcn_sched_barrier(0);
+      }
+    } else {
+      const float* sp = p.lnb_stats + (int64_t)b * 2 * p.Ncol;
+      float mu[NACC], rs[NACC];
+      vload<NACC>(sp + nc, mu);
+      vload<NACC>(sp + p.Ncol + nc, rs);
+      float xs[32][NACC];
+      float m1[NACC] = {0.f, 0.f}, m2[NACC] = {0.f, 0.f};
+#pragma unroll
+      for (int g8 = 0; g8 < 4; ++g8) {
+#pragma unroll
+        for (int i = 0; i < 8; ++i) {
+          const int rr = g8 * 8 + i, mb = rr >> 4, r = rr & 15;
+          vload<NACC>(p.lnb_x + sample + (int64_t)(mb * 32 + (r & 3) + 8 * (r >> 2)) * p.Ncol + lane_row, xs[rr]);
+        }
+#pragma unroll
+        for (int i = 0; i < 8; ++i) {
+          const int rr = g8 * 8 + i, mb = rr >> 4, r = rr & 15;
+          const float gc = tB[mb * 32 + (r & 3) + 8 * (r >> 2) + 4 * h];
+#pragma unroll
+          for (int q = 0; q < NACC; ++q) {
+            const float av = acc2[mb][q][r] * gc;
+            xs[rr][q] = (xs[rr][q] - mu[q]) * rs[q];
+            m1[q] += av;
+            m2[q] += av * xs[rr][q];
+          }
+        }
+        __builtin_amdgcn_sched_barrier(0);
+      }
+#pragma unroll
+      for (int q = 0; q < NACC; ++q) {
+        m1[q] = (m1[q] + __shfl_xor(m1[q], 32, 64)) * (1.0f / 64.0f);
+        m2[q] = (m2[q] + __shfl_xor(m2[q], 32, 64)) * (1.0f / 64.0f);
+      }
+#pragma unroll
+      for (int g8 = 0; g8 < 4; ++g8) {
+        float ga[8][NACC];
+#pragma unroll
+        for (int i = 0; i < 8; ++i) {
+          const int rr = g8 * 8 + i, mb = rr >> 4, r = rr & 15;
+          vload<NACC>(p.lnb_gadd + sample + (int64_t)(mb * 32 + (r & 3) + 8 * (r >> 2)) * p.Ncol + lane_row, ga[i]);
+        }
+#pragma unroll
+        for (int i = 0; i < 8; ++i) {
+          const int rr = g8 * 8 + i, mb = rr >> 4, r = rr & 15;
+          const int rbase = mb * 32 + (r & 3) + 8 * (r >> 2);
+          const int row = rbase + 4 * h;
+          const float gc = tB[row];
+          float v[NACC];
+#pragma unroll
+          for (int q = 0; q < NACC; ++q) v[q] = rs[q] * (acc2[mb][q][r] * gc - m1[q] - xs[rr][q] * m2[q]) + ga[i][q];
+          if (col_ok) vstore<NACC>(p.y + sample + (int64_t)rbase * p.Ncol + lane_row, v);
+          float sg = col_ok ? acc2[mb][0][r] * xs[rr][0] + acc2[mb][1][r] * xs[rr][1] : 0.f;
+          float sb = col_ok ? acc2[mb][0][r] + acc2[mb][1][r] : 0.f;
+          sg = half_sum32(sg);
+          sb = half_sum32(sb);
+          if ((lane & 31) == 31) {
+            red[wave * 128 + row] = sg;
+            red[wave * 128 + 64 + row] = sb;
+          }
+        }
+        __builtin_amdgcn_sched_barrier(0);
+      }
+      __syncthreads();
+      if ((threadIdx.x & 255) < 128) {
+        const int e = threadIdx.x & 255;
+        p.lnb_part[(int64_t)tile * 128 + e] = (red[e] + red[128 + e]) + (red[256 + e] + red[384 + e]);
+      }
+      __syncthreads();
+    }
+  }
diff --git a/factorizer_amd/csrc/mlp_wgrad_pair.hip b/factorizer_amd/csrc/mlp_wgrad_pair.hip
--- /dev/null
+++ b/factorizer_amd/csrc/mlp_wgrad_pair.hip
@@ -0,0 +1,265 @@
+#include "finish.h"
+#include "mlp_chain.h"
+
+namespace fz {
+
+constexpr int kPairTile = 32;
+constexpr int kPairCap = 512;
+constexpr int kPairImg = 768;
+constexpr int kPairLdsFloats = 2 * 3 * kPairImg * 4;
+
+struct PairArgs {
+  const float* g2;
+  const float* z1;
+  const float* x1;
+  const float* stats;
+  const float* w2;
+  float* p2;
+  float* pb2;
+  float* p1;
+  float* pb1;
+  int64_t V;
+  int tiles_per_sample, ntiles;
+};
+
+__device__ __forceinline__ void pair_gelu_both(float x, float& g, float& dg) {
+  const float ax = fabsf(x) * 0.70710678118654752f;
+  const float E = __expf(-0.5f * x * x);
+  const float t = __builtin_amdgcn_rcpf(1.0f + 0.3275911f * ax);
+  const float poly = t * (0.254829592f + t * (-0.284496736f + t * (1.421413741f + t * (-1.453152027f + t * 1.061405429f))));
+  const float r = 1.0f - poly * E;
+  const float cdf = 0.5f * (1.0f + __builtin_copysignf(r, x));
+  g = x * cdf;
+  dg = cdf + x * (0.3989422804014327f * E);
+}
+
+typedef __bf16 bx4 __attribute__((ext_vector_type(4)));
+__device__ __forceinline__ bx4 bx_half(const bx8& v, int hi) {
+  return hi ? __builtin_shufflevector(v, v, 4, 5, 6, 7) : __builtin_shufflevector(v, v, 0, 1, 2, 3);
+}
+
+__global__ __launch_bounds__(256, 2) void mlp_wgrad_pair_kernel(PairArgs a) {
+  extern __shared__ __attribute__((aligned(16))) float fz_lds_pair[];
+  bx8* const lds = reinterpret_cast<bx8*>(fz_lds_pair);
+  static_assert(2 * 3 * kPairImg * 4 == kPairLdsFloats, "the launcher's dynamic LDS ends where this carve-up does");
+  const int tid = threadIdx.x, lane = tid & 63, wave = __builtin_amdgcn_readfirstlane(tid >> 6);
+  const int n = lane & 31, h = lane >> 5;
+  const int nwg = gridDim.x;
+  const int t0 = (int)((int64_t)blockIdx.x * a.ntiles / nwg), t1 = (int)((int64_t)(blockIdx.x + 1) * a.ntiles / nwg);
+  const int64_t V = a.V;
+
+  bx8 w2op[4][3];
+#pragma unroll
+  for (int s = 0; s < 4; ++s) {
+    float w8[8];
+#pragma unroll
+    for (int e = 0; e < 8; ++e) w8[e] = a.w2[(16 * s + 8 * h + e) * 128 + 32 * wave + n];
+    bx_split<3>(w8, w2op[s]);
+  }
+
+  const int sc = tid >> 3, sq = tid & 7;
+  const int sv = tid & 31, sg = tid >> 5;
+  float pg[2][4], px[2][4], pmu[4], prs[4], pa[8];
+  auto load_tile = [&](int t) {
+    const int b = t / a.tiles_per_sample;
+    const int64_t v0 = (int64_t)(t - b * a.tiles_per_sample) * kPairTile;
+    const float* gb = a.g2 + (int64_t)b * 64 * V + v0;
+    const float* xb = a.x1 + (int64_t)b * 64 * V + v0;
+    const float* sb = a.stats + (int64_t)b * 2 * V + v0;
+#pragma unroll
+    for (int i = 0; i < 2; ++i) {
+      aload<4>(gb + (int64_t)(sc + 32 * i) * V + 4 * sq, pg[i]);
+      aload<4>(xb + (int64_t)(sc + 32 * i) * V + 4 * sq, px[i]);
+    }
+    aload<4>(sb + 4 * sq, pmu);
+    aload<4>(sb + V + 4 * sq, prs);
+#pragma unroll
+    for (int e = 0; e < 8; ++e) pa[e] = gb[(int64_t)(8 * sg + e) * V + sv];
+  };
+  auto load_z = [&](int t, float (&z)[16]) {
+    const int b = t / a.tiles_per_sample;
+    const int64_t v0 = (int64_t)(t - b * a.tiles_per_sample) * kPairTile;
+    const float* zb = a.z1 + ((int64_t)b * 128 + 32 * wave + n) * V + v0 + 4 * h;
+#pragma unroll
+    for (int g = 0; g < 4; ++g) {
+      float q[4];
+      aload<4>(zb + 8 * g, q);
+#pragma unroll
+      for (int i = 0; i < 4; ++i) z[4 * g + i] = q[i];
+    }
+  };
+
+  f32x16 acc2[2], acc1[2];
+#pragma unroll
+  for (int cb = 0; cb < 2; ++cb)
+#pragma unroll
+    for (int r = 0; r < 16; ++r) { acc2[cb][r] = 0.f; acc1[cb][r] = 0.f; }
+  float sb2[2] = {0.f, 0.f}, sb1 = 0.f;
+
+  load_tile(t0);
+  for (int t = t0; t < t1; ++t) {
+    bx8* const GA = lds + ((t - t0) & 1) * 3 * kPairImg;
+    bx8* const GB = GA + kPairImg;
+    bx8* const XB = GB + kPairImg;
+    float z[16];
+    load_z(t, z);
+    {
+      float v8[8];
+      bx8 t3[3];
+      const int unit = (sq >> 2) * 64 + (sc & 31) + 32 * (sq & 1), slot = (sq >> 1) & 1;
+#pragma unroll
+      for (int i = 0; i < 8; ++i) v8[i] = pg[i >> 2][i & 3];
+      sb2[0] += (pg[0][0] + pg[0][1]) + (pg[0][2] + pg[0][3]);
+      sb2[1] += (pg[1][0] + pg[1][1]) + (pg[1][2] + pg[1][3]);
+      bx_split<3>(v8, t3);
+#pragma unroll
+      for (int lv = 0; lv < 3; ++lv)
+#pragma unroll
+        for (int cb = 0; cb < 2; ++cb)
+          reinterpret_cast<bx4*>(GB + ((lv * 2 + cb) * 2) * 64 + unit)[slot] = bx_half(t3[lv], cb);
+#pragma unroll
+      for (int i = 0; i < 8; ++i) v8[i] = (px[i >> 2][i & 3] - pmu[i & 3]) * prs[i & 3];
+      bx_split<3>(v8, t3);
+#pragma unroll
+      for (int lv = 0; lv < 3; ++lv)
+#pragma unroll
+        for (int cb = 0; cb < 2; ++cb)
+          reinterpret_cast<bx4*>(XB + ((lv * 2 + cb) * 2) * 64 + unit)[slot] = bx_half(t3[lv], cb);
+      bx_split<3>(pa, t3);
+#pragma unroll
+      for (int lv = 0; lv < 3; ++lv) GA[(lv * 4 + (sg >> 1)) * 64 + sv + 32 * (sg & 1)] = t3[lv];
+    }
+    load_tile(t + 1 < t1 ? t + 1 : t);
+    __syncthreads();
+
+    f32x16 gh;
+#pragma unroll
+    for (int r = 0; r < 16; ++r) gh[r] = 0.f;
+#pragma unroll
+    for (int s = 0; s < 4; ++s) {
+      bx8 aop[3];
+#pragma unroll
+      for (int lv = 0; lv < 3; ++lv) aop[lv] = GA[(lv * 4 + s) * 64 + lane];
+      bx_mfma<3, 3>(gh, aop, w2op[s]);
+    }
+    float ge[16], gz[16];
+#pragma unroll
+    for (int r = 0; r < 16; ++r) {
+      float dg;
+      pair_gelu_both(z[r], ge[r], dg);
+      gz[r] = gh[r] * dg;
+    }
+    {
+      float s4[4];
+#pragma unroll
+      for (int g = 0; g < 4; ++g) s4[g] = (gz[4 * g] + gz[4 * g + 1]) + (gz[4 * g + 2] + gz[4 * g + 3]);
+      sb1 += (s4[0] + s4[1]) + (s4[2] + s4[3]);
+    }
+#pragma unroll
+    for (int s = 0; s < 2; ++s) {
+      float v8[8];
+      bx8 eop[3], zop[3];
+#pragma unroll
+      for (int e = 0; e < 8; ++e) v8[e] = ge[8 * s + e];
+      bx_split<3>(v8, eop);
+#pragma unroll
+      for (int e = 0; e < 8; ++e) v8[e] = gz[8 * s + e];
+      bx_split<3>(v8, zop);
+#pragma unroll
+      for (int cb = 0; cb < 2; ++cb) {
+        bx8 bop[3];
+#pragma unroll
+        for (int lv = 0; lv < 3; ++lv) bop[lv] = GB[((lv * 2 + cb) * 2 + s) * 64 + lane];
+        bx_mfma<3, 3>(acc2[cb], eop, bop);
+#pragma unroll
+        for (int lv = 0; lv < 3; ++lv) bop[lv] = XB[((lv * 2 + cb) * 2 + s) * 64 + lane];
+        bx_mfma<3, 3>(acc1[cb], zop, bop);
+      }
+    }
+  }
+
+  const int64_t row = blockIdx.x;
+  float* p2 = a.p2 + row * 8192;
+  float* p1 = a.p1 + row * 8192;
+#pragma unroll
+  for (int cb = 0; cb < 2; ++cb) {
+    const int c = 32 * cb + n;
+#pragma unroll
+    for (int g = 0; g < 4; ++g) {
+      const int hid = 32 * wave + 8 * g + 4 * h;
+      *reinterpret_cast<float4*>(p2 + c * 128 + hid) = make_float4(acc2[cb][4 * g], acc2[cb][4 * g + 1], acc2[cb][4 * g + 2], acc2[cb][4 * g + 3]);
+#pragma unroll
+      for (int i = 0; i < 4; ++i) p1[(hid + i) * 64 + c] = acc1[cb][4 * g + i];
+    }
+  }
+  sb1 += __shfl_xor(sb1, 32, 64);
+  if (h == 0) a.pb1[row * 128 + 32 * wave + n] = sb1;
+#pragma unroll
+  for (int i = 0; i < 2; ++i) {
+    float s = sb2[i];
+    s += __shfl_xor(s, 1, 64);
+    s += __shfl_xor(s, 2, 64);
+    s += __shfl_xor(s, 4, 64);
+    if (sq == 0) a.pb2[row * 64 + sc + 32 * i] = s;
+  }
+}
+
+static int64_t pair_units(int B, int64_t V) { return (V / kPairTile) * (int64_t)B; }
+
+}
+
+using namespace fz;
+
+extern "C" int fz_mlp_wgrad_pair_supported(int C, int H, int64_t V, int act_dtype, int products) {
+  return (C == 64 && H == 128 && V > 0 && (V % kPairTile) == 0 && V <= ((int64_t)1 << 27) && act_dtype == FZ_STORE_F32
+          && products_split(products)) ? 1 : 0;
+}
+
+extern "C" int fz_mlp_wgrad_pair_rows(int B, int64_t V) {
+  if (B < 0 || V < 0) return 0;
+  const int64_t u = pair_units(B, V);
+  return (int)(u < kPairCap ? u : kPairCap);
+}
+
+extern "C" int64_t fz_mlp_wgrad_pair_workspace_bytes(int B, int64_t V) {
+  const int64_t rows = fz_mlp_wgrad_pair_rows(B, V);
+  return (rows > 0 ? rows : 1) * (int64_t)(2 * 8192 + 64 + 128) * (int64_t)sizeof(float);
+}
+
+extern "C" int fz_mlp_wgrad_pair(const fz_mlp_desc* d, void* workspace, fz_stream_t stream) {
+  if (!d || !workspace) return fail(FZ_E_ARG, "fz_mlp_wgrad_pair: null descriptor/workspace");
+  if (d->act_dtype != FZ_STORE_F32 && d->act_dtype != FZ_STORE_BF16)
+    return fail(FZ_E_ARG, "fz_mlp_wgrad_pair: act_dtype must be FZ_STORE_F32 or FZ_STORE_BF16");
+  if (!fz_mlp_wgrad_pair_supported(d->C, d->H, d->V, d->act_dtype, d->products))
+    return fail(FZ_E_UNSUPPORTED, "fz_mlp_wgrad_pair: needs (C, H) = (64, 128), V % 32 == 0, fp32 storage, split-bf16 products");
+  if (d->B < 0) return fail(FZ_E_SHAPE, "fz_mlp_wgrad_pair: negative batch");
+  if (!d->in || !d->z1 || !d->x1 || !d->stats || !d->w2 || !d->ln_g || !d->ln_b || !d->gw1 || !d->gb1 || !d->gw2 || !d->gb2)
+    return fail(FZ_E_ARG, "fz_mlp_wgrad_pair: needs in (g2), z1, x1, stats, w2, gamma, beta, gw1, gb1, gw2, gb2");
+  if ((reinterpret_cast<uintptr_t>(d->in) | reinterpret_cast<uintptr_t>(d->z1) | reinterpret_cast<uintptr_t>(d->x1) |
+       reinterpret_cast<uintptr_t>(d->stats) | reinterpret_cast<uintptr_t>(workspace)) & 15)
+    return fail(FZ_E_ARG, "fz_mlp_wgrad_pair: in, z1, x1, stats and the workspace must be 16-byte aligned");
+  hipStream_t st = (hipStream_t)stream;
+  if (d->B == 0) {
+    FZ_HIP_OK(hipMemsetAsync(d->gw1, 0, sizeof(float) * 8192, st));
+    FZ_HIP_OK(hipMemsetAsync(d->gw2, 0, sizeof(float) * 8192, st));
+    FZ_HIP_OK(hipMemsetAsync(d->gb1, 0, sizeof(float) * 128, st));
+    FZ_HIP_OK(hipMemsetAsync(d->gb2, 0, sizeof(float) * 64, st));
+    return FZ_OK;
+  }
+  const int rows = fz_mlp_wgrad_pair_rows(d->B, d->V);
+  PairArgs a;
+  a.g2 = (const float*)d->in; a.z1 = (const float*)d->z1; a.x1 = (const float*)d->x1; a.stats = d->stats; a.w2 = d->w2;
+  a.p2 = (float*)workspace;
+  a.p1 = a.p2 + (int64_t)rows * 8192;
+  a.pb2 = a.p1 + (int64_t)rows * 8192;
+  a.pb1 = a.pb2 + (int64_t)rows * 64;
+  a.V = d->V; a.tiles_per_sample = (int)(d->V / kPairTile); a.ntiles = (int)pair_units(d->B, d->V);
+  const int rc = launch_lds(mlp_wgrad_pair_kernel, dim3((unsigned)rows), dim3(256), kPairLdsFloats, st, a);
+  if (rc != FZ_OK) return rc;
+  FinishJob fj[2];
+  fj[0] = finish_job(FK_WGRAD, 8192 / 64 + 1);
+  fj[0].u.wg = WgradFinishOne{a.p2, a.pb2, d->gw2, d->gb2, nullptr, nullptr, rows, 64, 128, 0, 8192 / 64, 2};
+  fj[1] = finish_job(FK_WGRAD, 8192 / 64 + 2);
+  fj[1].u.wg = WgradFinishOne{a.p1, a.pb1, d->gw1, d->gb1, d->ln_g, d->ln_b, rows, 128, 64, 0, 8192 / 64, 2};
+  return finish_run(fj, 2, st);
+}
diff --git a/factorizer_amd/pointwise.py b/factorizer_amd/pointwise.py
--- a/factorizer_amd/pointwise.py
+++ b/factorizer_amd/pointwise.py
@@ -328,6 +328,49 @@
         N.check(rc, "fz_mlp_chain")
         ggamma, gbeta = _reduce_affine_rows(part, rows, C, x1)
     return gz1, gx1, ggamma, gbeta
+
+
+def _mlp_wgrad_pair_ok(C, Hd, V, dtype=torch.float32, drop=None):
+    if (C, Hd) != (64, 128) or drop is not None or dtype != torch.float32 or os.environ.get("FZ_MLP_WGRAD_PAIR", "1") == "0":
+        return False
+    return _mlp_chain_ok(C, Hd, V) and bool(N.lib().fz_mlp_wgrad_pair_supported(C, Hd, V, N.STORE_F32, N.products()))
+
+
+def _mlp_bwd_chain_nostore(g2, z1, w12, w22, x1, st, ln_w):
+    B, C = x1.shape[:2]
+    V = _vox(x1)
+    Hd = w12.shape[0]
+    gx1 = torch.empty_like(x1)
+    rows = N.lib().fz_mlp_partials(B, V)
+    part = torch.empty((rows, 2 * C), dtype=torch.float32, device=x1.device)
+    d = _mlp_desc(1, x1, w12, w22, B=B, C=C, Hd=Hd, V=V, inp=g2, ln_w=ln_w, stats=st, z1=z1, x1=x1, out=gx1)
+    d.part = part.data_ptr()
+    with torch.cuda.device(x1.device):
+        rc = Fn._timed(f"mlp_chain_bwd_{C}", x1.element_size() * (3 * x1.numel() + z1.numel()),
+                       lambda: N.lib().fz_mlp_chain_nostore(ctypes.byref(d), N.stream_ptr(x1)), cols=B * V, flops=4 * B * V * C * Hd)
+        N.check(rc, "fz_mlp_chain_nostore")
+        ggamma, gbeta = _reduce_affine_rows(part, rows, C, x1)
+    return gx1, ggamma, gbeta
+
+
+def _mlp_wgrad_pair(g2, z1, w12, w22, x1, st, ln_w, ln_b):
+    B, C = x1.shape[:2]
+    V = _vox(x1)
+    Hd = w12.shape[0]
+    dev = x1.device
+    gw1 = _GB.out_like(w12, (Hd, C), torch.float32)
+    gw2 = _GB.out_like(w22, (C, Hd), torch.float32)
+    gb1 = torch.empty(Hd, dtype=torch.float32, device=dev)
+    gb2 = torch.empty(C, dtype=torch.float32, device=dev)
+    ws = torch.empty(N.lib().fz_mlp_wgrad_pair_workspace_bytes(B, V) // 4, dtype=torch.float32, device=dev)
+    d = _mlp_desc(1, x1, w12, w22, B=B, C=C, Hd=Hd, V=V, inp=g2, ln_w=ln_w, ln_b=ln_b, stats=st, z1=z1, x1=x1)
+    d.gw1, d.gb1, d.gw2, d.gb2 = gw1.data_ptr(), gb1.data_ptr(), gw2.data_ptr(), gb2.data_ptr()
+    with torch.cuda.device(dev), _finish_scope(ws, gw1, gb1, gw2, gb2):
+        rc = Fn._timed(f"wgrad_mlp_pair_{C}x{Hd}", x1.element_size() * (2 * x1.numel() + z1.numel()),
+                       lambda: N.lib().fz_mlp_wgrad_pair(ctypes.byref(d), ws.data_ptr(), N.stream_ptr(x1)),
+                       cols=B * V, flops=6 * B * V * C * Hd)
+    N.check(rc, "fz_mlp_wgrad_pair")
+    return gw1, gb1, gw2, gb2
 
 
 def _mlp_wgrad_fused_ok(C, Hd, V):
@@ -1400,6 +1443,9 @@
         (p0, p1, p2), (m0, m1, m2) = drop or (0, 0, 0), bits
         if drop is None and _mlp_wgrad_fused_ok(C, Hd, V):
             gx1, gg2, gbt2, gw1, gb1, gw2, gb2 = _mlp_bwd_chain_wgrad(g2, z1, w12, w22, x1, st2, n2w, n2b)
+        elif chain and _mlp_wgrad_pair_ok(C, Hd, V, dt, drop):
+            gx1, gg2, gbt2 = _mlp_bwd_chain_nostore(g2, z1, w12, w22, x1, st2, n2w)
+            gw1, gb1, gw2, gb2 = _mlp_wgrad_pair(g2, z1, w12, w22, x1, st2, n2w, n2b)
         else:
             gelu = ACT["gelu" if m1 is None else "none"]
             gf = Fn.dropout_apply(N.DROP_RES, m2, p2, g2) if m2 is not None else g2
diff --git a/include/factorizer_hip.h b/include/factorizer_hip.h
--- a/include/factorizer_hip.h
+++ b/include/factorizer_hip.h
@@ -309,6 +309,11 @@
 int64_t fz_mlp_wgrad_workspace_bytes(int B, int64_t V);
 int fz_mlp_chain(const fz_mlp_desc* desc, fz_stream_t stream);
 int fz_mlp_chain_drop(const fz_mlp_desc* desc, const fz_mlp_dropout* drop, fz_stream_t stream);
+int fz_mlp_chain_nostore(const fz_mlp_desc* desc, fz_stream_t stream);
+int fz_mlp_wgrad_pair_supported(int C, int H, int64_t V, int act_dtype, int products);
+int fz_mlp_wgrad_pair_rows(int B, int64_t V);
+int64_t fz_mlp_wgrad_pair_workspace_bytes(int B, int64_t V);
+int fz_mlp_wgrad_pair(const fz_mlp_desc* desc, void* workspace, fz_stream_t stream);
 
 #define FZ_QL_PLAIN 0
 #define FZ_QL_S2D 1
```

After: 135.7 (median of 6 runs). About the same (+0.2%).
